# swacisko/ALGA

Measured on AMD Instinct MI355X. Metric: overlap_edges_per_sec, higher is better.
Workload: dtype u32; 1 GPU; cfg4_50M_150bp: 50000000 x 150 bp reads, genome 250000000, seed 11, err 0.00 -> 90621096 nodes (both strands, duplicates removed), min_overlap 82, rsoemo 116; generated on the device (alga_amd.workload.device_build) in 1.0 s; nodes=90621096, edges=92350115

## Files before the change

### alga_amd/csrc/engine.hip

```cpp
#include <hip/hip_runtime.h>

#include <algorithm>
#include <chrono>
#include <cstdio>
#include <cstdlib>
#include <cstring>
#include <new>
#include <string>
#include <thread>
#include <vector>

#include "engine_internal.h"

using namespace alga;

namespace {

using Prepared = AlgaPrepared;

int prepare(alga_engine *e, const alga_nodes *nodes, const alga_prefsuf_params *p, hipStream_t s, Prepared &out) {
    if (!nodes || !p) return alga_fail(e, ALGA_ERR_INVALID_ARGUMENT, "nodes/params must not be NULL");
    if (nodes->n < 0) return alga_fail(e, ALGA_ERR_INVALID_ARGUMENT, "negative node count");
    if (nodes->n > 0 && (!nodes->words || !nodes->len)) return alga_fail(e, ALGA_ERR_INVALID_ARGUMENT, "words/len must not be NULL");
    if (nodes->stride_words <= 0 && nodes->n > 0) return alga_fail(e, ALGA_ERR_INVALID_ARGUMENT, "stride_words must be positive");
// ... 89 lines not shown
    if ((rc = alga_ensure(e, e->cl_pile_tab, pile_table_bytes(n_buckets)))) return rc;
    if (e->cl_pile_tab.p != before || e->cl_pile_tab.cap != cap_before) {
        HIP_TRY(e, hipMemsetAsync(e->cl_pile_tab.p, 0, e->cl_pile_tab.cap, s));
        HIP_TRY(e, hipStreamSynchronize(s));
        e->pile_epoch = 0;
    }
    return ALGA_OK;
}

int discover_impl(alga_engine *e, const Prepared &pp, int32_t src_begin, int32_t src_end, hipStream_t s, uint64_t *n_rec, bool local = false,
                  bool *overflow = nullptr) {
    int rc;
    const NodesDev &nd = pp.nd;
    const PrefSufCfg &cfg = pp.cfg;
    unsigned long long *cnt = (unsigned long long *) e->counters.p;
    *n_rec = 0;
    HIP_TRY(e, hipEventRecord(e->ev[EV_START], s));
    if (pp.live >= (1ull << 31)) return alga_fail(e, ALGA_ERR_CAPACITY, "too many nodes for one seed table; shard the input");
    const bool clustered = local && pp.cluster_eq != 0;
    e->pairs_timed = false;
    e->store_timed = false;
    e->pile_timed = false;
    e->pile_deg_pending = false;
    const bool all_sources = src_begin == 0 && src_end == pp.nd.n;
    const bool pile_index_left = e->opt_pile_range != 0 && e->pile_n == pp.nd.n && e->pile_words == (const void *) pp.nd.words;
    bool pile = clustered && e->opt_pile != 0 && e->opt_cluster_pairs != 0 && e->opt_cluster_order != 0 && pp.local_sw == 1 &&
                      (pp.keys_shared == 0 || (pp.keys_shared == 2 && pile_index_left)) &&
                      (all_sources || (e->opt_pile_range != 0 && src_begin >= 0 && src_end <= pp.nd.n && src_begin < src_end)) && pile_plan(cfg, pp.cluster, pp.cluster_eq, pp.uniform_len, pp.nd.from != nullptr || pp.nd.to != nullptr);
    e->loc_second_used = false;
    bool keys_only = false;
    const bool need_vals = !e->opt_own_sort || e->opt_test_unsorted_index;
    uint32_t n_buckets = 0, filter_bits = 0;
    bool have_table = false;
    auto build_table = [&]() -> int {
        n_buckets = seed_buckets_for(pp.live, e->seed_fill_x10);
        const size_t table_bytes = (size_t) n_buckets * SEED_BUCKET * sizeof(unsigned long long);
        int r;
        if ((r = alga_ensure(e, e->table, table_bytes))) return r;
        HIP_TRY(e, hipMemsetAsync(e->table.p, 0xFF, table_bytes, s));
        filter_bits = seed_filter_bits_for(pp.live);
        if (filter_bits) {
            if ((r = alga_ensure(e, e->filter, filter_bits / 8))) return r;
            HIP_TRY(e, hipMemsetAsync(e->filter.p, 0, filter_bits / 8, s));
        }
        launch_seed_build(nd, cfg, (unsigned long long *) e->table.p, n_buckets, (uint32_t *) e->filter.p, filter_bits, s);
        if ((r = alga_check_launch(e, "k_seed_build"))) return r;
        e->stats.table_slots = (uint64_t) n_buckets * SEED_BUCKET;
        have_table = true;
        return ALGA_OK;
    };
    ClusterCfg cc{};
    if (clustered) {
        cc = pp.cluster;
        if ((rc = cluster_alloc(e, pp))) return rc;
        if (pp.keys_shared == 2) {
            const bool store_left = e->store_n == nd.n && e->store_words == (const void *) nd.words && e->store_eq == pp.cluster_eq && e->store_buckets == cc.n_buckets;
            const bool piles_serve = pile && e->pile_kept_pure && e->store_buckets == cc.n_buckets && e->store_eq == pp.cluster_eq;
            if (!(store_left || piles_serve) || src_begin < e->store_run_begin || src_end > e->store_run_end)
                return alga_fail(e, ALGA_ERR_INVALID_ARGUMENT, "keys_shared = 2: no entry array of this node set that covers the sources is left from the previous build");
            keys_only = pile && e->pile_keys_only;
        } else {
            int32_t run_begin = 0, run_end = nd.n;
            if (pp.keys_shared == 1) {
                if (e->keyed_n != nd.n || e->keyed_words != (const void *) nd.words || src_begin < e->keyed_begin || src_end > e->keyed_end)
                    return alga_fail(e, ALGA_ERR_INVALID_ARGUMENT, "keys_shared: alga_prefsuf_keys_device has not been called on this node set for a range that covers the sources");
                run_begin = e->keyed_begin; run_end = e->keyed_end;
            } else {
                keys_only = pile && e->opt_pile_runs != 0 && !e->expect_pairwise && !e->opt_pile_check;
                launch_cluster_keys(nd, cfg, cc, 0, nd.n, (uint32_t *) e->cl_keys[0].p, need_vals ? (uint32_t *) e->cl_vals[0].p : nullptr, (uint32_t *) e->cl_meta.p, e->cl_runs.p,
                                    (uint8_t *) e->cl_nruns.p, s, !keys_only);
                if ((rc = alga_check_launch(e, "k_node_runs"))) return rc;
            }
            HIP_TRY(e, hipEventRecord(e->ev[EV_KEYS], s));
            e->keyed_n = -1;
            e->store_n = -1;
            HIP_TRY(e, launch_cluster_store(nd, cc, (uint32_t *) e->cl_keys[0].p, (uint32_t *) e->cl_vals[0].p, (uint32_t *) e->cl_keys[1].p,
                                            (uint32_t *) e->cl_vals[1].p, e->sort_temp.p, cluster_sort_temp_bytes((uint64_t) nd.n), e->cl_dir.p, pp.keys_shared == 1 || !need_vals,
                                            e->ev[EV_SORT], cnt + CNT_TOTAL + 1, e->opt_test_unsorted_index != 0, s, e->opt_own_sort != 0));
            HIP_TRY(e, hipEventRecord(e->ev[EV_DIR], s));
            e->pile_n = -1;
            if (pile) {
                rc = e->opt_test_pile_oom ? alga_fail(e, ALGA_ERR_OUT_OF_MEMORY, "pile_alloc (option test_pile_oom)") : pile_alloc(e, (uint64_t) nd.n, cc.n_buckets, s);
                if (rc == ALGA_ERR_OUT_OF_MEMORY) {
                    (void) hipGetLastError();
                    alga_release(e->cl_pile_tab); alga_release(e->cl_pile_rec); alga_release(e->cl_pile_rec2); alga_release(e->cl_pile_succ); alga_release(e->cl_pile_own);
                    alga_release(e->cl_pile_list);
                    e->pile_epoch = 0; e->pile_n = -1;
                    e->err.clear();
                    pile = false;
                    rc = ALGA_OK;
                    if (keys_only) {
                        launch_cluster_keys(nd, cfg, cc, 0, nd.n, (uint32_t *) e->cl_keys[0].p, (uint32_t *) e->cl_vals[0].p, (uint32_t *) e->cl_meta.p, e->cl_runs.p,
                                            (uint8_t *) e->cl_nruns.p, s, true);
                        if ((rc = alga_check_launch(e, "k_node_runs"))) return rc;
                        keys_only = false;
                    }
                } else if (rc) return rc;
            }
            if (pile) {
                launch_pile_sample(nd, cc, pp.uniform_len, (const uint32_t *) e->cl_keys[1].p, (const uint32_t *) e->cl_vals[1].p, e->cl_dir.p,
                                   (unsigned long long *) e->cl_pile_cnt.p, e->opt_pile >= 2 ? e->opt_pile - 1 : 0, s);
                if ((rc = alga_check_launch(e, "k_pile_build<sample>"))) return rc;
            }
            HIP_TRY(e, launch_cluster_gather(nd, cc, pp.cluster_eq, (const uint32_t *) e->cl_keys[1].p, (const uint32_t *) e->cl_vals[1].p, (const uint32_t *) e->cl_meta.p,
                                             pp.uniform_len, e->cl_store.p, (pile && e->opt_pile_skip_gather) ? (const unsigned long long *) e->cl_pile_cnt.p : nullptr, s));
            HIP_TRY(e, hipEventRecord(e->ev[EV_GATHER], s));
            if (pile) {
                if (e->pile_epoch >= 511u) {
                    HIP_TRY(e, hipMemsetAsync(e->cl_pile_tab.p, 0, e->cl_pile_tab.cap, s));
                    e->pile_epoch = 0;
                }
                e->pile_epoch++;
                const bool from_consensus = e->opt_pile_runs != 0;
                launch_pile_build(nd, cfg, cc, pp.uniform_len, (const uint32_t *) e->cl_keys[1].p, (const uint32_t *) e->cl_vals[1].p, e->cl_dir.p, e->cl_pile_rec.p, e->cl_pile_rec2.p, e->cl_pile_tab.p,
                                  e->pile_epoch, e->cl_pile_succ.p, e->cl_runs.p, pp.uniform_len - cfg.Lmin + 1, (const unsigned long long *) e->cl_pile_cnt.p,
                                  from_consensus ? (uint32_t *) e->cl_pile_own.p : nullptr, (from_consensus && e->opt_pile_runs_list) ? e->cl_pile_list.p : nullptr, s);
                if ((rc = alga_check_launch(e, "k_pile_build"))) return rc;
                if (keys_only) {
                    launch_pile_own_ids((const uint32_t *) e->cl_pile_own.p, (const uint32_t *) e->cl_vals[1].p, (uint64_t) nd.n, (int32_t *) e->cl_defer.p, (uint32_t) nd.n,
                                        (unsigned long long *) e->cl_pile_cnt.p, s);
                    launch_cluster_runs_list(nd, cfg, cc, (const int32_t *) e->cl_defer.p, (const unsigned long long *) e->cl_pile_cnt.p + 3, (uint32_t) nd.n, (uint32_t) e->n_cu * 16u,
                                             e->cl_runs.p, (uint8_t *) e->cl_nruns.p, s);
                    launch_cluster_keys(nd, cfg, cc, 0, nd.n, (uint32_t *) e->cl_keys[0].p, (uint32_t *) e->cl_vals[0].p, (uint32_t *) e->cl_meta.p, e->cl_runs.p,
                                        (uint8_t *) e->cl_nruns.p, s, true, (const unsigned long long *) e->cl_pile_cnt.p);
                    if ((rc = alga_check_launch(e, "k_node_runs (own lists)"))) return rc;
                }
                if (e->opt_pile_check && from_consensus)
                    launch_pile_check(e->cl_pile_succ.p, (uint64_t) nd.n, cc.n_buckets, e->cl_pile_tab.p, e->cl_pile_rec2.p, e->pile_epoch, e->cl_runs.p, nd.n, pp.uniform_len - cfg.Lmin + 1,
                                      (unsigned long long *) e->cl_pile_cnt.p, s);
                e->pile_n = nd.n; e->pile_words = (const void *) nd.words;
                e->pile_keys_only = keys_only; e->pile_kept_pure = false;
                e->pile_timed = nd.n > 0;
            }
            e->store_timed = nd.n > 0;
            e->store_n = pile ? -1 : nd.n;
            e->store_words = (const void *) nd.words; e->store_eq = pp.cluster_eq; e->store_buckets = cc.n_buckets;
            e->store_run_begin = run_begin; e->store_run_end = run_end;
        }
        e->stats.table_slots = cc.n_buckets;
    } else if ((rc = build_table())) return rc;
    HIP_TRY(e, hipEventRecord(e->ev[EV_SEED], s));

    const uint64_t n_src = (uint64_t) std::max<int64_t>(0, (int64_t) src_end - src_begin);
    const uint64_t slack = std::max(probe_record_slack(e->n_cu, n_src, local), clustered ? cluster_record_slack(e->n_cu, n_src) : 0);
    uint64_t &hint = local ? e->rec_cap_hint_local : e->rec_cap_hint;
    uint64_t cap = std::max<uint64_t>(hint, (local ? 2 : 16) * n_src + 4096) + slack;
    if (local) {
        if ((rc = alga_ensure(e, e->outdeg, (size_t) (n_src + 1) * sizeof(uint32_t)))) return rc;
        if ((rc = alga_ensure(e, e->loc_first, (size_t) (n_src + 1) * sizeof(unsigned long long)))) return rc;
    }
    const uint32_t big_list_cap = 1u << 20;
    if (local && (rc = alga_ensure(e, e->loc_big_list, big_list_cap * sizeof(int32_t)))) return rc;
    for (int attempt = 0; attempt < 4; attempt++) {
        if (cap >= (1ull << 32) - 16) return alga_fail(e, ALGA_ERR_CAPACITY, "more than 2^32 overlap records; shard the input");
        if (local) HIP_TRY(e, hipMemsetAsync(e->outdeg.p, 0, (size_t) (n_src + 1) * sizeof(uint32_t), s));
        if ((rc = alga_ensure(e, e->rec_dst, cap * sizeof(uint32_t)))) return rc;
        if ((rc = alga_ensure(e, e->rec_val, cap * sizeof(unsigned long long)))) return rc;
        HIP_TRY(e, hipMemsetAsync(cnt, 0, CNT_TOTAL * sizeof(unsigned long long), s));
        ProbeBig big{(int32_t *) e->loc_big_list.p, big_list_cap, 0u, nullptr, 0u};
        e->defer_list_valid = clustered && e->opt_cluster_pairs && pp.local_sw == 1 && pp.cluster_eq <= 4;
        if (clustered) {
            if (e->opt_cluster_pairs && pp.local_sw == 1 && pp.cluster_eq <= 4) {
                if ((rc = alga_ensure(e, e->cl_defer, (size_t) (n_src + 64) * sizeof(int32_t)))) return rc;
                const uint32_t slot_stride = e->opt_stream_slots >= 4 ? (uint32_t) (n_src + 1) : 0u;
                if ((rc = alga_ensure(e, e->loc_second, (size_t) (slot_stride ? LOCAL_SLOTS_MAX - 1 : 1) * (n_src + 1) * sizeof(unsigned long long)))) return rc;
                e->loc_second_used = true;
                e->loc_slot_stride = slot_stride;
                const bool by_key = e->opt_cluster_order != 0 && src_begin == 0 && src_end == nd.n;
                const bool piled = pile && e->pile_n == nd.n && e->pile_words == (const void *) nd.words;
                if (piled) {
// ... 44 lines not shown
        if ((rc = alga_check_launch(e, "k_probe_sources"))) return rc;
        HIP_TRY(e, hipEventRecord(e->ev[EV_PROBE], s));
        HIP_TRY(e, hipMemcpyAsync(e->h_counters, cnt, (CNT_TOTAL + 2) * sizeof(unsigned long long), hipMemcpyDeviceToHost, s));
        HIP_TRY(e, hipStreamSynchronize(s));
        if (clustered && e->h_counters[CNT_TOTAL + 1] != 0) {
            e->store_n = -1; e->keyed_n = -1;
            return alga_fail(e, ALGA_ERR_HIP, "clustered index: the sorted key array is not in order (entry directory invalid)");
        }
        if (local && e->h_counters[CNT_LOCAL_OVERFLOW] != 0) {
            const uint64_t n_big = e->h_counters[CNT_LOCAL_OVERFLOW], max_items = e->h_counters[CNT_LOCAL_MAXITEMS];
            const uint64_t limit = e->big_limit >= 0 ? (uint64_t) e->big_limit : (uint64_t) local_big_limit();
            if (n_big > big_list_cap || max_items > limit) { if (overflow) *overflow = true; *n_rec = 0; return ALGA_OK; }
            big.count = (uint32_t) n_big;
            big.item_cap = (uint32_t) ((max_items + 63) & ~63ull);
            if ((rc = alga_ensure(e, e->loc_big_items, probe_big_bytes(e->n_cu, big.count, pp.local_sw, big.item_cap)))) return rc;
            big.items = e->loc_big_items.p;
            if (!have_table && (rc = build_table())) return rc;
            if (e->pile_deg_pending) {
                launch_pile_deg((int32_t) n_src, (unsigned long long *) e->loc_first.p, (uint32_t *) e->outdeg.p, (const unsigned long long *) e->cl_pile_cnt.p, s);
                e->pile_deg_pending = false;
            }
            HIP_TRY(e, hipMemsetAsync(cnt + CNT_LOCAL_OVERFLOW, 0, sizeof(unsigned long long), s));
            launch_probe(nd, cfg, (const unsigned long long *) e->table.p, n_buckets, (const uint32_t *) e->filter.p, filter_bits, src_begin, src_end,
                         (uint32_t *) e->rec_dst.p, (unsigned long long *) e->rec_val.p, cap, cnt, e->n_cu, pp.local_sw, (uint32_t *) e->outdeg.p,
                         (unsigned long long *) e->loc_first.p, &big, s);
            if ((rc = alga_check_launch(e, "k_probe_sources (second pass)"))) return rc;
            HIP_TRY(e, hipEventRecord(e->ev[EV_PROBE], s));
            HIP_TRY(e, hipMemcpyAsync(e->h_counters, cnt, CNT_TOTAL * sizeof(unsigned long long), hipMemcpyDeviceToHost, s));
            HIP_TRY(e, hipStreamSynchronize(s));
            if (e->h_counters[CNT_LOCAL_OVERFLOW] != 0) { if (overflow) *overflow = true; *n_rec = 0; return ALGA_OK; }
            e->stats.big_sources = n_big;
        }
        const uint64_t need = e->h_counters[CNT_RECORDS];
        if (need <= cap) {
            *n_rec = need;
            hint = std::max<uint64_t>(hint, need + need / 16 + 4096);
            if (overflow) *overflow = false;
            if (local) { e->stats.transitive_compares = e->h_counters[CNT_TR_COMPARES]; e->stats.generic_sources = e->h_counters[CNT_LOCAL_GENERIC]; }
            e->stats.records = e->h_counters[CNT_VALID_RECORDS];
            e->stats.raw_overlaps = e->h_counters[CNT_RAW];
            e->stats.windows_probed = e->h_counters[CNT_WINDOWS];
            e->stats.slots_scanned = e->h_counters[CNT_SLOTS];
            e->stats.probe_rounds = e->h_counters[CNT_ROUNDS];
            e->stats.pile_buckets = e->h_counters[CNT_PILE_BUCKETS]; e->stats.pile_irregular = e->h_counters[CNT_PILE_IRREGULAR];
            e->stats.pile_own_lists = e->h_counters[CNT_PILE_OWN];
            if (pile && pp.keys_shared != 2 && e->pile_n == nd.n) {
                const bool kept = e->opt_pile == 2 || e->stats.pile_irregular * (uint64_t) ALGA_PILE_DECLINE_ONE_IN <= e->stats.pile_buckets;
                e->stats.pile_mixed = kept && e->stats.pile_irregular * (uint64_t) ALGA_PILE_IRREGULAR_ONE_IN > e->stats.pile_buckets;
                e->stats.pile_deferred = e->stats.pile_mixed ? e->h_counters[CNT_DEFERRED_PILE] : (kept ? e->h_counters[CNT_DEFERRED] : 0);
                if (!kept || e->stats.pile_mixed || !e->opt_pile_skip_gather) e->store_n = nd.n;
                e->expect_pairwise = !kept;
                e->pile_kept_pure = kept && !e->stats.pile_mixed && e->opt_pile_skip_gather != 0;
                e->stats.pile_list_checked = 0; e->stats.pile_list_mismatch = 0;
                if (e->opt_pile_check) {
                    unsigned long long chk[2] = {0ull, 0ull};
                    HIP_TRY(e, hipMemcpyAsync(chk, (const unsigned long long *) e->cl_pile_cnt.p + 4, sizeof(chk), hipMemcpyDeviceToHost, s));
                    HIP_TRY(e, hipStreamSynchronize(s));
                    e->stats.pile_list_checked = chk[0]; e->stats.pile_list_mismatch = chk[1];
                }
            }
            if (!pile) e->expect_pairwise = false;
            e->stats.probe_used = clustered ? ALGA_PROBE_CLUSTER : ALGA_PROBE_TABLE;
            if (clustered) e->stats.deferred_sources = e->defer_list_valid ? e->h_counters[CNT_DEFERRED] : n_src;
            return ALGA_OK;
        }
        cap = need + need / 16 + 4096 + slack;
    }
    return alga_fail(e, ALGA_ERR_HIP, "record buffer kept overflowing");
}

int key_bits_for(int64_t n_owned) {
    int b = 1;
    while (b < 31 && (1ll << b) < n_owned) b++;
    return std::min(32, b + 1);
}

int reduce_impl(alga_engine *e, const Prepared &pp, const uint32_t *rec_dst, const unsigned long long *rec_val, uint64_t n_rec,
                uint64_t n_valid_hint, int32_t dst_begin, int32_t dst_end, hipStream_t s, uint64_t *n_edges) {
    int rc;
    const NodesDev &nd = pp.nd;
    const PrefSufCfg &cfg = pp.cfg;
    unsigned long long *cnt = (unsigned long long *) e->counters.p;
    const int32_t n_owned = dst_end - dst_begin;
    *n_edges = 0;
    if (n_rec >= (1ull << 32) - 16) return alga_fail(e, ALGA_ERR_CAPACITY, "more than 2^32 overlap records; shard the input");
    const int bits = key_bits_for(n_owned);
    const size_t temp_bytes = sort_records_temp_bytes(n_rec, bits);
    if ((rc = alga_ensure(e, e->keys, (size_t) (n_rec + 1) * sizeof(uint32_t)))) return rc;
    if ((rc = alga_ensure(e, e->seg_key, (size_t) (n_rec + 1) * sizeof(uint32_t)))) return rc;
    if ((rc = alga_ensure(e, e->seg_val, (size_t) (n_rec + 1) * sizeof(unsigned long long)))) return rc;
    if ((rc = alga_ensure(e, e->sort_temp, temp_bytes))) return rc;
    if ((rc = alga_ensure(e, e->heads, (size_t) (n_rec + 1) * 16))) return rc;
    if ((rc = alga_ensure(e, e->rowptr, (size_t) (n_owned + 2) * sizeof(uint32_t)))) return rc;
    HIP_TRY(e, hipMemsetAsync(cnt + CNT_SORT_VALID, 0, sizeof(unsigned long long), s));
    launch_make_keys(rec_dst, n_rec, dst_begin, dst_end, (uint32_t *) e->keys.p, cnt + CNT_SORT_VALID, s);
    if ((rc = alga_check_launch(e, "k_make_keys"))) return rc;
    HIP_TRY(e, sort_records(e->sort_temp.p, temp_bytes, (const uint32_t *) e->keys.p, (uint32_t *) e->seg_key.p, rec_val,
                            (unsigned long long *) e->seg_val.p, n_rec, bits, s));
    launch_rowptr_from_sorted((const uint32_t *) e->seg_key.p, cnt + CNT_SORT_VALID, n_rec, n_owned, (uint32_t *) e->rowptr.p, s);
    if ((rc = alga_check_launch(e, "k_rowptr_from_sorted"))) return rc;
    launch_gather_heads(nd, (const unsigned long long *) e->seg_val.p, cnt + CNT_SORT_VALID, n_rec, e->heads.p, s);
    if ((rc = alga_check_launch(e, "k_gather_heads"))) return rc;
    HIP_TRY(e, hipEventRecord(e->ev[EV_GROUP], s));

    if ((rc = alga_ensure(e, e->out_cnt, (size_t) (n_owned + 1) * sizeof(uint32_t)))) return rc;
    if ((rc = alga_ensure(e, e->outdeg, (size_t) (nd.n + 1) * sizeof(uint32_t)))) return rc;
// ... 151 lines not shown
    *out = e;
    return ALGA_OK;
}

void alga_engine_destroy(alga_engine *e) {
    if (!e) return;
    DeviceGuard guard;
    (void) hipSetDevice(e->device);
    if (e->own_stream) (void) hipStreamSynchronize(e->own_stream);
    if (e->side_stream) (void) hipStreamSynchronize(e->side_stream);
    for (DevBuf *b : e->owned) alga_release(*b);
    alga_release(e->up_raw);
    for (DevBuf *b : {&e->in_bytes[0], &e->in_bytes[1], &e->in_nl[0], &e->in_nl[1], &e->in_tiles, &e->in_tile_off}) alga_release(*b);
    for (DevBuf *b : {&e->sp_rowptr, &e->sp_sorted, &e->sp_list, &e->sp_cnt, &e->sp_orow, &e->sp_out, &e->sp_in}) alga_release(*b);
    alga_staging_release(e);
    for (void *&p : e->gfa_pin) { if (p) (void) hipHostFree(p); p = nullptr; }
    for (auto &kv : e->host_lists) free(kv.first);
    e->host_lists.clear();
    engine_free_handles(e);
    delete e;
}

const char *alga_last_error(const alga_engine *e) { return e ? e->err.c_str() : "no engine"; }

int alga_engine_device_name(const alga_engine *e, char *buf, size_t buflen) {
    if (!e || !buf || buflen == 0) return ALGA_ERR_INVALID_ARGUMENT;
    snprintf(buf, buflen, "%s", e->dev_name);
    return ALGA_OK;
}

int alga_engine_set_option(alga_engine *e, const char *name, int64_t value) {
    if (!e || !name) return ALGA_ERR_INVALID_ARGUMENT;
    e->err.clear();
    if (!strcmp(name, "probe")) {
        if (value < ALGA_PROBE_AUTO || value > ALGA_PROBE_CLUSTER) return alga_fail(e, ALGA_ERR_INVALID_ARGUMENT, "option probe: 0 auto, 1 table, 2 cluster");
        e->opt_probe = (int) value;
    } else if (!strcmp(name, "cluster_bucket_bias")) {
        if (value < -8 || value > 8) return alga_fail(e, ALGA_ERR_INVALID_ARGUMENT, "option cluster_bucket_bias: -8 .. 8");
        e->opt_cluster_bucket_bias = (int) value;
    } else if (!strcmp(name, "cluster_pairs")) {
        e->opt_cluster_pairs = value != 0;
    } else if (!strcmp(name, "pile")) {
        e->opt_pile = (value == 2 || value == 3) ? (int) value : (value != 0);
    } else if (!strcmp(name, "pile_runs")) {
        e->opt_pile_runs = value != 0;
    } else if (!strcmp(name, "pile_runs_list")) {
        e->opt_pile_runs_list = value != 0;
    } else if (!strcmp(name, "pile_deg_fold")) {
        e->opt_pile_deg_fold = value != 0;
    } else if (!strcmp(name, "pile_probe_lean")) {
        e->opt_pile_probe_lean = value != 0;
    } else if (!strcmp(name, "pile_check")) {
        e->opt_pile_check = value != 0;
    } else if (!strcmp(name, "pile_skip_gather")) {
        e->opt_pile_skip_gather = value != 0;
    } else if (!strcmp(name, "cluster_order")) {
        e->opt_cluster_order = value != 0;
    } else if (!strcmp(name, "local_big_max")) {
        e->big_limit = value < 0 ? -1 : (int) std::min<int64_t>(value, 1 << 20);
    } else if (!strcmp(name, "shard_bucket_max")) {
        e->opt_shard_dmax = (int) std::max<int64_t>(1, std::min<int64_t>(value, 4096));
    } else if (!strcmp(name, "rsort_variant")) {
        rsort_set_variant((int) value);
    } else if (!strcmp(name, "stream_slots")) {
        e->opt_stream_slots = value >= 4 ? 4 : 2;
    } else if (!strcmp(name, "pile_range")) {
        e->opt_pile_range = value != 0;
    } else if (!strcmp(name, "pkb_legacy")) {
        e->opt_pkb_legacy = (int) value;
    } else if (!strcmp(name, "own_sort")) {
        e->opt_own_sort = value != 0;
    } else if (!strcmp(name, "test_presort_oom")) {
        e->opt_test_presort_oom = value != 0;
    } else if (!strcmp(name, "test_pile_oom")) {
        e->opt_test_pile_oom = value != 0;
    } else if (!strcmp(name, "test_unsorted_index")) {
        e->opt_test_unsorted_index = value != 0;
    } else if (!strcmp(name, "gfa_chunk_mb")) {
        if (value < 1 || value > 4096) return alga_fail(e, ALGA_ERR_INVALID_ARGUMENT, "option gfa_chunk_mb: 1 .. 4096");
        e->opt_gfa_chunk_mb = (int) value;
    } else if (!strcmp(name, "auto_reduction_per_target")) {
        e->opt_force_per_target = value != 0;
    } else return alga_fail(e, ALGA_ERR_INVALID_ARGUMENT, "unknown option");
    return ALGA_OK;
}

int alga_engine_reserve(alga_engine *e, int32_t n_nodes, int32_t max_len, int32_t min_overlap, uint64_t n_edges_hint) {
    if (!e) return ALGA_ERR_INVALID_ARGUMENT;
    e->err.clear();
    if (n_nodes < 0 || max_len < 1 || min_overlap < 1) return alga_fail(e, ALGA_ERR_INVALID_ARGUMENT, "alga_engine_reserve: n_nodes >= 0, max_len >= 1, min_overlap >= 1");
    DeviceGuard guard;
    HIP_TRY(e, hipSetDevice(e->device));
    int rc;
    const uint64_t n = (uint64_t) n_nodes;
    const uint64_t E = n_edges_hint ? n_edges_hint : n + n / 16 + 4096;
    if ((rc = alga_ensure(e, e->counters, (CNT_TOTAL + 2) * sizeof(unsigned long long)))) return rc;
    Prepared pp;
    pp.nd.n = n_nodes; pp.max_len = max_len; pp.live = n;
    pp.cfg.Lmin = min_overlap; pp.cfg.Lcap = std::min(max_len, 500) + 1; pp.cfg.rsoemo = min_overlap; pp.cfg.soes = 3;
    int eq = 0;
    const bool local = max_len <= 500 && max_len - min_overlap <= LOCAL_MAX_SPAN;
    const bool clustered = local && e->opt_probe != ALGA_PROBE_TABLE &&
                           cluster_plan(pp.cfg, max_len, n, e->opt_cluster_bucket_bias, &pp.cluster, &eq);
    if (clustered) {
        pp.cluster_eq = eq;
        if ((rc = cluster_alloc(e, pp))) return rc;
// ... 644 lines not shown
```

### alga_amd/csrc/engine_internal.h

```cpp
#pragma once
#include <hip/hip_runtime.h>

#include <cstdio>
#include <algorithm>
#include <string>
#include <vector>
#include <unordered_map>

#include "../../include/alga_amd.h"
#include "prefsuf_common.h"
#include "prefsuf_kernels.h"
#include "pkb_kernels.h"

struct DevBuf {
    void  *p = nullptr;
    size_t cap = 0;
};

enum { EV_START = 0, EV_SEED, EV_PROBE, EV_GROUP, EV_REDUCE, EV_EMIT, EV_PAIRS, EV_KEYS, EV_SORT, EV_GATHER, EV_DIR, EV_COUNT };
constexpr int ALGA_STAGE_THREADS = 8;

struct alga_engine {
    std::vector<DevBuf *> owned;
    int         device = -1;
    hipStream_t own_stream = nullptr;
    hipStream_t side_stream = nullptr;
    hipEvent_t  ev_side = nullptr;
    std::string err;
    char        dev_name[256] = {0};
    int         n_cu = 256;
    int         seed_fill_x10 = 20;
    int         opt_probe = 0;
    int         opt_cluster_bucket_bias = 0;
    int         opt_force_per_target = 0;
    int         opt_shard_dmax = 4096;
    int         opt_test_unsorted_index = 0;
    hipEvent_t  ev[EV_COUNT] = {};
    DevBuf table, filter, counters, rowptr, rec_dst, rec_val, keys, seg_key, seg_val, heads, sort_temp, out_cnt, outdeg, out_rowptr, edges, scan_scratch;
    DevBuf cl_defer;
    uint32_t h_first_hkey = 255;
    int32_t keyed_n = -1, keyed_begin = 0, keyed_end = 0;
    bool defer_list_valid = false;
    const void *keyed_words = nullptr;
    int32_t store_n = -1, store_run_begin = 0, store_run_end = 0, store_eq = 0;
    uint32_t store_buckets = 0;
    const void *store_words = nullptr;
    int stat_max_len = 0, stat_min_len = 0; uint64_t stat_live = 0; unsigned long long stat_mask_asym = 0;
    const void *stat_len = nullptr, *stat_from = nullptr, *stat_to = nullptr;
    bool   warmed = false;
    bool   pairs_timed = false;
    bool   store_timed = false;
    bool   pile_keys_only = false, pile_kept_pure = false;
    int    opt_pile_range = 1;
    int    opt_pile_skip_gather = 1;
    int    opt_pile = 1;
    int    opt_pile_runs = 1;
    int    opt_pile_runs_list = 1;
    DevBuf cl_pile_list;
    int    opt_pile_deg_fold = 1;
    int    opt_pile_probe_lean = 1;
    bool   pile_deg_pending = false;
    int    opt_pile_check = 0;
    bool   expect_pairwise = false;
    DevBuf cl_pile_side_r, cl_pile_cursor;
    DevBuf cl_pile_own;
    int    opt_pkb_legacy = 0;
    int    opt_own_sort = 1;
    int    opt_test_presort_oom = 0;
    int    opt_test_pile_oom = 0;
    bool   pile_timed = false;
    DevBuf cl_pile_succ;
    DevBuf cl_pile_rec2;
    DevBuf cl_pile_rec, cl_pile_cnt, cl_pile_tab;
    uint32_t pile_epoch = 0;
    int32_t pile_n = -1; const void *pile_words = nullptr;
    int    opt_cluster_order = 1;
    int    opt_cluster_pairs = 1;
    DevBuf cl_keys[2], cl_vals[2], cl_meta, cl_runs, cl_nruns, cl_store, cl_dir;
    DevBuf loc_second;
    bool   loc_second_used = false;
    uint32_t loc_slot_stride = 0;
    int    opt_stream_slots = 4;
    DevBuf loc_first, loc_big_list, loc_big_items;
    int    big_limit = -1;
    DevBuf edge_keys, edge_keys2, edge_vals, edge_vals2, edges_sorted, xs_dst, xs_val;
    DevBuf up_words, up_len, up_from, up_to;
    DevBuf up_len_narrow;
    DevBuf cp_deg, cp_dst, cp_off;
    DevBuf cl_defer2;
    DevBuf pk_keys, pk_keys2, pk_vals, pk_vals2, pk_marks, pk_big, pk_add, pk_ekeys, pk_ekeys2, pk_flag, pk_pos, pk_edges[2], pk_rowptr, pk_deg,
           pk_mask, pk_cnt, pk_io, pk_io2, pk_tips, pk_heads, pk_g[2], pk_addk, pk_addk2, pk_merged, pk_hsz, pk_hsz2, pk_heads2, pk_nadd, pk_koff,
           pk_gsz, pk_fixlist, pk_bounds, pk_tiprec, pk_tipidx, pk_keys_all, pk_vals_all;
    DevBuf pk_keys2b, pk_vals2b, pk_headsb, pk_hszb, sort_temp2, pk_fixlist2, pk_cnt2;
    DevBuf pp_rows, pp_len, pp_perm[2], pp_keys[2], pp_mark, pp_keep, pp_pos, pp_out_rows, pp_out_len, pp_out_pair, pp_tally;
    bool        stage_ready = false;
    void       *stage_pin[ALGA_STAGE_THREADS][2] = {};
    hipEvent_t  stage_ev[ALGA_STAGE_THREADS][2] = {};
    hipStream_t stage_stream[ALGA_STAGE_THREADS] = {};
    DevBuf      up_raw;
    std::unordered_map<void *, size_t> host_lists;
    void       *host_spare = nullptr;
    size_t      host_spare_cap = 0;
    DevBuf      in_bytes[2], in_nl[2], in_tiles, in_tile_off;
    DevBuf      sp_rowptr, sp_sorted, sp_list, sp_cnt, sp_orow, sp_out, sp_in;
    DevBuf      gfa_sizes, gfa_off, gfa_rowptr, gfa_tiles, gfa_bounds, gfa_buf;
    void       *gfa_pin[2] = {nullptr, nullptr};
    size_t      gfa_pin_cap = 0;
    int         opt_gfa_chunk_mb = 256;
    DevBuf      sh_keys[2], sh_vals[2], sh_store, sh_dir, sh_desc_out, sh_dkey[2], sh_dval[2], sh_small_top, sh_pending, sh_bitmap, sh_small_out,
                sh_ssrc[2], sh_skey[2], sh_edges_out, sh_deg, sh_rowptr, sh_cursor, sh_edges, sh_flagged, sh_cnt, sh_gflag, sh_gpos, sh_gstart;
    struct {
        int      phase = 0;
        int      rank = 0, n_ranks = 1, eq = 0, uniform_len = 0;
        int32_t  n = 0;
        const void *words = nullptr;
        alga::PrefSufCfg cfg{};
        alga::ClusterCfg cc{};
        uint32_t bucket_base = 0, bpr = 0;
        uint64_t n_targets = 0, n_desc = 0, n_rec = 0;
        uint32_t *d_keys_sorted = nullptr;
        unsigned long long *d_vals_sorted = nullptr;
    } sh;
    alga_shard_stats shard_stats{};
    struct {
        int      phase = 0;
        int      rounds = 0, round = 0, rank = 0, n_ranks = 1, cur = 0, key_bits = 0;
        int32_t  prio[4] = {0, 1, 2, 3};
        uint64_t E = 0, nk = 0;
        uint32_t n_tips = 0;
        int      pre_set = 0, cur_set = 0;
        bool     no_look_ahead = false;
// ... 84 lines not shown
```

### alga_amd/csrc/prefsuf_cluster.hip

```cpp
#include <hip/hip_runtime.h>
#include <algorithm>
#include "prefsuf_common.h"
#include "prefsuf_kernels.h"
#include "prefsuf_device.h"
#include "prefsuf_cluster_device.h"

namespace alga {


template <int TKW, bool WIDE, bool RUNS>
__global__ void __launch_bounds__(TK_ROWS) k_node_runs(NodesDev nd, PrefSufCfg cfg, ClusterCfg cc, int node_begin, int node_end,
                                                        uint32_t *__restrict__ keys, uint32_t *__restrict__ vals, uint32_t *__restrict__ meta,
                                                        uint2 *__restrict__ runs, uint8_t *__restrict__ nruns, const int32_t *__restrict__ id_list, const unsigned long long *__restrict__ id_count,
                                                        const unsigned long long *__restrict__ only_if_declined ) {
    if (only_if_declined && !pile_cnt_declines(only_if_declined)) return;
    __shared__ uint32_t s[TK_ROWS][TKW];
    __shared__ uint32_t stk[RUNS ? 2 * (NR_STACK + 1) : 1][TK_ROWS];
    __shared__ uint16_t rbuf[RUNS ? CL_RMAX + 1 : 1][TK_ROWS];
    const int list_n = id_list ? (int) min((unsigned long long) (node_end - node_begin), *id_count) : 0;
    __shared__ int sid[TK_ROWS];
    for (int blk = (int) blockIdx.x; id_list ? blk * TK_ROWS < list_n : node_begin + blk * TK_ROWS < node_end; blk += (int) gridDim.x) {
    const int base = node_begin + blk * TK_ROWS;
    const int nrows = id_list ? min(TK_ROWS, list_n - blk * TK_ROWS) : min(TK_ROWS, node_end - base);
    if (blk != (int) blockIdx.x) __syncthreads();
// ... 64 lines not shown
            b0 &= b0 - 1ull;
            const int bit = 2 * e, q = bit >> 5, r = bit & 31;
            const uint32_t x0 = row[q], x1 = row[q + 1], x2 = row[q + 2];
            const uint32_t pk = order_key0(kmer_hash(funnel(x0, x1, r) & cc.lo_mask, funnel(x1, x2, r) & cc.hi_mask), e);
            cur0 = pk < cur0 ? pk : cur0;
        }
    }
    uint32_t key = 0xFFFFFFFFu, m = act ? (((uint32_t) len << 8) | (is_src ? CL_META_FROM : 0u)) : 0u;
    if (is_tgt) {
        uint32_t pmin = cur0;
        if (pmin == 0xFFFFFFFFu) {
            for (int k = 0; k < w; k++) { uint32_t h, pk; kmer_key(row, k, true, cc, h, pk); pmin = pk < pmin ? pk : pmin; }
        }
        uint32_t h, pk;
        kmer_key(row, (int) (pmin & 255u), true, cc, h, pk);
        key = tgt_sort_key(cluster_key(h, fs), pmin & 255u, fs);
        m = (pmin & 255u) | ((uint32_t) len << 8) | (is_src ? CL_META_FROM : 0u);
    }
    if (in) { keys[i] = key; if (vals) vals[i] = (uint32_t) i; meta[i] = m; }
    }
}

template <int EQ, bool UNIFORM>
__global__ void __launch_bounds__(256) k_tgt_gather(NodesDev nd, uint64_t count ,
                                                     const uint32_t *__restrict__ keys, const uint32_t *__restrict__ vals,
                                                     const uint32_t *__restrict__ meta, uint32_t uniform_meta, int fs, uint4 *__restrict__ store,
                                                     const unsigned long long *__restrict__ pile_cnt ) {
    if (pile_cnt && pile_cnt[1] * PILE_IRREGULAR_ONE_IN <= pile_cnt[0]) return;
    for (uint64_t t = (uint64_t) blockIdx.x * blockDim.x + threadIdx.x; t < count * EQ; t += (uint64_t) gridDim.x * blockDim.x) {
    const uint64_t j = t / EQ;
    const int c = (int) (t % EQ);
    const uint32_t key = keys[j];
    const uint32_t id = vals[j];
    const uint32_t *row = nd.words + (size_t) id * nd.stride;
    uint4 v;
    if ((nd.stride & 3) == 0 && 4 * c + 3 < nd.stride && ((uintptr_t) nd.words & 15u) == 0) v = reinterpret_cast<const uint4 *>(row)[c];
    else {
        v.x = 4 * c + 0 < nd.stride ? row[4 * c + 0] : 0u; v.y = 4 * c + 1 < nd.stride ? row[4 * c + 1] : 0u;
        v.z = 4 * c + 2 < nd.stride ? row[4 * c + 2] : 0u; v.w = 4 * c + 3 < nd.stride ? row[4 * c + 3] : 0u;
    }
    if (c == EQ - 1) {
        v.y = id; v.z = key;
        if (!UNIFORM) v.w = meta[id];
        else if (key != 0xFFFFFFFFu) v.w = uniform_meta | ((key >> fs) & ((1u << CL_MBITS) - 1u));
        else v.w = (uint32_t) nd.len[id] == (uniform_meta >> 8 & 0xFFFu) ? uniform_meta : 0u;
    }
    store[j * EQ + c] = v;
    }
}

constexpr int TD_TILE = 256, TD_HALO = 96;
__global__ void __launch_bounds__(TD_TILE) k_tgt_dir(const uint32_t *__restrict__ keys, uint64_t n, int shift, uint32_t n_buckets ,
                                                     uint32_t bucket_base , uint4 *__restrict__ dir,
                                                     unsigned long long *__restrict__ bad ) {
    __shared__ uint32_t sb[TD_TILE + TD_HALO + 1];
    const uint64_t base = (uint64_t) blockIdx.x * TD_TILE;
    const uint32_t nb3 = n_buckets << 3;
    auto tagged = [&](uint64_t k) -> uint32_t { if (k >= n) return nb3; const uint32_t x = keys[k]; return x == 0xFFFFFFFFu ? nb3 : (x >> (shift - 3)) - (bucket_base << 3); };
    for (int k = (int) threadIdx.x; k <= TD_TILE + TD_HALO; k += TD_TILE)
        sb[k] = (base == 0 && k == 0) ? 0xFFFFFFFFu : tagged(base + (uint64_t) k - 1u);
    __syncthreads();
    const int t = (int) threadIdx.x, lane = lane_id();
    const uint64_t j = base + (uint64_t) t;
    auto put = [&](int64_t b, const uint4 &rec) { dir[b] = rec; };
    auto tally = [](unsigned long long acc, uint32_t cls) { return acc + (0x0101010101010100ull << (8u * cls)); };
    if (j >= 1 && j < n && sb[t + 1] < sb[t]) atomicOr(bad, 1ull);
    const uint32_t b = sb[t + 1] >> 3;
    const bool start = j <= n && b != (sb[t] >> 3);
    if (start && b == n_buckets) put(b, make_uint4((uint32_t) j, 0u, 0u, 0u));
    const bool real = start && b != n_buckets;
    constexpr int TD_SHORT = 4;
    const bool is_short = real && (sb[t + 1 + TD_SHORT] >> 3) != b;
    if (is_short) {
        unsigned long long acc = 0ull;
        int u = 0;
#pragma unroll
        for (; u < TD_SHORT; u++) {
            const uint32_t x = sb[t + 1 + u];
            if ((x >> 3) != b) break;
            acc = tally(acc, x & 7u);
        }
        put(b, make_uint4((uint32_t) j, (uint32_t) u, (uint32_t) acc, (uint32_t) (acc >> 32)));
    }
    unsigned long long longs = __ballot(real && !is_short);
    const int g = lane >> 4, gl = lane & 15;
    while (longs != 0ull) {
        int lsel = 64;
#pragma unroll
        for (int q = 0; q < 4; q++) {
            const int l = longs ? __builtin_ctzll(longs) : 64;
            longs = longs ? (longs & (longs - 1ull)) : 0ull;
            lsel = g == q ? l : lsel;
        }
        const bool has = lsel < 64;
        const int t0 = (t & ~63) + (has ? lsel : 0);
        const uint32_t bb = bperm(b, has ? lsel : 0);
        unsigned long long acc = 0ull;
        bool open = has, past = false;
        for (int u = 0;; u += 16) {
            const int idx = t0 + 1 + u + gl;
            const bool staged = idx <= TD_TILE + TD_HALO;
            const uint32_t x = staged ? sb[idx] : 0xFFFFFFFFu;
            const bool inb = open && staged && (x >> 3) == bb;
            const unsigned long long c = inb ? ((0x0101010101010100ull << (8u * (x & 7u))) | 1ull) : 0ull;
            uint32_t lo = (uint32_t) c, hi = (uint32_t) (c >> 32);
            lo += (uint32_t) __builtin_amdgcn_update_dpp(0, (int) lo, 0x111, 0xF, 0xF, true); hi += (uint32_t) __builtin_amdgcn_update_dpp(0, (int) hi, 0x111, 0xF, 0xF, true);
            lo += (uint32_t) __builtin_amdgcn_update_dpp(0, (int) lo, 0x112, 0xF, 0xF, true); hi += (uint32_t) __builtin_amdgcn_update_dpp(0, (int) hi, 0x112, 0xF, 0xF, true);
            lo += (uint32_t) __builtin_amdgcn_update_dpp(0, (int) lo, 0x114, 0xF, 0xF, true); hi += (uint32_t) __builtin_amdgcn_update_dpp(0, (int) hi, 0x114, 0xF, 0xF, true);
            lo += (uint32_t) __builtin_amdgcn_update_dpp(0, (int) lo, 0x118, 0xF, 0xF, true); hi += (uint32_t) __builtin_amdgcn_update_dpp(0, (int) hi, 0x118, 0xF, 0xF, true);
            lo = bperm(lo, lane | 15); hi = bperm(hi, lane | 15);
            acc += ((unsigned long long) hi << 32) | lo;
            const uint32_t took = lo & 255u, cnt = (uint32_t) acc & 255u;
            if (open && took < 16u) { open = false; past = t0 + 1 + u + (int) took > TD_TILE + TD_HALO; }
            else if (open && cnt >= 240u) { open = false; past = true; }
            if (__ballot(open) == 0ull) break;
        }
        if (has && gl == 0) {
// ... 48 lines not shown
    __shared__ uint32_t sRecC[PROBE_WAVES][WBUF_LOCAL];
    __shared__ unsigned long long sRecV[PROBE_WAVES][WBUF_LOCAL];
    __shared__ uint32_t sCnt[PROBE_WAVES][3];
    __shared__ uint32_t sItemC[PROBE_WAVES][ITEMMAX];
    __shared__ uint32_t sItemM[PROBE_WAVES][ITEMMAX];
    __shared__ uint4 sItemO[PROBE_WAVES][ITEMMAX * SW];
    __shared__ uint8_t sItemT[PROBE_WAVES][64 * SW];
    __shared__ uint4 sMask[KF > 0 ? 129 : 1];
    const int wave = __builtin_amdgcn_readfirstlane((int) (threadIdx.x >> 6));
    const int lane = lane_id();
    WaveLds w{sB[wave][0], nullptr, nullptr, &sCnt[wave][0], sRecC[wave], sRecV[wave], &sCnt[wave][1]};
    ItemLds it{sItemC[wave], sItemM[wave], sItemO[wave], sItemT[wave], &sCnt[wave][2]};
    if (lane == 0) { *w.recN = 0; *it.N = 0; }
    if constexpr (KF > 0) {
        for (int t = (int) threadIdx.x; t <= 128; t += PROBE_WAVES * 64)
            sMask[t] = make_uint4(low_bits32(t), low_bits32(t - 32), low_bits32(t - 64), low_bits32(t - 96));
        __syncthreads();
    }
    uint64_t chunk_base = 0;
    int chunk_fill = REC_CHUNK_LOCAL;
    uint64_t st_raw = 0, st_slots = 0, st_win = 0, st_rec = 0, st_cmp = 0, st_generic = 0;
    const int total_waves = (int) gridDim.x * PROBE_WAVES;
    const int kfull = KF ? KF : (2 * cfg.Lmin) >> 5;

    const int pre_words = nd.stride < STAGE_WORDS ? nd.stride : STAGE_WORDS;
    int Bl = src_begin + (int) blockIdx.x * PROBE_WAVES + wave;
    int n_id = 0, n_len = 0, n_nr = 0; uint32_t n_word = 0; uint2 n_run = make_uint2(0u, 0u);
    auto fetch = [&]() {
        if (Bl < src_end) {
            const int b = src_list ? __builtin_amdgcn_readfirstlane(src_list[Bl]) : Bl;
            n_id = b;
            n_len = nd.len[b];
            n_nr = nruns[b];
            n_word = lane < pre_words ? nd.words[(size_t) b * nd.stride + lane] : 0u;
            if (lane < CL_RMAX) n_run = runs[(size_t) b * CL_RMAX + lane];
        }
    };
    fetch();
    auto advance = [&](int &B, int &lenB, int &nr, uint32_t &word0, uint2 &run) -> bool {
        while (Bl < src_end) {
            B = n_id; lenB = __builtin_amdgcn_readfirstlane(n_len); nr = __builtin_amdgcn_readfirstlane(n_nr); word0 = n_word; run = n_run;
            Bl = total_waves <= src_end - Bl ? Bl + total_waves : src_end;
            fetch();
            if (nr != 0) return true;
        }
        return false;
    };
    auto stage = [&](int buf, int lenB, int nr, uint32_t word0, const uint2 &run) -> uint32_t {
        const int nwB = blocks_of(lenB);
        wave_lds_fence();
        if (lane < STAGE_WORDS) sB[wave][buf][lane] = lane < nwB ? word0 : 0u;
        return lane < nr ? run.x >> cc.idx_shift : 0u;
    };
    auto index_loads = [&](uint32_t bucket, uint4 &rec) { rec = dir[bucket]; };
    auto finish_runs = [&](int buf, int nr, const uint2 &run, const uint4 &rec) -> uint32_t {
        uint32_t e0, cnt;
        run_slice(rec, run.y, e0, cnt);
        cnt = lane < nr ? cnt : 0u;
        if (lane < CL_RMAX) sRun[wave][buf][lane] = make_uint4(run.y, run.x, e0, cnt);
        uint32_t m = cnt, t;
        t = (uint32_t) __builtin_amdgcn_update_dpp(0, (int) m, 0x111, 0xF, 0xF, true); m = m > t ? m : t;
        t = (uint32_t) __builtin_amdgcn_update_dpp(0, (int) m, 0x112, 0xF, 0xF, true); m = m > t ? m : t;
        t = (uint32_t) __builtin_amdgcn_update_dpp(0, (int) m, 0x114, 0xF, 0xF, true); m = m > t ? m : t;
        wave_lds_fence();
        return (uint32_t) __builtin_amdgcn_readlane((int) m, CL_RMAX - 1);
    };
    auto load_runs = [&](int buf, int gs, uint4 &rp) { rp = sRun[wave][buf][(lane >> gs) & (CL_RMAX - 1)]; };
    auto load_entries = [&](const uint4 &rp, uint32_t k0, int gs, bool &ev, size_t &ei, uint32_t (&ew)[4 * EQ]) {
        const uint32_t j = k0 + ((uint32_t) lane & ((1u << gs) - 1u));
        ev = j < rp.w;
        ei = ev ? (size_t) min(rp.z + j, (uint32_t) nd.n - 1u) : (size_t) 0;
        if (BYID) {
            const uint32_t key = by.skeys[ei], id = min(by.sids[ei], (uint32_t) nd.n - 1u);
            const uint32_t *row = nd.words + (size_t) id * nd.stride;
#pragma unroll
            for (int k = 0; k < WC; k++) ew[k] = k < nd.stride ? row[k] : 0u;
            ew[4 * EQ - 3] = id; ew[4 * EQ - 2] = key;
            ew[4 * EQ - 1] = key != 0xFFFFFFFFu ? (by.uniform_meta | ((key >> (cc.idx_shift - CL_MBITS)) & ((1u << CL_MBITS) - 1u))) : 0u;
            return;
        }
#pragma unroll
        for (int c = 0; c < EQ; c++) { const uint4 v = store[ei * EQ + c]; ew[4 * c] = v.x; ew[4 * c + 1] = v.y; ew[4 * c + 2] = v.z; ew[4 * c + 3] = v.w; }
    };

    int B = 0, lenB = 0, nr = 0;
    uint32_t word0 = 0, mc = 0;
    uint2 run = make_uint2(0u, 0u);
    bool have = advance(B, lenB, nr, word0, run);
    int buf = 0;
    if (have) {
        uint4 rec0;
        const uint32_t bk = stage(0, lenB, nr == CL_RUNS_FLAGGED ? 0 : nr, word0, run);
        index_loads(bk, rec0);
        mc = finish_runs(0, nr == CL_RUNS_FLAGGED ? 0 : nr, run, rec0);
    }
    while (have) {
        const uint32_t *sb = sB[wave][buf];
        const int nwin = lenB - cfg.Lmin + 1;
        int nB = 0, nlenB = 0, nnr = 0;
        uint32_t nword0 = 0, nbk = 0;
        uint4 nrec;
        uint2 nrun = make_uint2(0u, 0u);
        const bool have_next = advance(nB, nlenB, nnr, nword0, nrun);
        const int nnr_eff = nnr == CL_RUNS_FLAGGED ? 0 : nnr;
        const bool flagged = nr == CL_RUNS_FLAGGED;
        int gs = (nr > 4 || flagged) ? 3 : 4;
        uint32_t k0 = 0;
// ... 101 lines not shown
                        if (__popcll(surv) == 1) {
                            if (v_pass && !removed) {
                                o.first[B - o.src_base] = ((unsigned long long) v_id << 32) | (uint32_t) d;
                                o.deg[B - o.src_base] = 1u;
                                st_rec++;
                            }
                            if (STATS && has_pred) st_cmp++;
                            reduced = true;
                        }
                    }
                }
                if (!reduced) {
                    if (v_pass) {
                        const int slot = (int) __builtin_amdgcn_mbcnt_hi((uint32_t) (v_pm >> 32), __builtin_amdgcn_mbcnt_lo((uint32_t) v_pm, 0u));
                        it.C[slot] = v_id; it.M[slot] = v_m; it.O[slot] = v_o;
                    }
                }
            }
        } else {
            for (;;) {
                k0 += 1u << gs;
                if (k0 >= mc) break;
                load_entries(rp, k0, gs, ev, ei, ew);
                verify(true);
            }
        }
        if (flagged) {
            gs = 3;
            for (int wb = 0; wb < nwin; wb += 64) {
                const int wl = wb + lane;
                const bool wv = wl < nwin;
                uint32_t wm = 0xFFFFFFFFu;
                for (int k = 0; k < cc.w; k++) {
                    uint32_t h, pk;
                    kmer_key(sb, (wv ? wl : 0) + k, true, cc, h, pk);
                    wm = pk < wm ? pk : wm;
                }
                const uint32_t prev = bperm(wm, (lane + 63) & 63);
                const bool start = wv && (lane == 0 || wm != prev);
                const uint64_t runmask = __ballot(start);
                const int nrun_all = __popcll(runmask);
                const uint64_t higher = lane >= 63 ? 0ull : runmask & ~((2ull << lane) - 1ull);
                const int wend = nwin - wb < 64 ? nwin - wb : 64;
                const int p1 = wb + (higher ? __builtin_ctzll(higher) : wend);
                const int rank = (int) __builtin_amdgcn_mbcnt_hi((uint32_t) (runmask >> 32), __builtin_amdgcn_mbcnt_lo((uint32_t) runmask, 0u));
                uint32_t key = 0u;
                { uint32_t h, pk; kmer_key(sb, (int) (wm & 255u) < 192 ? (int) (wm & 255u) : 0, true, cc, h, pk); key = cluster_key(h, cc.idx_shift - CL_MBITS); }
                for (int rb = 0; rb < nrun_all; rb += CL_RMAX) {
                    wave_lds_fence();
                    if (lane < CL_RMAX) sRun[wave][buf][lane] = make_uint4(0u, 0u, 0u, 0u);
                    wave_lds_fence();
                    uint32_t cnt = 0u;
                    if (start && rank >= rb && rank < rb + CL_RMAX) {
                        const uint4 rec = dir[key >> cc.idx_shift];
                        const uint32_t ry = (wm & 255u) | ((uint32_t) wl << 8) | ((uint32_t) p1 << 16);
                        uint32_t e0;
                        run_slice(rec, ry, e0, cnt);
                        sRun[wave][buf][rank - rb] = make_uint4(ry, key, e0, cnt);
                    }
                    wave_lds_fence();
                    const uint32_t mcs = (uint32_t) wave_max_u64_dpp((uint64_t) cnt);
                    load_runs(buf, gs, rp);
                    for (k0 = 0; k0 < mcs; k0 += 1u << gs) { load_entries(rp, k0, gs, ev, ei, ew); verify(true); }
                }
            }
        }
        wave_lds_fence();
        if (STATS && lane == 0) st_win += (uint64_t) nwin;
        if (n_items > ITEMMAX) {
            if (lane == 0) {
                const unsigned long long k = atomicAdd(&o.counters[CNT_LOCAL_OVERFLOW], 1ull);
                if (k < (unsigned long long) o.big_list_cap) o.big_list[k] = B;
                atomicMax(&o.counters[CNT_LOCAL_MAXITEMS], (unsigned long long) n_items);
                if (STATS) { st_raw -= (uint64_t) n_items; st_win -= (uint64_t) nwin; }
            }
        } else if (n_items > 0 && !reduced) {
            local_reduce<STATS, WBUF_LOCAL, SW>(nd, cfg, it, w, o, B, lenB, n_items, st_rec, st_cmp, st_generic);
        }
        const int nb2 = (int) __builtin_amdgcn_readfirstlane((int) *w.recN);
        if (nb2 >= WFLUSH_LOCAL) flush_records<REC_CHUNK_LOCAL, WBUF_LOCAL>(o, w, chunk_base, chunk_fill);
        mc = finish_runs(buf ^ 1, nnr_eff, nrun, nrec);
        have = have_next; B = nB; lenB = nlenB; nr = nnr; buf ^= 1;
    }
    flush_records<REC_CHUNK_LOCAL, WBUF_LOCAL>(o, w, chunk_base, chunk_fill);
    close_chunk<REC_CHUNK_LOCAL>(o, chunk_base, chunk_fill);
    st_rec = wave_sum_u64(st_rec);
    if (lane == 0 && st_rec) atomicAdd(&o.counters[CNT_VALID_RECORDS], (unsigned long long) st_rec);
    if (STATS) {
        st_raw = wave_sum_u64(st_raw); st_slots = wave_sum_u64(st_slots); st_win = wave_sum_u64(st_win);
        st_cmp = wave_sum_u64(st_cmp); st_generic = wave_sum_u64(st_generic);
        if (lane == 0) {
            atomicAdd(&o.counters[CNT_RAW], (unsigned long long) st_raw);
            atomicAdd(&o.counters[CNT_SLOTS], (unsigned long long) st_slots);
            atomicAdd(&o.counters[CNT_WINDOWS], (unsigned long long) st_win);
            atomicAdd(&o.counters[CNT_TR_COMPARES], (unsigned long long) st_cmp);
            atomicAdd(&o.counters[CNT_LOCAL_GENERIC], (unsigned long long) st_generic);
        }
    }
}

#ifndef CLQ_OCC_IDORDER
#define CLQ_OCC_IDORDER 5
#endif
constexpr int clq_occ(int eq, int kf, bool bykey) { return (eq == 4 || (eq == 3 && kf == 3)) ? 5 : (bykey ? 6 : CLQ_OCC_IDORDER); }
template <bool STATS, int EQ, int KF, bool BYKEY, bool LIST = false>
__global__ void __launch_bounds__(PROBE_WAVES * 64, clq_occ(EQ, KF, BYKEY))
k_probe_stream(NodesDev nd, PrefSufCfg cfg, ClusterCfg cc, const uint4 *__restrict__ store, const uint4 *__restrict__ dir,
// ... 71 lines not shown
    uint2 b_run = make_uint2(0u, 0u);
    auto next_pos = [&](int p) { return step <= src_end - p ? p + step : src_end; };
    auto list_at = [&](int pos) -> int {
        const int j = pos + g, js = j < last_src ? j : last_src;
        return (int) min((uint32_t) src_list[js], (uint32_t) nd.n - 1u);
    };
    int a_lid = 0, n_lid = 0;
    if constexpr (LIST) { a_lid = list_at(posA); n_lid = list_at(next_pos(posA)); }
    auto fetchA = [&]() {
        const int j = posA + g;
        a_valid = j < src_end;
        const int js = j < last_src ? j : last_src;
        if constexpr (LIST) {
            a_id = a_lid;
            a_len = nd.len[a_lid];
            a_word = nd.words[(size_t) a_lid * nd.stride + col];
        } else
        if constexpr (BYKEY) {
            const uint32_t *ent = reinterpret_cast<const uint32_t *>(store) + (size_t) js * (4 * EQ);
            a_word = ent[col];
            a_id = (int) min(ent[4 * EQ - 3], (uint32_t) nd.n - 1u);
            a_len = (int) ((ent[4 * EQ - 1] >> 8) & 0xFFFu);
        } else {
            a_id = js;
            a_len = nd.len[js];
            a_word = nd.words[(size_t) js * nd.stride + col];
        }
    };
    auto fetchB = [&]() {
        b_run = runs[(size_t) b_id * CL_RMAX + (gl & (CL_RMAX - 1))];
        b_nrw = run_w[(size_t) b_id * (2 * CL_RMAX) + 1];
    };
    auto take = [&](int &id, int &len, int &nrn, uint32_t &word, uint2 &run) {
        id = b_id;
        len = b_valid ? b_len : 0; nrn = b_valid ? (int) (b_nrw >> 24) : 0;
        word = (b_valid && gl < pre_words) ? b_word : 0u;
        run = (b_valid && gl < CL_RMAX) ? b_run : make_uint2(0u, 0u);
    };
    auto advance = [&](bool adv) {
        b_valid = adv ? a_valid : b_valid; b_id = adv ? a_id : b_id; b_len = adv ? a_len : b_len; b_word = adv ? a_word : b_word;
        posB = adv ? posA : posB;
        posA = adv ? (step <= src_end - posA ? posA + step : src_end) : posA;
        if constexpr (LIST) { a_lid = adv ? n_lid : a_lid; n_lid = list_at(next_pos(posA)); }
        fetchB();
        fetchA();
    };
    fetchA();
    auto stage = [&](int qb, int id, int lenB, int nr_eff, uint32_t word0, const uint2 &run) -> uint32_t {
        wave_lds_fence();
        sB[wave][4 * qb + g][gl] = gl < blocks_of(lenB) ? word0 : 0u;
        if (gl == 0) sSrc[wave][4 * qb + g] = make_uint2((uint32_t) id, (uint32_t) lenB);
        return gl < nr_eff ? run.x >> cc.idx_shift : 0u;
    };
    auto index_loads = [&](uint32_t bucket, uint4 &rec) { rec = dir[bucket]; };
    auto finish_runs = [&](int qb, int nr_eff, const uint2 &run, const uint4 &rec) -> uint32_t {
        uint32_t e0, cnt;
        run_slice(rec, run.y, e0, cnt);
        cnt = gl < nr_eff ? cnt : 0u;
        uint32_t inc = cnt, t;
        t = (uint32_t) __builtin_amdgcn_update_dpp(0, (int) inc, 0x111, 0xF, 0xF, true); inc += t;
        t = (uint32_t) __builtin_amdgcn_update_dpp(0, (int) inc, 0x112, 0xF, 0xF, true); inc += t;
        t = (uint32_t) __builtin_amdgcn_update_dpp(0, (int) inc, 0x114, 0xF, 0xF, true); inc += t;
        if (gl < CL_RMAX) {
            sRun[wave][4 * qb + g][gl] = make_uint4(run.y, run.x, e0 - (inc - cnt), cnt);
            reinterpret_cast<uint8_t *>(&sIncl[wave][4 * qb + g])[gl] = (uint8_t) (inc > 255u ? 255u : inc);
        }
        if (gl == 0) { sOcc[wave][4 * qb + g] = 0ull; sStat[wave][4 * qb + g] = 0u; }
        wave_lds_fence();
        return inc;
    };
    auto quad_plan = [&](uint32_t inc, int nrv, uint32_t &t4w, uint32_t &fl ) {
        t4w = 0u; fl = 0u;
#pragma unroll
        for (int q = 0; q < 4; q++) {
            const int T = __builtin_amdgcn_readlane((int) inc, q * 16 + CL_RMAX - 1), nrq = __builtin_amdgcn_readlane(nrv, q * 16);
            const bool p = nrq != 0 && nrq != CL_RUNS_FLAGGED && T <= 64;
            t4w |= (p ? (uint32_t) T : 0u) << (8 * q);
            fl |= (p ? 1u << q : 0u) | (nrq != 0 ? 16u << q : 0u);
        }
    };

    uint64_t tw = 0ull;
    uint32_t fl0 = 0u, fl1 = 0u;
    int b0 = 0, b1 = 1, b2 = 2, cur = 0;
    uint32_t red = 0u;
    int pos0 = posA;
    bool have0 = posA < src_end;
    if (have0) {
        int id, len, nrv; uint32_t word0; uint2 run; uint4 rec;
        advance(true);
        take(id, len, nrv, word0, run);
        pos0 = posB;
        advance(true);
        {
            const int ne = nrv == CL_RUNS_FLAGGED ? 0 : nrv;
            const uint32_t bk = stage(0, id, len, ne, word0, run);
            index_loads(bk, rec);
            const uint32_t inc = finish_runs(0, ne, run, rec);
            uint32_t t4w;
            quad_plan(inc, nrv, t4w, fl0);
            tw = (uint64_t) t4w;
        }
        const bool have1 = posB < src_end;
        take(id, len, nrv, word0, run);
        advance(have1);
        {
            const int ne = nrv == CL_RUNS_FLAGGED ? 0 : nrv;
// ... 260 lines not shown
    const int nwin = max_len - cfg.Lmin + 1;
    if (e > CL_MAX_EQ || nwin < 1 || nwin > 128) return false;
    int kk = std::min(32, std::max(cfg.Lmin - 63, std::min(cfg.Lmin, CL_KMIN)));
    const int nw_half = std::min(nwin, 64);
    if (nw_half > std::min(cfg.Lmin - kk + 1, 64)) kk = cfg.Lmin - nw_half + 1;
    if (kk < CL_KMIN_HARD || kk > 32 || kk > cfg.Lmin) return false;
    c->kk = kk;
    c->w = std::min(cfg.Lmin - kk + 1, 64);
    c->lo_mask = kk >= 16 ? 0xFFFFFFFFu : ((1u << (2 * kk)) - 1u);
    c->hi_mask = kk <= 16 ? 0u : (kk >= 32 ? 0xFFFFFFFFu : ((1u << (2 * kk - 32)) - 1u));
    int bits = 4;
    while (bits < 28 && (1ull << bits) < live) bits++;
    bits = std::max(4, std::min(32 - CL_MBITS, bits + bucket_log2_bias));
    c->n_buckets = 1u << bits;
    c->idx_shift = 32 - bits;
    *eq = e;
    return true;
}

size_t cluster_sort_temp_bytes(uint64_t n) { return sort_u32_pairs_temp_bytes(n); }

void launch_cluster_keys(const NodesDev &nd, const PrefSufCfg &cfg, const ClusterCfg &cc, int32_t node_begin, int32_t node_end, uint32_t *keys, uint32_t *vals,
                         uint32_t *meta, void *runs, uint8_t *nruns, hipStream_t s, bool with_runs, const unsigned long long *only_if_declined) {
    if (node_end <= node_begin) return;
    const uint64_t m = (uint64_t) (node_end - node_begin);
    const unsigned long long *gate = only_if_declined;
    const dim3 grid((unsigned) (gate ? std::min<uint64_t>((m + TK_ROWS - 1) / TK_ROWS, 8192) : (m + TK_ROWS - 1) / TK_ROWS)), block(TK_ROWS);
    const int32_t *nol = nullptr; const unsigned long long *noc = nullptr;
#define NR_LAUNCH(TKW, WIDE) do { if (with_runs) hipLaunchKernelGGL((k_node_runs<TKW, WIDE, true>), grid, block, 0, s, nd, cfg, cc, (int) node_begin, (int) node_end, keys, vals, meta, (uint2 *) runs, nruns, nol, noc, gate); \
                                  else hipLaunchKernelGGL((k_node_runs<TKW, WIDE, false>), grid, block, 0, s, nd, cfg, cc, (int) node_begin, (int) node_end, keys, vals, meta, (uint2 *) runs, nruns, nol, noc, gate); } while (0)
    if (blocks_of(cfg.Lcap - 1) > 13 || (cfg.Lcap - 1) - cfg.Lmin + 1 > 64) NR_LAUNCH(21, true);
    else if (blocks_of(cfg.Lcap - 1) <= 9) NR_LAUNCH(11, false);
    else NR_LAUNCH(17, false);
#undef NR_LAUNCH
}

void launch_cluster_runs_list(const NodesDev &nd, const PrefSufCfg &cfg, const ClusterCfg &cc, const int32_t *ids, const unsigned long long *count, uint32_t cap, uint32_t grid_blocks,
                              void *runs, uint8_t *nruns, hipStream_t s) {
    if (cap == 0 || nd.n <= 0) return;
    const dim3 grid(std::max<uint32_t>(1u, std::min<uint32_t>(grid_blocks, (cap + TK_ROWS - 1) / TK_ROWS))), block(TK_ROWS);
    uint32_t *nok = nullptr;
#define NR_LAUNCH(TKW, WIDE) hipLaunchKernelGGL((k_node_runs<TKW, WIDE, true>), grid, block, 0, s, nd, cfg, cc, 0, (int) cap, nok, nok, nok, (uint2 *) runs, nruns, ids, count, (const unsigned long long *) nullptr)
    if (blocks_of(cfg.Lcap - 1) > 13 || (cfg.Lcap - 1) - cfg.Lmin + 1 > 64) NR_LAUNCH(21, true);
    else if (blocks_of(cfg.Lcap - 1) <= 9) NR_LAUNCH(11, false);
    else NR_LAUNCH(17, false);
#undef NR_LAUNCH
}

__global__ void __launch_bounds__(256) k_iota(uint32_t *__restrict__ v, uint32_t n) {
    for (uint32_t i = blockIdx.x * 256u + threadIdx.x; i < n; i += gridDim.x * 256u) v[i] = i;
}

hipError_t launch_cluster_store(const NodesDev &nd, const ClusterCfg &cc, uint32_t *keys, uint32_t *vals, uint32_t *keys2, uint32_t *vals2,
                                void *sort_temp, size_t sort_temp_bytes, void *dir, bool fill_vals,
                                hipEvent_t ev_sorted, unsigned long long *bad_flag, bool test_skip_sort, hipStream_t s, bool own_sort) {
    if (nd.n <= 0) return hipSuccess;
    const uint64_t n = (uint64_t) nd.n;
    if (fill_vals && (!own_sort || test_skip_sort)) hipLaunchKernelGGL(k_iota, dim3((unsigned) std::min<uint64_t>((n + 255) / 256, 8192)), dim3(256), 0, s, vals, (uint32_t) n);
    hipError_t err = hipSuccess;
    if (test_skip_sort) {
        err = hipMemcpyAsync(keys2, keys, n * sizeof(uint32_t), hipMemcpyDeviceToDevice, s);
        if (err == hipSuccess) err = hipMemcpyAsync(vals2, vals, n * sizeof(uint32_t), hipMemcpyDeviceToDevice, s);
    } else err = sort_u32_pairs(sort_temp, sort_temp_bytes, keys, keys2, own_sort ? (const uint32_t *) nullptr : vals, vals2, n, cc.idx_shift - 3, s, own_sort);
    if (err != hipSuccess) return err;
    if (ev_sorted) (void) hipEventRecord(ev_sorted, s);
    err = hipMemsetAsync(dir, 0, ((size_t) cc.n_buckets + 2) * 16, s);
    if (err != hipSuccess) return err;
    hipLaunchKernelGGL(k_tgt_dir, dim3((unsigned) ((n + 1 + TD_TILE - 1) / TD_TILE)), dim3(TD_TILE), 0, s, (const uint32_t *) keys2, n, cc.idx_shift, cc.n_buckets, 0u, (uint4 *) dir, bad_flag);
    return hipGetLastError();
}

hipError_t launch_cluster_gather(const NodesDev &nd, const ClusterCfg &cc, int eq, const uint32_t *keys2, const uint32_t *vals2, const uint32_t *meta, int uniform_len,
                                 void *store, const unsigned long long *pile_cnt, hipStream_t s) {
    if (nd.n <= 0) return hipSuccess;
    const uint64_t n = (uint64_t) nd.n;
    const uint64_t pieces = n * (uint64_t) eq;
    const unsigned g = (unsigned) std::min<uint64_t>((pieces + 255) / 256, 1u << 16);
    const int fs = cc.idx_shift - CL_MBITS;
    const uint32_t um = uniform_len > 0 ? (((uint32_t) uniform_len << 8) | CL_META_FROM) : 0u;
#define TG_LAUNCH(E, U) hipLaunchKernelGGL((k_tgt_gather<E, U>), dim3(g), dim3(256), 0, s, nd, n, keys2, vals2, meta, um, fs, (uint4 *) store, pile_cnt)
#define TG_EQ(E) do { if (uniform_len > 0) TG_LAUNCH(E, true); else TG_LAUNCH(E, false); } while (0)
    if (eq == 2)      TG_EQ(2);
    else if (eq == 3) TG_EQ(3);
    else if (eq == 4) TG_EQ(4);
    else              TG_EQ(5);
#undef TG_EQ
#undef TG_LAUNCH
    return hipGetLastError();
}

hipError_t launch_cluster_store_slice(const NodesDev &nd, const ClusterCfg &cc, int eq, uint64_t m, uint32_t bucket_base, uint32_t n_buckets_local, uint32_t *keys,
                                      uint32_t *vals, uint32_t *keys2, uint32_t *vals2, const uint32_t *meta, int uniform_len, void *sort_temp, size_t sort_temp_bytes,
                                      void *store, void *dir, unsigned long long *bad_flag, hipStream_t s, bool own_sort) {
    hipError_t err = hipMemsetAsync(dir, 0, ((size_t) n_buckets_local + 2) * 16, s);
    if (err != hipSuccess || m == 0) return err;
    err = sort_u32_pairs(sort_temp, sort_temp_bytes, keys, keys2, vals, vals2, m, cc.idx_shift - 3, s, own_sort);
    if (err != hipSuccess) return err;
    const uint64_t n = m, pieces = m * (uint64_t) eq;
    const unsigned g = (unsigned) ((pieces + 255) / 256);
    const int fs = cc.idx_shift - CL_MBITS;
    const uint32_t um = uniform_len > 0 ? (((uint32_t) uniform_len << 8) | CL_META_FROM) : 0u;
#define TG_LAUNCH(E, U) hipLaunchKernelGGL((k_tgt_gather<E, U>), dim3(g), dim3(256), 0, s, nd, n, (const uint32_t *) keys2, (const uint32_t *) vals2, meta, um, fs, (uint4 *) store, (const unsigned long long *) nullptr)
#define TG_EQ(E) do { if (uniform_len > 0) TG_LAUNCH(E, true); else TG_LAUNCH(E, false); } while (0)
    if (eq == 2)      TG_EQ(2);
    else if (eq == 3) TG_EQ(3);
    else if (eq == 4) TG_EQ(4);
    else              TG_EQ(5);
#undef TG_EQ
#undef TG_LAUNCH
    hipLaunchKernelGGL(k_tgt_dir, dim3((unsigned) ((n + 1 + TD_TILE - 1) / TD_TILE)), dim3(TD_TILE), 0, s, (const uint32_t *) keys2, n, cc.idx_shift, n_buckets_local, bucket_base,
                       (uint4 *) dir, bad_flag);
    return hipGetLastError();
}

uint64_t cluster_probe_blocks(int n_cu, uint64_t n_src) {
    return std::max<uint64_t>(1, std::min<uint64_t>((n_src + PROBE_WAVES - 1) / PROBE_WAVES, (uint64_t) std::max(1, n_cu) * CL_OCC));
}

uint64_t cluster_record_slack(int n_cu, uint64_t n_src) { return cluster_probe_blocks(n_cu, n_src) * PROBE_WAVES * (uint64_t) REC_CHUNK_LOCAL; }

void launch_probe_stream(const NodesDev &nd, const PrefSufCfg &cfg, const ClusterCfg &cc, int eq, const void *store, const void *dir,
                         const void *runs, const uint8_t *nruns, int32_t src_begin, int32_t src_end, bool by_key, unsigned long long *counters, int n_cu,
                         uint32_t *deg, unsigned long long *first, unsigned long long *second, int32_t *defer_list, uint32_t defer_cap,
                         const unsigned long long *pile_cnt, hipStream_t s, uint32_t slot_stride) {
    const int64_t ns = (int64_t) src_end - src_begin;
    if (ns <= 0) return;
    const uint64_t quads = ((uint64_t) ns + 3) / 4;
    const int kf = (2 * cfg.Lmin) >> 5;
    const int kfs = (eq == 3 && (kf == 5 || kf == 3)) || (eq == 2 && kf == 3) ? kf : 0;
    dim3 grid((unsigned) std::max<uint64_t>(1, std::min<uint64_t>((quads + PROBE_WAVES - 1) / PROBE_WAVES, (uint64_t) std::max(1, n_cu) * clq_occ(eq <= 3 ? eq : 4, kfs, by_key)))),
         block(PROBE_WAVES * 64);
    ProbeOut o{nullptr, nullptr, 0, counters, deg, first, by_key ? 0 : src_begin, second};
    o.slot_stride = slot_stride;
    const uint4 *st = (const uint4 *) store;
#define CLQ_LAUNCH(ST, E, K, BK) hipLaunchKernelGGL((k_probe_stream<ST, E, K, BK>), grid, block, 0, s, nd, cfg, cc, st, (const uint4 *) dir, (const uint2 *) runs, nruns, src_begin, src_end, o, defer_list, defer_cap, pile_cnt, \
                                                    (const int32_t *) nullptr, (const unsigned long long *) nullptr)
#define CLQ_ORDER(ST, E, K) do { if (by_key) CLQ_LAUNCH(ST, E, K, true); else CLQ_LAUNCH(ST, E, K, false); } while (0)
#define CLQ_STATS(E, K) do { if (cfg.stats) CLQ_ORDER(true, E, K); else CLQ_ORDER(false, E, K); } while (0)
    if (eq == 3 && kf == 5)      CLQ_STATS(3, 5);
    else if (eq == 3 && kf == 3) CLQ_STATS(3, 3);
    else if (eq == 2 && kf == 3) CLQ_STATS(2, 3);
    else if (eq == 2)            CLQ_STATS(2, 0);
    else if (eq == 3)            CLQ_STATS(3, 0);
    else                         CLQ_STATS(4, 0);
#undef CLQ_STATS
#undef CLQ_ORDER
#undef CLQ_LAUNCH
}

__global__ void __launch_bounds__(256) k_defer_swap(const unsigned long long *__restrict__ pile_cnt, unsigned long long *__restrict__ counters, const int32_t *__restrict__ list2,
                                                     int32_t *__restrict__ list, uint32_t cap) {
    if (!pile_cnt_mixed(pile_cnt)) return;
    const uint64_t n2 = min(counters[CNT_DEFERRED2], (unsigned long long) cap);
    for (uint64_t i = (uint64_t) blockIdx.x * blockDim.x + threadIdx.x; i < n2; i += (uint64_t) gridDim.x * blockDim.x) list[i] = list2[i];
    if (blockIdx.x == 0 && threadIdx.x == 0) { counters[CNT_DEFERRED_PILE] = counters[CNT_DEFERRED]; counters[CNT_DEFERRED] = n2; }
}

void launch_probe_stream_list(const NodesDev &nd, const PrefSufCfg &cfg, const ClusterCfg &cc, int eq, const void *store, const void *dir, const void *runs, const uint8_t *nruns,
                              int32_t *src_list, uint32_t list_cap, unsigned long long *counters, int n_cu, uint32_t *deg, unsigned long long *first,
                              unsigned long long *second, int32_t *defer2, const unsigned long long *pile_cnt, hipStream_t s, uint32_t slot_stride, int32_t src_base) {
    if (eq != 3 || list_cap == 0) return;
    const int kf = (2 * cfg.Lmin) >> 5;
    const int kfs = (kf == 5 || kf == 3) ? kf : 0;
    const dim3 grid((unsigned) std::max(1, n_cu) * clq_occ(3, kfs, false)), block(PROBE_WAVES * 64);
// ... 51 lines not shown
```

### alga_amd/csrc/prefsuf_cluster_device.h

```cpp
#pragma once
#include <hip/hip_runtime.h>
#include "prefsuf_common.h"
#include "../../include/alga_amd.h"
#include "prefsuf_device.h"

namespace alga {

__device__ __forceinline__ uint32_t kmer_hash(uint32_t lo, uint32_t hi) {
    return (lo ^ __funnelshift_l(hi, hi, 13) ^ (hi >> 7)) * 0x9E3779B1u;
}

__device__ __forceinline__ bool kmer_class0(uint32_t lo) { return (lo & 3u) == 0u && ((((lo >> 2) ^ (lo >> 3)) & 1u) != 0u); }
__device__ __forceinline__ uint32_t order_key0(uint32_t h, int pos) { return ((h >> 1) & 0x7FFFFF00u) | (uint32_t) pos; }
__device__ __forceinline__ uint32_t order_key(uint32_t h, uint32_t lo, int pos) { return order_key0(h, pos) | (kmer_class0(lo) ? 0u : 0x80000000u); }
__device__ __forceinline__ uint32_t class0_mask16(uint32_t cur, uint32_t nxt) {
    const uint32_t nx = __funnelshift_r(cur, nxt, 2);
    return ~(cur | (cur >> 1)) & (nx ^ (nx >> 1)) & 0x55555555u;
}
__device__ __forceinline__ uint32_t compress_even(uint32_t x) {
    x = (x | (x >> 1)) & 0x33333333u;
    x = (x | (x >> 2)) & 0x0F0F0F0Fu;
    x = (x | (x >> 4)) & 0x00FF00FFu;
    return (x | (x >> 8)) & 0x0000FFFFu;
}

__device__ __forceinline__ uint32_t cluster_key(uint32_t h, int fs) {
    uint32_t k = h * 0x9E3779B1u;
    k ^= k >> 15;
    k *= 0x85EBCA77u;
    k ^= k >> 13;
    k *= 0xC2B2AE3Du;
    return (k >> (fs + CL_MBITS)) == (0xFFFFFFFFu >> (fs + CL_MBITS)) ? k ^ 0x80000000u : k;
}

__device__ __forceinline__ uint32_t tgt_sort_key(uint32_t ckey, uint32_t m_c, int fs) {
    const uint32_t fm = ((1u << CL_MBITS) - 1u) << fs;
    return (ckey & ~fm) | ((m_c << fs) & fm);
}
__device__ __forceinline__ bool same_cluster(uint32_t entry_key, uint32_t ckey, int fs) {
    return ((entry_key ^ ckey) & ~(((1u << CL_MBITS) - 1u) << fs)) == 0u;
}

constexpr unsigned long long PILE_IRREGULAR_ONE_IN = ALGA_PILE_IRREGULAR_ONE_IN;
constexpr unsigned long long PILE_DECLINE_ONE_IN = ALGA_PILE_DECLINE_ONE_IN;
__device__ __forceinline__ bool pile_cnt_declines(const unsigned long long *c) { return c[1] * PILE_DECLINE_ONE_IN > c[0]; }
__device__ __forceinline__ bool pile_cnt_mixed(const unsigned long long *c) { return !pile_cnt_declines(c) && c[1] * PILE_IRREGULAR_ONE_IN > c[0]; }
__device__ __forceinline__ void run_slice(const uint4 &rec, uint32_t run_y, uint32_t &e0, uint32_t &cnt) {
    const int q = (int) (run_y & 255u), p0 = (int) ((run_y >> 8) & 255u), p1 = (int) ((run_y >> 16) & 255u);
    int mlo = q - p1 + 1, mhi = q - p0;
    mlo = mlo < 0 ? 0 : mlo; mhi = mhi > 63 ? 63 : mhi;
    e0 = rec.x; cnt = rec.y;
    if (mhi < mlo) { cnt = 0u; return; }
    if (rec.y > 255u) return;
    const int s0 = mlo >> 3, s1 = (mhi >> 3) + 1;
    const uint32_t b0 = ((s0 < 4 ? rec.z : rec.w) >> (8 * (s0 & 3))) & 255u;
    const uint32_t b1 = s1 >= 8 ? rec.y : (((s1 < 4 ? rec.z : rec.w) >> (8 * (s1 & 3))) & 255u);
    e0 = rec.x + b0; cnt = b1 - b0;
}

template <int RS = 1, int RW = 0>
__device__ __forceinline__ uint32_t row_word(const uint32_t *row, int k) {
    if (RW > 0) { const uint32_t v = row[(k < RW ? k : RW - 1) * RS]; return k < RW ? v : 0u; }
    return row[k * RS];
}

template <int RS = 1, int RW = 0>
__device__ __forceinline__ void kmer_key(const uint32_t *row, int i, bool valid, const ClusterCfg &cc, uint32_t &h, uint32_t &pk) {
    const int bit = 2 * i, q = bit >> 5, r = bit & 31;
    const uint32_t x0 = row_word<RS, RW>(row, q), x1 = row_word<RS, RW>(row, q + 1), x2 = row_word<RS, RW>(row, q + 2);
    const uint32_t lo = funnel(x0, x1, r) & cc.lo_mask;
    h = kmer_hash(lo, funnel(x1, x2, r) & cc.hi_mask);
    pk = valid ? order_key(h, lo, i) : 0xFFFFFFFFu;
}

constexpr int TK_ROWS = 128;
constexpr int NR_STACK = 8;

template <bool WIDE, int RCAP = CL_RMAX, int RS = 1, int RW = 0>
__device__ __forceinline__ void node_runs_core(const uint32_t *row, int nwin, bool act, const ClusterCfg &cc, uint32_t (*stk)[TK_ROWS], uint16_t (*rbuf)[TK_ROWS], int t,
                                               int &nr, bool &uncovered, bool &stack_ovf, uint32_t &cur0, int step = 64) {
    constexpr int S0 = NR_STACK + 1;
    const int w = cc.w;
    nr = 0; uncovered = false; stack_ovf = false; cur0 = 0xFFFFFFFFu;
    for (int hb = (WIDE && nwin > step) ? ((nwin - 1) / step) * step : 0; hb >= 0; hb -= step) {
        const int h0 = hb >> 4;
        auto rowh = [&](int k) -> uint32_t { return row_word<RS, RW>(row, h0 + k); };
        const int nwh = !WIDE ? nwin : (nwin - hb < step ? nwin - hb : step);
        const int nk = act ? nwh - 1 + w : 0;
        uint64_t m_lo, m_hi;
        {
            uint32_t dm[4];
#pragma unroll
            for (int d = 0; d < 4; d++) {
                const uint32_t x0 = rowh(2 * d), x1 = rowh(2 * d + 1), x2 = rowh(2 * d + 2);
                dm[d] = compress_even(class0_mask16(x0, x1)) | (compress_even(class0_mask16(x1, x2)) << 16);
            }
            m_lo = (uint64_t) dm[0] | ((uint64_t) dm[1] << 32);
            m_hi = (uint64_t) dm[2] | ((uint64_t) dm[3] << 32);
            m_lo &= nk >= 64 ? ~0ull : (nk <= 0 ? 0ull : ((1ull << nk) - 1ull));
// ... 77 lines not shown
```

### alga_amd/csrc/prefsuf_common.h

```cpp
#pragma once
#include <stdint.h>

#if defined(__HIPCC__)
#define ALGA_HD __host__ __device__
#else
#define ALGA_HD
#endif

namespace alga {

constexpr uint32_t OL_OFF_MASK = 0x3FFFFFu;
constexpr int      OL_LEN_SHIFT = 22;
constexpr uint32_t OL_LEN_MASK = 0x1FFu;
constexpr int      OL_MAX_NODE_LEN = (1 << 22) - 1;
constexpr uint32_t OL_SMALL = 0x80000000u;

ALGA_HD inline uint32_t ol_pack(int off, int L, bool small) {
    return (uint32_t) off | ((uint32_t) L << OL_LEN_SHIFT) | (small ? OL_SMALL : 0u);
}
ALGA_HD inline int  ol_off(uint32_t ol) { return (int) (ol & OL_OFF_MASK); }
ALGA_HD inline int  ol_len(uint32_t ol) { return (int) ((ol >> OL_LEN_SHIFT) & OL_LEN_MASK); }
ALGA_HD inline bool ol_small(uint32_t ol) { return (ol & OL_SMALL) != 0; }

constexpr int SEED_MAX_NT = 64;
// ... 19 lines not shown

enum Counter {
    CNT_RECORDS = 0,
    CNT_RAW,
    CNT_WINDOWS,
    CNT_SLOTS,
    CNT_TR_LISTED,
    CNT_TR_COMPARES,
    CNT_TR_REMOVED,
    CNT_EDGES,
    CNT_MAX_IN,
    CNT_LIVE_NODES,
    CNT_VALID_RECORDS,
    CNT_SORT_VALID,
    CNT_MASK_ASYM,
    CNT_LOCAL_OVERFLOW,
    CNT_LOCAL_GENERIC,
    CNT_LOCAL_MAXITEMS,
    CNT_DEFERRED,
    CNT_ROUNDS,
    CNT_PILE_BUCKETS,
    CNT_PILE_IRREGULAR,
    CNT_PILE_OWN,
    CNT_DEFERRED2,
    CNT_DEFERRED_PILE,
    CNT_TOTAL = 24
};
constexpr int LOCAL_SLOTS_MAX = 4;


struct NodesDev {
    const uint32_t *words;
    const int32_t  *len;
    const uint8_t  *from;
    const uint8_t  *to;
    int32_t n;
    int32_t stride;
};

constexpr int      CL_KMIN = 16;
constexpr int      CL_KMIN_HARD = 8;
constexpr int      CL_MBITS = 6;
constexpr int      CL_RMAX = 8;
constexpr int      CL_RUNS_FLAGGED = 0xFF;
constexpr int      CL_MAX_EQ = 5;
constexpr uint32_t CL_META_FROM = 1u << 20;
struct ClusterCfg {
    int32_t  kk;
    int32_t  w;
    uint32_t lo_mask;
    uint32_t hi_mask;
    int32_t  idx_shift;
    uint32_t n_buckets;
};

struct PrefSufCfg {
    int32_t Lmin;
    int32_t rsoemo;
    int32_t Lcap;
    int32_t soes;
    int32_t seed_words;
    uint32_t seed_last_mask;
    int32_t reversed;
    int32_t stats;
};

}
```

### alga_amd/csrc/prefsuf_kernels.h

```cpp
#pragma once
#include <hip/hip_runtime.h>
#include <stddef.h>
#include <stdint.h>
#include "prefsuf_common.h"

namespace alga {

struct alga_edge_dev { int32_t src, dst, offset; };

void launch_restride(const uint32_t *in, int stride_in, uint32_t *out, int stride_out, uint64_t n, hipStream_t s);
void launch_widen_len(const void *in, int elem_bytes , int32_t *out, uint64_t n, hipStream_t s);
void launch_compact_edges(const alga_edge_dev *edges, int32_t n, uint64_t n_edges, uint8_t *deg, uint32_t *dst, uint8_t *off, unsigned long long *bad, hipStream_t s);
void launch_expand_twins(const uint32_t *in, int stride_in, const int32_t *len , uint32_t *out, int stride_out, uint64_t n_pairs, hipStream_t s);
void launch_node_stats(const NodesDev &nd, unsigned long long *counters, int *max_len , hipStream_t s);

uint32_t seed_buckets_for(uint64_t live_nodes, int fill_x10);
uint32_t seed_filter_bits_for(uint64_t live_nodes);
void launch_seed_build(const NodesDev &nd, const PrefSufCfg &cfg, unsigned long long *table, uint32_t n_buckets, uint32_t *filter,
                       uint32_t filter_bits, hipStream_t s);

struct ProbeBig { int32_t *list; uint32_t list_cap; uint32_t count; void *items; uint32_t item_cap; };
int    local_item_capacity();
int    local_big_limit();
size_t probe_big_bytes(int n_cu, uint32_t count, int local, uint32_t item_cap);

void launch_probe(const NodesDev &nd, const PrefSufCfg &cfg, const unsigned long long *table, uint32_t n_buckets,
                  const uint32_t *filter, uint32_t filter_bits, int32_t src_begin, int32_t src_end, uint32_t *rec_dst, unsigned long long *rec_val, uint64_t rec_cap,
                  unsigned long long *counters, int n_cu, int local , uint32_t *deg , unsigned long long *first ,
                  const ProbeBig *big , hipStream_t s);
uint64_t probe_record_slack(int n_cu, uint64_t n_src, bool local);
void launch_local_emit(int32_t src_base, int32_t n_src, const uint32_t *deg, const unsigned long long *first, const unsigned long long *second,
                       const uint32_t *rec_dst, const unsigned long long *rec_val, uint64_t n_rec, const uint32_t *rowptr, uint32_t *cursor,
                       alga_edge_dev *edges, const int32_t *record_sources, const unsigned long long *record_sources_count, uint32_t record_sources_cap, hipStream_t s, uint32_t slot_stride = 0);

bool       cluster_plan(const PrefSufCfg &cfg, int max_len, uint64_t live, int bucket_log2_bias, ClusterCfg *c, int *eq);
size_t     cluster_sort_temp_bytes(uint64_t n);
void       launch_cluster_keys(const NodesDev &nd, const PrefSufCfg &cfg, const ClusterCfg &cc, int32_t node_begin, int32_t node_end, uint32_t *keys,
                               uint32_t *vals, uint32_t *meta, void *runs, uint8_t *nruns, hipStream_t s, bool with_runs = true ,
                               const unsigned long long *only_if_declined = nullptr );
void       launch_cluster_runs_list(const NodesDev &nd, const PrefSufCfg &cfg, const ClusterCfg &cc, const int32_t *ids, const unsigned long long *count, uint32_t cap,
                                    uint32_t grid_blocks, void *runs, uint8_t *nruns, hipStream_t s);
hipError_t launch_cluster_store(const NodesDev &nd, const ClusterCfg &cc, uint32_t *keys, uint32_t *vals, uint32_t *keys2 , uint32_t *vals2, void *sort_temp,
                                size_t sort_temp_bytes, void *dir, bool fill_vals, hipEvent_t ev_sorted ,
                                unsigned long long *bad_flag ,
                                bool test_skip_sort , hipStream_t s, bool own_sort = true);
hipError_t launch_cluster_gather(const NodesDev &nd, const ClusterCfg &cc, int eq, const uint32_t *keys2, const uint32_t *vals2, const uint32_t *meta,
                                 int uniform_len , void *store,
                                 const unsigned long long *pile_cnt , hipStream_t s);
uint64_t   cluster_record_slack(int n_cu, uint64_t n_src);
void       launch_probe_clustered(const NodesDev &nd, const PrefSufCfg &cfg, const ClusterCfg &cc, int eq, const void *store, const void *dir,
                                  const void *runs, const uint8_t *nruns, int32_t src_begin, int32_t src_end, const int32_t *src_list, int32_t src_base, uint32_t *rec_dst, unsigned long long *rec_val, uint64_t rec_cap,
                                  unsigned long long *counters, int n_cu, uint32_t *deg, unsigned long long *first, const ProbeBig *big,
                                  const unsigned long long *list_count ,
                                  int sw , hipStream_t s,
                                  const uint32_t *skeys = nullptr, const uint32_t *sids = nullptr, int uniform_len = 0,
                                  const unsigned long long *pile_cnt = nullptr );
void       launch_probe_stream(const NodesDev &nd, const PrefSufCfg &cfg, const ClusterCfg &cc, int eq, const void *store, const void *dir,
                               const void *runs, const uint8_t *nruns, int32_t src_begin, int32_t src_end, bool by_key ,
                               unsigned long long *counters, int n_cu, uint32_t *deg, unsigned long long *first, unsigned long long *second, int32_t *defer_list,
                               uint32_t defer_cap, const unsigned long long *pile_cnt ,
                               hipStream_t s, uint32_t slot_stride = 0 );
void       launch_pile_deg(int32_t n, unsigned long long *first, uint32_t *deg, const unsigned long long *pile_cnt, hipStream_t s);
bool       pile_plan(const PrefSufCfg &cfg, const ClusterCfg &cc, int eq, int uniform_len, bool masks);
size_t     pile_record_bytes(uint64_t n);
size_t     pile_table_bytes(uint32_t n_buckets);
void       launch_pile_sample(const NodesDev &nd, const ClusterCfg &cc, int uniform_len, const uint32_t *skeys , const uint32_t *sids , const void *dir,
                              unsigned long long *pile_cnt , int no_sample, hipStream_t s);
constexpr int PILE_CNT_WORDS = 6;
size_t     pile_own_mask_bytes(uint64_t n);
size_t     pile_list_bytes(uint64_t n);
void       launch_pile_build(const NodesDev &nd, const PrefSufCfg &cfg, const ClusterCfg &cc, int uniform_len, const uint32_t *skeys, const uint32_t *sids, const void *dir, void *rec,
                             void *rec2 , void *tab, uint32_t epoch, void *side, const void *runs, int nwin, const unsigned long long *pile_cnt,
                             uint32_t *own_mask ,
                             void *plist , hipStream_t s);
void       launch_pile_own_ids(const uint32_t *own_mask, const uint32_t *sids, uint64_t n_entries, int32_t *list, uint32_t cap, unsigned long long *pile_cnt, hipStream_t s);
void       launch_pile_check(const void *side, uint64_t n_entries, uint32_t n_buckets, const void *tab, const void *rec2, uint32_t epoch, const void *runs, int n_nodes, int nwin,
                             unsigned long long *pile_cnt, hipStream_t s);
void       launch_probe_stream_list(const NodesDev &nd, const PrefSufCfg &cfg, const ClusterCfg &cc, int eq, const void *store, const void *dir, const void *runs, const uint8_t *nruns,
                                    int32_t *src_list, uint32_t list_cap, unsigned long long *counters, int n_cu, uint32_t *deg, unsigned long long *first,
                                    unsigned long long *second, int32_t *defer2, const unsigned long long *pile_cnt, hipStream_t s, uint32_t slot_stride = 0,
                                    int32_t src_base = 0 );
void       launch_pile_probe(const NodesDev &nd, const PrefSufCfg &cfg, const ClusterCfg &cc, int uniform_len, const void *tab, uint32_t epoch, const void *rec, const void *rec2, const void *side,
                             const void *runs, unsigned long long *counters, uint32_t *deg, unsigned long long *first, unsigned long long *second, int32_t *defer_list,
                             uint32_t defer_cap, const unsigned long long *pile_cnt, int n_cu, hipStream_t s, int32_t src_begin, int32_t src_end,
                             void *side_range , unsigned long long *cursor ,
                             bool lean = true );

size_t     rsort_u32_pairs_temp_bytes(uint64_t n);
void       rsort_set_variant(int v);
hipError_t rsort_u32_pairs(void *temp, size_t temp_bytes, const uint32_t *keys_in, uint32_t *keys_out, const uint32_t *vals_in, uint32_t *vals_out, uint64_t n,
                           int begin_bit, hipStream_t s);
size_t     sort_u32_pairs_temp_bytes(uint64_t n);
hipError_t sort_u32_pairs(void *temp, size_t temp_bytes, const uint32_t *keys_in, uint32_t *keys_out, const uint32_t *vals_in, uint32_t *vals_out,
                          uint64_t n, int begin_bit , hipStream_t s, bool own_sort = true );
size_t     rsort_u64_pairs_temp_bytes(uint64_t n);
hipError_t rsort_u64_pairs(void *temp, size_t temp_bytes, const unsigned long long *keys_in, unsigned long long *keys_out, const unsigned long long *vals_in,
                           unsigned long long *vals_out, uint64_t n, int bits, hipStream_t s);
hipError_t rsort_u32_u64(void *temp, size_t temp_bytes, const uint32_t *keys_in, uint32_t *keys_out, const unsigned long long *vals_in, unsigned long long *vals_out,
                         uint64_t n, int begin_bit, int end_bit, hipStream_t s);
size_t     sort_u64_pairs_temp_bytes(uint64_t n, int bits);
hipError_t sort_u64_pairs(void *temp, size_t temp_bytes, const unsigned long long *keys_in, unsigned long long *keys_out,
                          const unsigned long long *vals_in, unsigned long long *vals_out, uint64_t n, int bits, hipStream_t s);

void launch_make_keys(const uint32_t *rec_dst, uint64_t n_rec, int32_t dst_begin, int32_t dst_end, uint32_t *keys,
                      unsigned long long *n_valid, hipStream_t s);
size_t     sort_records_temp_bytes(uint64_t n, int bits);
hipError_t sort_records(void *temp, size_t temp_bytes, const uint32_t *keys_in, uint32_t *keys_out, const unsigned long long *vals_in,
                        unsigned long long *vals_out, uint64_t n, int bits, hipStream_t s);
void launch_rowptr_from_sorted(const uint32_t *keys, const unsigned long long *n_valid_ptr, uint64_t n_rec_max, int32_t n_owned,
                               uint32_t *rowptr, hipStream_t s);

size_t   scan_scratch_bytes(uint64_t n);
uint64_t scan_total_index(uint64_t n);
void launch_exclusive_scan(const uint32_t *in, uint64_t n, uint32_t *out, uint64_t *scratch, hipStream_t s);
void launch_exclusive_scan_pile_deg(uint32_t *deg, uint64_t n, uint32_t *out, uint64_t *scratch, unsigned long long *first, const unsigned long long *pile_cnt, hipStream_t s);
constexpr int MAIL_SEGS = 6;
struct MailSeg { const uint32_t *src; uint32_t words, dst; };
struct MailArgs {
    MailSeg seg[MAIL_SEGS];
    int n = 0;
    void add(const void *src, uint32_t words, uint32_t dst_word) { seg[n].src = (const uint32_t *) src; seg[n].words = words; seg[n].dst = dst_word; n++; }
};
void launch_mail(const MailArgs &a, uint32_t *host_block_dev, hipStream_t s);

int  reduce_targets_per_block(uint64_t n_records, uint64_t n_targets);
void launch_gather_heads(const NodesDev &nd, const unsigned long long *seg_val, const unsigned long long *n_valid_ptr, uint64_t n_rec_max,
                         void *heads , hipStream_t s);
void launch_reduce_targets(const NodesDev &nd, const PrefSufCfg &cfg, int32_t dst_begin, int32_t n_owned, int32_t targets_per_block,
// ... 15 lines not shown
```

### alga_amd/csrc/prefsuf_pile.hip

```cpp
#include <hip/hip_runtime.h>
#include <algorithm>
#include "prefsuf_common.h"
#include "prefsuf_kernels.h"
#include "prefsuf_device.h"
#include "prefsuf_cluster_device.h"

namespace alga {

constexpr int PB_TILE = 192, PB_HALO = 64, PB_THREADS = PB_TILE + PB_HALO;
constexpr int PILE_SW = 13;
constexpr int PILE_MAXSUB = 4;
constexpr int PILE_EQ = 3;

__device__ __forceinline__ bool pile_declines(const unsigned long long *pile_cnt) { return pile_cnt_declines(pile_cnt); }

__device__ __forceinline__ uint32_t pile_who(uint32_t group, uint32_t w, uint32_t n_buckets, uint64_t n_entries) {
    return group == 0u ? min(w, n_buckets) : (uint32_t) min((uint64_t) w, n_entries) | 0x80000000u;
}

__device__ __forceinline__ void load_row9(const NodesDev &nd, uint32_t id, uint32_t (&row)[9]) {
    const uint32_t *rp = nd.words + (size_t) id * nd.stride;
    if ((nd.stride & 3) == 0 && nd.stride >= 12 && ((uintptr_t) nd.words & 15u) == 0) {
        const uint4 v0 = reinterpret_cast<const uint4 *>(rp)[0], v1 = reinterpret_cast<const uint4 *>(rp)[1];
        row[0] = v0.x; row[1] = v0.y; row[2] = v0.z; row[3] = v0.w; row[4] = v1.x; row[5] = v1.y; row[6] = v1.z; row[7] = v1.w;
        row[8] = rp[8];
    } else {
#pragma unroll
        for (int k = 0; k < 9; k++) row[k] = k < nd.stride ? rp[k] : 0u;
    }
}

template <bool SAMPLE>
__global__ void __launch_bounds__(PB_THREADS, 6) k_pile_build(NodesDev nd, const uint32_t *__restrict__ skeys, const uint32_t *__restrict__ sids, uint64_t n_entries, const uint4 *__restrict__ dir, ClusterCfg cc, int U,
                                                           uint4 *__restrict__ rec, uint4 *__restrict__ tab, uint32_t epoch,
                                                           uint4 *__restrict__ side, unsigned long long *__restrict__ pile_cnt, uint32_t *__restrict__ own_mask,
                                                           uint32_t *__restrict__ plist, uint32_t *__restrict__ pcount) {
    if (!SAMPLE && pile_declines(pile_cnt)) return;
    const int idx_shift = cc.idx_shift, kk = cc.kk;
    __shared__ uint32_t sRow[PB_THREADS][PILE_SW];
    __shared__ unsigned long long sKm[PB_THREADS];
    __shared__ unsigned long long sLead[PB_THREADS];
    __shared__ unsigned long long sRm[PB_THREADS];
    __shared__ uint32_t sMin[PB_THREADS], sMax[PB_THREADS];
    __shared__ uint32_t sBad[PB_THREADS];
    __shared__ uint8_t sTag[PB_THREADS];
    __shared__ uint32_t sCount[3];
    __shared__ uint32_t sPiles;
    const int t = (int) threadIdx.x;
    const uint64_t base = (uint64_t) blockIdx.x * PB_TILE;
    const uint64_t j = base + (uint64_t) t;
    const bool have = j < n_entries;
    const uint64_t jc = have ? j : (n_entries ? n_entries - 1 : 0);
    const uint32_t key = skeys[jc], node_id = min(sids[jc], (uint32_t) nd.n - 1u);
    const uint32_t meta = key >> (cc.idx_shift - CL_MBITS);
    const bool tgt = have && key != 0xFFFFFFFFu;
    uint4 drec = make_uint4(0u, 0u, 0u, 0u);
    if (tgt) drec = dir[key >> idx_shift];
    const uint64_t e0 = drec.x;
    const uint32_t cnt = drec.y;
    const bool owned = tgt && e0 >= base && e0 < base + PB_TILE && e0 <= j && j - e0 < (uint64_t) cnt;
    const int s = owned ? (int) (e0 - base) : 0;
    const int i = owned ? (int) (j - e0) : 0;
    const bool part = owned && cnt <= 64u;
    uint32_t row[9] = {0u, 0u, 0u, 0u, 0u, 0u, 0u, 0u, 0u};
    if (part) load_row9(nd, node_id, row);
    sLead[t] = 0ull; sRm[t] = 0ull; sMin[t] = 0xFFFFFFFFu; sMax[t] = 0u; sBad[t] = 0u;
    if (t < 3) sCount[t] = 0u;
    if (t == 0) sPiles = 0u;
    __syncthreads();
    const int m = (int) (meta & 63u);
    uint32_t A[PILE_SW];
    {
        const int w0 = (2 * m) >> 5, sh = (2 * m) & 31;
        const int lo = 2 * (64 - m), hi = lo + 2 * U;
        uint32_t Rp[18];
#pragma unroll
        for (int k = 0; k < 18; k++) Rp[k] = 0u;
#pragma unroll
        for (int k = 0; k < 9; k++) Rp[4 + k] = row[k];
        uint32_t m1 = 0u - (uint32_t) (w0 & 1), m2 = 0u - (uint32_t) ((w0 >> 1) & 1);
        asm volatile("" : "+v"(m1), "+v"(m2));
        uint32_t y1[PILE_SW + 3], y[PILE_SW + 1];
#pragma unroll
        for (int k = 0; k < PILE_SW + 3; k++) y1[k] = (Rp[k + 1] & m1) | (Rp[k] & ~m1);
#pragma unroll
        for (int k = 0; k <= PILE_SW; k++) y[k] = (y1[k + 2] & m2) | (y1[k] & ~m2);
#pragma unroll
        for (int k = 0; k < PILE_SW; k++) A[k] = funnel(y[k], y[k + 1], sh) & low_bits32(hi - 32 * k) & ~low_bits32(lo - 32 * k);
    }
    const unsigned long long kmask = kk >= 32 ? ~0ull : ((1ull << (2 * kk)) - 1ull);
    const unsigned long long kmer = (((unsigned long long) A[5] << 32) | A[4]) & kmask;
    sKm[t] = kmer;
#pragma unroll
    for (int k = 0; k < PILE_SW; k++) sRow[t][k] = A[k];
    __syncthreads();
    int L = t;
    if (part) {
        for (int u = 0; u < i; u++) if (sKm[s + u] == kmer) { L = s + u; break; }
        if (L == t) {
            atomicOr(&sLead[s], 1ull << i);
            sTag[t] = (uint8_t) (cluster_key(kmer_hash((uint32_t) kmer & cc.lo_mask, (uint32_t) (kmer >> 32) & cc.hi_mask), idx_shift - CL_MBITS) & 31u);
        }
        atomicMin(&sMin[L], ((uint32_t) m << 16) | (uint32_t) t);
        atomicMax(&sMax[L], ((uint32_t) m << 16) | (uint32_t) t);
        const unsigned long long bit = 1ull << (63 - m);
        if (atomicOr(&sRm[L], bit) & bit) atomicOr(&sBad[s], 1u);
    }
    __syncthreads();
    uint32_t *sSlot = reinterpret_cast<uint32_t *>(sKm);
    int my_slot = -1, my_rank = 0;
    if (part) {
        const unsigned long long lm = sLead[s];
        const int kgrp = __popcll(lm & ((1ull << (L - s)) - 1ull));
        if (kgrp < PILE_MAXSUB) {
            int before = 0;
            unsigned long long rest = lm;
#pragma unroll
            for (int g = 0; g < PILE_MAXSUB - 1; g++) {
                if (g < kgrp) { before += __popcll(sRm[s + __builtin_ctzll(rest)]); rest &= rest - 1ull; }
            }
            my_rank = m == 0 ? 0 : __popcll(sRm[L] >> (64 - m));
            my_slot = s + before + my_rank;
            if (my_slot < s + (int) cnt) sSlot[my_slot] = node_id; else my_slot = -1;
        }
    }
    uint32_t S[PILE_SW];
#pragma unroll
    for (int k = 0; k < PILE_SW; k++) S[k] = 0u;
    if (part) {
        const int t0 = (int) (sMax[L] & 0xFFFFu), t1 = (int) (sMin[L] & 0xFFFFu);
        const int lo = 2 * (64 - m), hi = lo + 2 * U;
        uint32_t diff = 0u;
#pragma unroll
        for (int k = 0; k < PILE_SW; k++) {
            S[k] = sRow[t0][k] | sRow[t1][k];
            diff |= (A[k] ^ S[k]) & low_bits32(hi - 32 * k) & ~low_bits32(lo - 32 * k);
        }
        if (diff != 0u) atomicOr(&sBad[s], 1u);
    }
    __syncthreads();
    if (owned) {
        uint4 *line = tab + (size_t) (key >> idx_shift) * 8;
        if (!part) {
            if (i == 0) {
                if (!SAMPLE) { line[3] = make_uint4(0u, 0u, 0u, (1u << 22) | (epoch << 23)); line[4] = make_uint4(127u, drec.x, drec.z, drec.w); }
                atomicAdd(&sCount[0], 1u); atomicAdd(&sCount[1], 1u);
            }
        } else {
            const unsigned long long lm = sLead[s];
            const int nsub = __popcll(lm);
            const int iL = L - s;
            const int k = __popcll(lm & ((1ull << iL) - 1ull));
            if (!SAMPLE) {
                const unsigned long long right = m == 0 ? 0ull : (sRm[L] >> (64 - m));
                uint32_t succ_id = 0xFFFFFFFFu, delta = 0u;
                if (right != 0ull && my_slot > s && my_rank >= 1) { succ_id = sSlot[my_slot - 1]; delta = 1u + (uint32_t) __builtin_ctzll(right); }
                const bool first_group = (k == 0 || own_mask != nullptr) && k < PILE_MAXSUB && sBad[s] == 0u && nsub <= PILE_MAXSUB;
                const bool leftmost = first_group && t == (int) (sMax[L] & 0xFFFFu);
                side[j] = make_uint4(node_id, succ_id, delta | ((uint32_t) m << 8) | ((uint32_t) k << 16) | (leftmost ? 0x40000000u : 0u) | (first_group ? 0x80000000u : 0u),
                                     k == 0 ? key >> idx_shift : (uint32_t) (e0 + (uint64_t) k));
                if (leftmost && plist) plist[(size_t) blockIdx.x * PB_THREADS + atomicAdd(&sPiles, 1u)] = pile_who((uint32_t) k, k == 0 ? key >> idx_shift : (uint32_t) (e0 + (uint64_t) k), cc.n_buckets, n_entries);
                if (!first_group && own_mask) atomicOr(&own_mask[j >> 5], 1u << (j & 31u));
            }
            if (!SAMPLE && L == t && k >= 1 && k < PILE_MAXSUB) {
                const unsigned long long rm = sRm[t];
                const uint64_t slot = e0 + (uint64_t) k;
                rec[slot * 4 + 0] = make_uint4(S[0], S[1], S[2], S[3]);
                rec[slot * 4 + 1] = make_uint4(S[4], S[5], S[6], S[7]);
                rec[slot * 4 + 2] = make_uint4(S[8], S[9], S[10], S[11]);
                rec[slot * 4 + 3] = make_uint4(S[12], 0u, (uint32_t) rm, (uint32_t) (rm >> 32));
            }
            if (i == 0) {
                uint32_t tg[PILE_MAXSUB] = {0u, 0u, 0u, 0u};
                unsigned long long rest = lm;
#pragma unroll
                for (int g = 0; g < PILE_MAXSUB; g++) {
                    if (rest) { tg[g] = sTag[s + __builtin_ctzll(rest)]; rest &= rest - 1ull; }
                }
                const bool irregular = sBad[s] != 0u || nsub > PILE_MAXSUB;
                const uint32_t ns1 = (uint32_t) (nsub < PILE_MAXSUB ? nsub : PILE_MAXSUB) - 1u;
                if (!SAMPLE) {
                    const unsigned long long rm = sRm[t];
                    line[0] = make_uint4(S[0], S[1], S[2], S[3]);
                    line[1] = make_uint4(S[4], S[5], S[6], S[7]);
                    line[2] = make_uint4(S[8], S[9], S[10], S[11]);
                    line[3] = make_uint4(S[12], (uint32_t) rm, (uint32_t) (rm >> 32), tg[0] | (tg[1] << 5) | (tg[2] << 10) | (tg[3] << 15) | (ns1 << 20) | (irregular ? 1u << 22 : 0u) | (epoch << 23));
                }
                atomicAdd(&sCount[0], 1u);
                if (irregular) atomicAdd(&sCount[1], 1u);
            }
            if (!SAMPLE && L == s && t == (int) (sMax[s] & 0xFFFFu)) {
                line[4] = make_uint4(cnt, drec.x, drec.z, drec.w);
                line[5] = make_uint4(sSlot[s], sMin[s] >> 16, 0u, 0u);
            }
        }
    }
    if (!SAMPLE && have && t < PB_TILE && !(tgt && cnt <= 64u)) {
        side[j] = make_uint4(node_id, 0xFFFFFFFFu, 0u, 0u);
        if (own_mask) atomicOr(&own_mask[j >> 5], 1u << (j & 31u));
    }
    if (SAMPLE && owned) atomicAdd(&sCount[2], 1u);
    __syncthreads();
    if (!SAMPLE && plist && t == 0) pcount[blockIdx.x] = sPiles;
    if (SAMPLE && t < 3 && sCount[t]) atomicAdd(&pile_cnt[t], (unsigned long long) sCount[t]);
}

constexpr int PILE_RUNS = 8;
__device__ __forceinline__ void pile_list_store(uint4 *line, uint32_t entries, bool ok, int n, const uint32_t (&key)[PILE_RUNS], const uint32_t (&kc)[PILE_RUNS], uint32_t c1_last) {
    uint32_t *lw = reinterpret_cast<uint32_t *>(line);
    if (ok) {
        line[5] = make_uint4(key[0], key[1], key[2], key[3]);
        line[6] = make_uint4(key[4], key[5], key[6], key[7]);
        line[7] = make_uint4(kc[0] | (kc[1] << 16), kc[2] | (kc[3] << 16), kc[4] | (kc[5] << 16), kc[6] | (kc[7] << 16));
        bool dup = false;
#pragma unroll
        for (int a = 0; a < PILE_RUNS; a++)
#pragma unroll
            for (int b = a + 1; b < PILE_RUNS; b++) dup = dup || (b < n && key[a] == key[b]);
        lw[16] = (entries & 255u) | ((uint32_t) n << 8) | ((c1_last & 255u) << 16) | (dup ? 0x80000000u : 0u);
    } else lw[16] = entries & 255u;
}

__global__ void __launch_bounds__(256) k_pile_runs(const uint4 *__restrict__ side, uint64_t n_entries, uint32_t n_buckets, uint4 *__restrict__ tab, const uint2 *__restrict__ runs,
                                                   int n_nodes, int nwin, const unsigned long long *__restrict__ pile_cnt) {
    if (pile_declines(pile_cnt)) return;
    const uint64_t j = (uint64_t) blockIdx.x * 256 + threadIdx.x;
    if (j >= n_entries) return;
    const uint4 sd = side[j];
    if (((sd.z >> 30) & 1u) == 0u) return;
    uint4 *line = tab + (size_t) min(sd.w, n_buckets) * 8;
    const uint4 l4 = line[4], l5 = line[5];
    const uint4 *r0 = reinterpret_cast<const uint4 *>(runs + (size_t) min(sd.x, (uint32_t) n_nodes - 1u) * CL_RMAX);
    const uint4 *r1 = reinterpret_cast<const uint4 *>(runs + (size_t) min(l5.x, (uint32_t) n_nodes - 1u) * CL_RMAX);
    const uint4 a0 = r0[0], a1 = r0[1], a2 = r0[2], a3 = r0[3], b0 = r1[0], b1 = r1[1], b2 = r1[2];
    const int s0 = -(int) ((sd.z >> 8) & 63u), s1 = -(int) (l5.y & 63u), seam = s0 + nwin;
    const uint32_t k0[CL_RMAX] = {a0.x, a0.z, a1.x, a1.z, a2.x, a2.z, a3.x, a3.z}, y0[CL_RMAX] = {a0.y, a0.w, a1.y, a1.w, a2.y, a2.w, a3.y, a3.w};
    const uint32_t k1[6] = {b0.x, b0.z, b1.x, b1.z, b2.x, b2.z}, y1[6] = {b0.y, b0.w, b1.y, b1.w, b2.y, b2.w};
    const int nr0 = (int) (y0[0] >> 24), nr1 = (int) (y1[0] >> 24);
    bool ok = nr0 >= 1 && nr0 <= CL_RMAX && nr1 >= 1 && nr1 <= 6 && s1 <= seam;
    uint32_t ok_[PILE_RUNS], kc_[PILE_RUNS];
#pragma unroll
    for (int k = 0; k < PILE_RUNS; k++) { ok_[k] = 0u; kc_[k] = 0u; }
    int n = 0;
    uint32_t last_key = 0u, last_pos = 0xFFFFFFFFu, c1_last = 0u;
#pragma unroll
    for (int r = CL_RMAX - 1; r >= 0; r--) {
        if (ok && r < nr0) {
            const uint32_t kpos = (uint32_t) (s0 + (int) (y0[r] & 255u) + 64), c0 = (uint32_t) (s0 + (int) ((y0[r] >> 8) & 255u) + 64), c1 = (uint32_t) (s0 + (int) ((y0[r] >> 16) & 255u) + 64);
#pragma unroll
// ... 603 lines not shown
            const int ds0 = U - cfg.rsoemo + 1;
            const unsigned long long lowm = ds0 <= 0 ? 0ull : (ds0 >= 64 ? ~0ull : ((1ull << ds0) - 1ull));
            two = d2 < ds0 || __popcll(occ & ((1ull << d2) - 1ull) & ~lowm) < 3;
        }
        if (id1 == 0xFFFFFFFFu || (nkept == 2 && id2 == 0xFFFFFFFFu)) dfr = true;
        else {
            slot_val = ((unsigned long long) id1 << 32) | (uint32_t) d1 | (two ? 0x100u : 0u);
            if (two) o.second[Bs - o.src_base] = ((unsigned long long) id2 << 32) | (uint32_t) d2;
            st_rec += two ? 2 : 1;
        }
    }
    if (have) o.first[Bs - o.src_base] = slot_val;
    dfr = dfr && nr_code != 0;
    const uint64_t dm = __ballot(dfr);
    if (dm != 0ull) {
        if (dfr) sDefer[wave][n_defer + (int) __builtin_amdgcn_mbcnt_hi((uint32_t) (dm >> 32), __builtin_amdgcn_mbcnt_lo((uint32_t) dm, 0u))] = Bs;
        n_defer += __popcll(dm);
        wave_lds_fence();
        if (n_defer >= 64) flush_defer();
    }
    }
    flush_defer();
    st_rec = wave_sum_u64(st_rec);
    if (lane == 0 && st_rec) atomicAdd(&o.counters[CNT_VALID_RECORDS], (unsigned long long) st_rec);
}

__global__ void __launch_bounds__(256) k_pile_deg(int32_t n, unsigned long long *__restrict__ first, uint32_t *__restrict__ deg, const unsigned long long *__restrict__ pile_cnt) {
    if (pile_declines(pile_cnt)) return;
    const int64_t i = (int64_t) blockIdx.x * 256 + threadIdx.x;
    if (i >= n) return;
    const unsigned long long f = first[i];
    if (f == LOCAL_FIRST_NONE || deg[i] != 0u) return;
    deg[i] = 1u + (uint32_t) ((f >> 8) & 1ull);
    if (f & 0x100ull) first[i] = f & ~0x100ull;
}

bool pile_plan(const PrefSufCfg &cfg, const ClusterCfg &cc, int eq, int uniform_len, bool masks) {
    if (eq != PILE_EQ || uniform_len <= 0 || masks || cfg.stats) return false;
    if (uniform_len > 144 || blocks_of(uniform_len) > 9) return false;
    if (uniform_len - cfg.Lmin + 1 > 64 || cc.w > 64 || cc.w < 16 || cc.kk > 32 || cc.kk < 1) return false;
    return true;
}
size_t pile_record_bytes(uint64_t n) { return (size_t) (n + 2) * 64; }

size_t pile_table_bytes(uint32_t n_buckets) { return ((size_t) n_buckets + 2) * 128; }

__global__ void k_pile_sample_close(unsigned long long *__restrict__ pile_cnt) {
    const unsigned long long by_entries = pile_cnt[2] / 8ull;
    if (by_entries > pile_cnt[0]) pile_cnt[0] = by_entries;
}

__global__ void k_pile_sample_force(unsigned long long *__restrict__ pile_cnt, unsigned long long buckets, unsigned long long irregular) { pile_cnt[0] = buckets; pile_cnt[1] = irregular; }

void launch_pile_sample(const NodesDev &nd, const ClusterCfg &cc, int uniform_len, const uint32_t *skeys, const uint32_t *sids, const void *dir, unsigned long long *pile_cnt,
                        int no_sample, hipStream_t s) {
    (void) hipMemsetAsync(pile_cnt, 0, PILE_CNT_WORDS * sizeof(unsigned long long), s);
    const uint64_t n_entries = nd.n > 0 ? (uint64_t) nd.n : 0;
    if (no_sample == 2) hipLaunchKernelGGL(k_pile_sample_force, dim3(1), dim3(1), 0, s, pile_cnt, 100ull, 1ull);
    if (n_entries == 0 || no_sample) return;
    const uint64_t tiles = (n_entries + PB_TILE - 1) / PB_TILE;
    const dim3 sample((unsigned) std::max<uint64_t>(1, std::min<uint64_t>(tiles, std::max<uint64_t>(64, tiles / 32)))), block(PB_THREADS);
    hipLaunchKernelGGL((k_pile_build<true>), sample, block, 0, s, nd, skeys, sids, n_entries, (const uint4 *) dir, cc, uniform_len, (uint4 *) nullptr, (uint4 *) nullptr, 0u, (uint4 *) nullptr, pile_cnt,
                       (uint32_t *) nullptr, (uint32_t *) nullptr, (uint32_t *) nullptr);
    hipLaunchKernelGGL(k_pile_sample_close, dim3(1), dim3(1), 0, s, pile_cnt);
}

void launch_pile_build(const NodesDev &nd, const PrefSufCfg &cfg, const ClusterCfg &cc, int uniform_len, const uint32_t *skeys, const uint32_t *sids, const void *dir, void *rec, void *rec2,
                       void *tab, uint32_t epoch, void *side, const void *runs, int nwin, const unsigned long long *pile_cnt, uint32_t *own_mask, void *plist, hipStream_t s) {
    const uint64_t n_entries = nd.n > 0 ? (uint64_t) nd.n : 0;
    if (n_entries == 0) return;
    const uint64_t tiles = (n_entries + PB_TILE - 1) / PB_TILE;
    if (!own_mask) plist = nullptr;
    uint32_t *pl = (uint32_t *) plist, *pc = pl ? pl + tiles * PB_THREADS : nullptr;
    if (own_mask) (void) hipMemsetAsync(own_mask, 0, pile_own_mask_bytes(n_entries), s);
    hipLaunchKernelGGL((k_pile_build<false>), dim3((unsigned) tiles), dim3(PB_THREADS), 0, s, nd, skeys, sids, n_entries, (const uint4 *) dir, cc, uniform_len, (uint4 *) rec, (uint4 *) tab, epoch,
                       (uint4 *) side, const_cast<unsigned long long *>(pile_cnt), own_mask, pl, pc);
    if (pl)
        hipLaunchKernelGGL(k_pile_runs_consensus_list, dim3((unsigned) ((tiles + PR_SEGS - 1) / PR_SEGS)), dim3(TK_ROWS), 0, s, (const uint32_t *) pl, (const uint32_t *) pc, (uint32_t) tiles,
                           (const uint4 *) side, n_entries, (uint4 *) tab, (const uint4 *) rec, (uint4 *) rec2, cc, uniform_len, cfg.Lmin, pile_cnt, own_mask);
    else if (own_mask)
        hipLaunchKernelGGL(k_pile_runs_consensus, dim3((unsigned) ((n_entries + PR_TILE - 1) / PR_TILE)), dim3(TK_ROWS), 0, s, (const uint4 *) side, n_entries, cc.n_buckets, (uint4 *) tab,
                           (const uint4 *) rec, (uint4 *) rec2, cc, uniform_len, cfg.Lmin, pile_cnt, own_mask);
    else
        hipLaunchKernelGGL(k_pile_runs, dim3((unsigned) ((n_entries + 255) / 256)), dim3(256), 0, s, (const uint4 *) side, n_entries, cc.n_buckets, (uint4 *) tab, (const uint2 *) runs, nd.n, nwin, pile_cnt);
}

size_t pile_own_mask_bytes(uint64_t n) { return (size_t) ((n + 31) / 32 + 1024) * 4; }

size_t pile_list_bytes(uint64_t n) { const uint64_t tiles = (n + PB_TILE - 1) / PB_TILE; return (size_t) (tiles * (PB_THREADS + 1) + 64) * 4; }

void launch_pile_own_ids(const uint32_t *own_mask, const uint32_t *sids, uint64_t n_entries, int32_t *list, uint32_t cap, unsigned long long *pile_cnt, hipStream_t s) {
    if (n_entries == 0) return;
    const uint64_t words = (n_entries + 31) / 32;
    hipLaunchKernelGGL(k_pile_own_ids, dim3((unsigned) ((words + 1023) / 1024)), dim3(256), 0, s, own_mask, sids, n_entries, list, cap, pile_cnt + 3, (const unsigned long long *) pile_cnt);
}

void launch_pile_check(const void *side, uint64_t n_entries, uint32_t n_buckets, const void *tab, const void *rec2, uint32_t epoch, const void *runs, int n_nodes, int nwin,
                       unsigned long long *pile_cnt, hipStream_t s) {
    if (n_entries == 0) return;
    hipLaunchKernelGGL(k_pile_list_check, dim3((unsigned) ((n_entries + 255) / 256)), dim3(256), 0, s, (const uint4 *) side, n_entries, n_buckets, (const uint4 *) tab, (const uint4 *) rec2, epoch,
                       (const uint2 *) runs,
                       n_nodes, nwin, pile_cnt + 4, (const unsigned long long *) pile_cnt);
}

constexpr int PSR_IPT = 4;
__global__ void __launch_bounds__(256) k_pile_side_range(const uint4 *__restrict__ side, uint64_t n_entries, uint32_t src_begin, uint32_t src_end, uint4 *__restrict__ out,
                                                         uint64_t out_cap, unsigned long long *__restrict__ cursor, const unsigned long long *__restrict__ pile_cnt) {
    if (pile_declines(pile_cnt)) return;
    __shared__ uint32_t cnt[PSR_IPT * 4];
    __shared__ unsigned long long base;
    const int wave = (int) (threadIdx.x >> 6);
    const uint64_t b0 = (uint64_t) blockIdx.x * (256 * PSR_IPT);
    uint4 v[PSR_IPT];
    uint32_t before[PSR_IPT];
    bool in[PSR_IPT];
#pragma unroll
    for (int k = 0; k < PSR_IPT; k++) {
        const uint64_t j = b0 + (uint64_t) k * 256 + threadIdx.x;
        v[k] = j < n_entries ? side[j] : make_uint4(0xFFFFFFFFu, 0u, 0u, 0u);
        in[k] = j < n_entries && v[k].x >= src_begin && v[k].x < src_end;
        const uint64_t m = __ballot(in[k]);
        before[k] = (uint32_t) __builtin_amdgcn_mbcnt_hi((uint32_t) (m >> 32), __builtin_amdgcn_mbcnt_lo((uint32_t) m, 0u));
        if ((threadIdx.x & 63u) == 0u) cnt[k * 4 + wave] = (uint32_t) __popcll(m);
    }
    __syncthreads();
    if (threadIdx.x == 0) {
        uint32_t tot = 0;
        for (int i = 0; i < PSR_IPT * 4; i++) tot += cnt[i];
        base = tot ? atomicAdd(cursor, (unsigned long long) tot) : 0ull;
    }
    __syncthreads();
    uint32_t run = 0;
#pragma unroll
    for (int k = 0; k < PSR_IPT; k++) {
        uint32_t mine = run;
        for (int w = 0; w < 4; w++) { if (w < wave) mine += cnt[k * 4 + w]; run += cnt[k * 4 + w]; }
        const unsigned long long at = base + mine + before[k];
        if (in[k] && at < out_cap) out[at] = v[k];
    }
}

void launch_pile_probe(const NodesDev &nd, const PrefSufCfg &cfg, const ClusterCfg &cc, int uniform_len, const void *tab, uint32_t epoch, const void *rec, const void *rec2,
                       const void *side, const void *runs, unsigned long long *counters, uint32_t *deg, unsigned long long *first, unsigned long long *second,
                       int32_t *defer_list, uint32_t defer_cap, const unsigned long long *pile_cnt, int n_cu, hipStream_t s, int32_t src_begin, int32_t src_end,
                       void *side_range, unsigned long long *cursor, bool lean) {
    const uint64_t n_entries = nd.n > 0 ? (uint64_t) nd.n : 0;
    if (n_entries == 0 || src_end <= src_begin) return;
// ... 24 lines not shown
```

### alga_amd/csrc/prefsuf_shard.hip

```cpp
#include <hip/hip_runtime.h>
#include <algorithm>
#include "prefsuf_common.h"
#include "prefsuf_kernels.h"
#include "prefsuf_device.h"
#include "prefsuf_cluster_device.h"
#include "prefsuf_shard.h"

namespace alga {

constexpr int SJ_QW = 17;
constexpr int SJ_DMAX = 4096;
constexpr int SJ_WAVES = 4;

__device__ __forceinline__ uint32_t shard_owner(uint32_t key, int shift, uint32_t bpr, uint32_t n_ranks) {
    const uint32_t o = (key >> shift) / bpr;
    return o < n_ranks ? o : n_ranks - 1u;
}

__device__ __forceinline__ uint32_t wave_min_u32_dpp(uint32_t v) {
    uint32_t t;
    t = (uint32_t) __builtin_amdgcn_update_dpp(-1, (int) v, 0x111, 0xF, 0xF, false); v = t < v ? t : v;
    t = (uint32_t) __builtin_amdgcn_update_dpp(-1, (int) v, 0x112, 0xF, 0xF, false); v = t < v ? t : v;
    t = (uint32_t) __builtin_amdgcn_update_dpp(-1, (int) v, 0x114, 0xF, 0xF, false); v = t < v ? t : v;
    t = (uint32_t) __builtin_amdgcn_update_dpp(-1, (int) v, 0x118, 0xF, 0xF, false); v = t < v ? t : v;
// ... 211 lines not shown
#pragma unroll
            for (int k = 4 * EQ; k < SJ_QW; k++) sb[k] = 0u;
        } else {
#pragma unroll
            for (int k = 0; k < SJ_QW; k++) sb[k] = (k < nw && k < nd.stride) ? row[k] : 0u;
        }
        sSrc[wave][lane] = src; sLen[wave][lane] = (uint32_t) lenA;
        wave_lds_fence();
    };
    auto verify = [&](bool has, const uint32_t (&ew)[4 * EQ], int &p) -> bool {
        const uint32_t id = ew[4 * EQ - 3], ekey = ew[4 * EQ - 2], meta = ew[4 * EQ - 1];
        const int lenC = (int) ((meta >> 8) & 0xFFFu);
        p = q - (int) (meta & 255u);
        const bool ok = has & same_cluster(ekey, key, fs) & (p >= p0) & (p < p1) & (id != src) & (lenC >= lenA - p);
        p = ok ? p : 0;
        const int nb = 2 * (lenA - p), qw = (2 * p) >> 5, sh = (2 * p) & 31;
        uint32_t diff = 0;
#pragma unroll
        for (int k = 0; k < WC; k++) {
            const uint32_t x = funnel(sb[qw + k], sb[qw + k + 1], sh) ^ ew[k];
            if (k < kfull) diff |= x;
            else diff |= x & low_bits32(nb - 32 * k);
        }
        return ok && diff == 0;
    };
    auto via = [&](uint32_t srcB, int lenB, int pB, uint32_t b0, uint32_t b1, uint32_t b2, uint32_t b3, int p, int rho_c) -> bool {
        const int delta = p - pB;
        const bool same = srcB == src;
        const int rho_b = lenB - (lenA - delta);
        const bool vok = (!same) & (pB > 0) & (delta >= 0) & (lenB - pB >= Lbig) & (rho_b >= 0) & (rho_b <= rho_c) & ((rho_b > 0) | (srcB > src));
        const int dd = delta < 0 ? 0 : delta;
        const int nb = 2 * pB, qw = (2 * dd) >> 5, sh = (2 * dd) & 31;
        const uint32_t diff = ((funnel(sb[qw], sb[qw + 1], sh) ^ b0) & low_bits32(nb)) | ((funnel(sb[qw + 1], sb[qw + 2], sh) ^ b1) & low_bits32(nb - 32)) |
                              ((funnel(sb[qw + 2], sb[qw + 3], sh) ^ b2) & low_bits32(nb - 64)) | ((funnel(sb[qw + 3], sb[qw + 4], sh) ^ b3) & low_bits32(nb - 96));
        return (vok && diff == 0) || (same && pB < p);
    };
    auto push = [&](uint32_t C, int p) {
        const int L = lenA - p;
        const unsigned long long val = ((unsigned long long) ol_pack(p, L, L < cfg.rsoemo) << 32) | src;
        const uint32_t i = atomicAdd(w.recN, 1u);
        if (i < (uint32_t) SJ_WB) { w.recC[i] = C; w.recV[i] = val; }
        else store_record(o, atomicAdd(&o.counters[CNT_RECORDS], 1ull), C, val);
        st_rec++;
    };
    auto maybe_flush = [&]() {
        wave_lds_fence();
        const int nb2 = (int) __builtin_amdgcn_readfirstlane((int) *w.recN);
        if (nb2 >= SJ_WB / 2) flush_records<REC_CHUNK, SJ_WB>(o, w, chunk_base, chunk_fill);
    };

    auto big_group = [&](uint64_t gs, int D) {
        if (D > dmax) { if (lane == 0) atomicOr(declined, 1ull); return; }
        const uint32_t b = (uint32_t) __builtin_amdgcn_readfirstlane((int) (dkey[gs] >> shift));
        const uint4 rec = dir[b];
        const uint32_t e0 = rec.x, ecnt = rec.y;
        const int nch = (D + 63) >> 6;
        for (int cc2 = 0; cc2 < nch; cc2++) {
            const int cnt = D - 64 * cc2 < 64 ? D - 64 * cc2 : 64;
            if (lane < cnt) { const uint64_t i = gs + 64u * (uint64_t) cc2 + lane; small_top[3 * i] = 0ull; small_top[3 * i + 1] = 0ull; small_top[3 * i + 2] = 0ull; }
        }
        for (uint32_t c = 0; c < ecnt; c++) {
            uint32_t ew[4 * EQ];
            {
                const uint4 *ent = store + (size_t) (e0 + c) * EQ;
#pragma unroll
                for (int k4 = 0; k4 < EQ; k4++) { const uint4 v = ent[k4]; ew[4 * k4] = v.x; ew[4 * k4 + 1] = v.y; ew[4 * k4 + 2] = v.z; ew[4 * k4 + 3] = v.w; }
            }
            const uint32_t meta = ew[4 * EQ - 1], idC = ew[4 * EQ - 3];
            const int lenC = (int) ((meta >> 8) & 0xFFFu);
            uint64_t any = 0ull;
            for (int cc2 = 0; cc2 < nch; cc2++) {
                const int cnt = D - 64 * cc2 < 64 ? D - 64 * cc2 : 64;
                load_descs(gs + 64u * (uint64_t) cc2, cnt);
                int p;
                const bool V = verify(act, ew, p);
                const uint64_t m = __ballot(V);
                if (lane == 0) sVM[wave][cc2] = m;
                any |= m;
                const int L = lenA - p;
                if (V && L < cfg.rsoemo) {
                    const uint64_t i = gs + 64u * (uint64_t) cc2 + lane;
                    uint64_t a = small_top[3 * i], b2 = small_top[3 * i + 1], c2 = small_top[3 * i + 2];
                    top3_insert(a, b2, c2, ((uint64_t) (uint32_t) L << 32) | idC);
                    small_top[3 * i] = a; small_top[3 * i + 1] = b2; small_top[3 * i + 2] = c2;
                }
            }
            wave_lds_fence();
            if (any == 0ull) continue;
            for (int cc2 = 0; cc2 < nch; cc2++) {
                const uint64_t cm = sVM[wave][cc2];
                if (cm == 0ull) continue;
                const int cnt = D - 64 * cc2 < 64 ? D - 64 * cc2 : 64;
                if (nch > 1) load_descs(gs + 64u * (uint64_t) cc2, cnt);
                const bool V = ((cm >> lane) & 1ull) != 0ull;
                const int p = q - (int) (meta & 255u);
                const int rho_c = lenC - (lenA - p);
                bool removed = false;
                for (int bb = 0; bb < nch; bb++) {
                    for (uint64_t bm = sVM[wave][bb]; bm != 0ull; bm &= bm - 1ull) {
                        const int bl = __builtin_ctzll(bm);
                        const bool test = V && !removed && !(bb == cc2 && bl == lane);
                        if (__ballot(test) == 0ull) continue;
                        const uint64_t bi = gs + 64u * (uint64_t) bb + (uint64_t) bl;
                        const unsigned long long vB = dval[bi];
                        const uint32_t srcB = (uint32_t) __builtin_amdgcn_readfirstlane((int) (uint32_t) vB);
                        const int pB = (int) ((uint32_t) __builtin_amdgcn_readfirstlane((int) (uint32_t) (vB >> 32)) & 255u) - (int) (meta & 255u);
                        const int lenB = ulen > 0 ? ulen : __builtin_amdgcn_readfirstlane(nd.len[srcB]);
                        const int nwB = blocks_of(lenB);
                        const uint32_t *rb = nd.words + (size_t) srcB * nd.stride;
                        uint32_t rB[4];
#pragma unroll
                        for (int k = 0; k < 4; k++) rB[k] = (k < nwB && k < nd.stride) ? rb[k] : 0u;
                        removed = removed || (test && p >= pB && via(srcB, lenB, pB, rB[0], rB[1], rB[2], rB[3], p, rho_c));
                    }
                }
                if (V && !removed) push(idC, p);
                maybe_flush();
            }
        }
    };

    const uint32_t total_waves = gridDim.x * SJ_WAVES;
    for (uint32_t g0 = ((uint32_t) blockIdx.x * SJ_WAVES + (uint32_t) wave) * SJ_GCH; g0 < n_groups; g0 += total_waves * SJ_GCH) {
        const uint32_t gend = g0 + SJ_GCH < n_groups ? g0 + SJ_GCH : n_groups;
        uint32_t ga = g0;
        while (ga < gend) {
            const uint32_t s0 = gstart[ga];
            const uint32_t gi = ga + 1u + (uint32_t) lane;
            const uint32_t ge = gstart[gi <= gend ? gi : gend];
            const uint64_t fits = __ballot(gi <= gend && ge - s0 <= 64u);
            const int ng = fits == ~0ull ? 64 : __builtin_ctzll(~fits);
            if (ng == 0) {
                big_group((uint64_t) s0, (int) min(gstart[ga + 1u] - s0, (uint32_t) SJ_DMAX + 1u));
                ga++;
                continue;
            }
            const int cnt = (int) ((uint32_t) __builtin_amdgcn_readlane((int) ge, ng - 1) - s0);
            ga += (uint32_t) ng;
            load_descs((uint64_t) s0, cnt);
            const uint32_t b = act ? key >> shift : 0xFFFFFFFFu;
            const uint32_t bprev = bperm(b, (lane + 63) & 63);
            const uint64_t starts = __ballot(act && (lane == 0 || b != bprev));
            const int gfirst = 63 - __builtin_clzll((long long) ((starts & (lane >= 63 ? ~0ull : ((2ull << lane) - 1ull))) | 1ull));
            const uint4 rec = dir[act ? b - bucket_base : 0u];
            uint32_t e0 = rec.x, ecnt = act ? rec.y : 0u;
            const uint64_t wide = __ballot(act && ecnt > 64u);
            if (wide != 0ull) ecnt = ecnt > 64u ? 0u : ecnt;
            const uint32_t max_e = wave_max_u32_dpp_or0(ecnt);
            int ebase;
            {
                uint32_t inc = (act && lane == gfirst) ? ecnt : 0u, t;
                t = (uint32_t) __builtin_amdgcn_update_dpp(0, (int) inc, 0x111, 0xF, 0xF, false); inc += t;
                t = (uint32_t) __builtin_amdgcn_update_dpp(0, (int) inc, 0x112, 0xF, 0xF, false); inc += t;
                t = (uint32_t) __builtin_amdgcn_update_dpp(0, (int) inc, 0x114, 0xF, 0xF, false); inc += t;
                t = (uint32_t) __builtin_amdgcn_update_dpp(0, (int) inc, 0x118, 0xF, 0xF, false); inc += t;
                t = (uint32_t) __builtin_amdgcn_update_dpp(0, (int) inc, 0x142, 0xA, 0xF, false); inc += t;
                t = (uint32_t) __builtin_amdgcn_update_dpp(0, (int) inc, 0x143, 0xC, 0xF, false); inc += t;
                ebase = (int) (bperm(inc, gfirst) - ecnt);
            }
            uint64_t vmask = 0, k0 = 0, k1 = 0, k2 = 0;
            uint32_t en[4 * EQ];
            auto load_entry = [&](uint32_t c, uint32_t (&ew)[4 * EQ]) {
                const uint4 *ent = store + (size_t) (c < ecnt ? e0 + c : e0) * EQ;
#pragma unroll
                for (int k4 = 0; k4 < EQ; k4++) { const uint4 v = ent[k4]; ew[4 * k4] = v.x; ew[4 * k4 + 1] = v.y; ew[4 * k4 + 2] = v.z; ew[4 * k4 + 3] = v.w; }
            };
            load_entry(0u, en);
            for (uint32_t c = 0; c < max_e; c++) {
                uint32_t ew[4 * EQ];
#pragma unroll
                for (int k = 0; k < 4 * EQ; k++) ew[k] = en[k];
                load_entry(c + 1u, en);
                const bool has = c < ecnt;
                int p;
                const bool V = verify(has, ew, p);
                vmask |= V ? 1ull << c : 0ull;
                const int L = lenA - p;
                if (V && L < cfg.rsoemo) top3_insert(k0, k1, k2, ((uint64_t) (uint32_t) L << 32) | ew[4 * EQ - 3]);
                if (has && lane == gfirst && ebase + (int) c < SJ_ES) { sEI[wave][ebase + (int) c] = ew[4 * EQ - 3]; sEM[wave][ebase + (int) c] = ew[4 * EQ - 1]; }
            }
            if (act && ((wide >> gfirst) & 1ull) == 0ull) { small_top[3 * ((uint64_t) s0 + lane)] = k0; small_top[3 * ((uint64_t) s0 + lane) + 1] = k1; small_top[3 * ((uint64_t) s0 + lane) + 2] = k2; }
            wave_lds_fence();
            bool serial = __ballot(act && vmask != 0ull && ebase + 64 - (int) __builtin_clzll(vmask | 1ull) > SJ_ES) != 0ull;
            if (!serial) {
                const int total_e = (int) bperm((uint32_t) (ebase + (int) ecnt), 63 - (int) __builtin_clzll((long long) (starts | 1ull)));
                wave_lds_fence();
                for (int k = lane; k < total_e && k < SJ_ES; k += 64) sTab[wave][k] = 0xFFFFFFFFu;
                wave_lds_fence();
                for (uint64_t m = vmask; m != 0ull; m &= m - 1ull) {
                    const int es = ebase + (int) __builtin_ctzll(m);
                    atomicMin(&sTab[wave][es], ((uint32_t) (q - (int) (sEM[wave][es] & 255u)) << 6) | (uint32_t) lane);
                }
                wave_lds_fence();
                bool undecided = false;
                uint64_t mine = 0ull;
                for (uint64_t m = vmask; m != 0ull; m &= m - 1ull) {
                    const int c = (int) __builtin_ctzll(m), es = ebase + c;
// ... 331 lines not shown
```

### alga_amd/engine.py

```python
import ctypes as C
import os

import numpy as np

_HERE = os.path.dirname(os.path.abspath(__file__))
_LIB = None

EDGE_DTYPE = np.dtype([("src", np.int32), ("dst", np.int32), ("offset", np.int32)])


class AlgaError(RuntimeError):
    def __init__(self, code, msg):
        super().__init__("alga_amd error %d: %s" % (code, msg))
        self.code = code


class _Nodes(C.Structure):
    _fields_ = [("words", C.c_void_p), ("stride_words", C.c_int32), ("len", C.c_void_p), ("n", C.c_int32),
                ("align_from", C.c_void_p), ("align_to", C.c_void_p)]


class PrefSufParams(C.Structure):
    _fields_ = [("min_overlap", C.c_int32), ("rsoe_min_overlap", C.c_int32), ("soes", C.c_int32),
                ("max_len_cap", C.c_int32), ("collect_stats", C.c_int32), ("reduction", C.c_int32),
                ("keys_shared", C.c_int32), ("twin_rows", C.c_int32)]


class CompactEdges(C.Structure):
    _fields_ = [("n_nodes", C.c_int32), ("n_edges", C.c_uint64), ("degree", C.c_void_p), ("dst", C.c_void_p), ("offset", C.c_void_p)]


class PrefSufStats(C.Structure):
    _fields_ = [("raw_overlaps", C.c_uint64), ("transitive_listed", C.c_uint64), ("transitive_compares", C.c_uint64),
                ("transitive_removed", C.c_uint64), ("windows_probed", C.c_uint64), ("slots_scanned", C.c_uint64),
                ("records", C.c_uint64), ("edges", C.c_uint64), ("table_slots", C.c_uint64),
                ("max_in_records", C.c_uint64), ("ms_total", C.c_double), ("ms_seed", C.c_double),
                ("ms_probe", C.c_double), ("ms_group", C.c_double), ("ms_reduce", C.c_double), ("ms_emit", C.c_double),
                ("nodes_live", C.c_uint64), ("reduction_used", C.c_uint64), ("generic_sources", C.c_uint64),
                ("big_sources", C.c_uint64), ("probe_used", C.c_uint64), ("deferred_sources", C.c_uint64), ("ms_probe_pairs", C.c_double),
                ("ms_keys", C.c_double), ("ms_sort", C.c_double), ("ms_gather", C.c_double), ("ms_dir", C.c_double), ("probe_rounds", C.c_uint64), ("ms_pile", C.c_double),
                ("pile_buckets", C.c_uint64), ("pile_irregular", C.c_uint64), ("pile_list_checked", C.c_uint64), ("pile_list_mismatch", C.c_uint64),
                ("pile_own_lists", C.c_uint64), ("host_ms_check", C.c_double), ("host_ms_upload", C.c_double), ("host_ms_build", C.c_double),
                ("host_ms_download", C.c_double), ("pile_mixed", C.c_uint64), ("pile_deferred", C.c_uint64)]

    def as_dict(self):
        return {k: getattr(self, k) for k, _ in self._fields_ if k != "reserved"}


class IngestParams(C.Structure):
    _fields_ = [("trim_left", C.c_int32), ("trim_right", C.c_int32), ("remove_reads_with_n", C.c_int32), ("rna", C.c_int32),
                ("scale", C.c_float), ("min_overlap", C.c_int32), ("rsoemo", C.c_int32), ("remove_pref_reads", C.c_int32),
                ("threads", C.c_int32)]


class NodeSet(C.Structure):
    _fields_ = [("n", C.c_int32), ("stride_words", C.c_int32), ("words", C.POINTER(C.c_uint32)), ("len", C.POINTER(C.c_int32)),
                ("pair_off", C.POINTER(C.c_uint8)), ("LEN", C.c_int32), ("min_overlap", C.c_int32), ("rsoemo", C.c_int32),
                ("li_kmer_length", C.c_int32), ("records", C.c_int64), ("removed_n", C.c_int32), ("removed_str", C.c_int32),
                ("removed_prefix", C.c_int32), ("removed_short", C.c_int32), ("avg_len", C.c_double)]


class ParsedReads(C.Structure):
    _fields_ = [("n_nodes", C.c_int64), ("stride_words", C.c_int32), ("rows", C.POINTER(C.c_uint32)), ("len", C.POINTER(C.c_int32)),
                ("paired", C.c_int32), ("records", C.c_int64), ("removed_n", C.c_int32), ("removed_str", C.c_int32), ("LEN", C.c_int32),
                ("min_overlap", C.c_int32), ("rsoemo", C.c_int32), ("li_kmer_length", C.c_int32), ("avg_len", C.c_double),
                ("owner", C.c_void_p)]


class PreprocessInput(C.Structure):
    _fields_ = [("rows", C.c_void_p), ("stride_words", C.c_int32), ("len", C.c_void_p), ("n_nodes", C.c_int64),
                ("remove_pref_reads", C.c_int32), ("min_keep_len", C.c_int32)]


class DeviceNodeSet(C.Structure):
    _fields_ = [("d_words", C.c_void_p), ("d_len", C.c_void_p), ("d_pair_off", C.c_void_p), ("n", C.c_int32), ("stride_words", C.c_int32),
                ("removed_prefix", C.c_int32), ("removed_short", C.c_int32), ("max_len", C.c_int32), ("ms_device", C.c_double)]


class IngestInfo(C.Structure):
    _fields_ = [("records", C.c_int64), ("removed_n", C.c_int32), ("removed_str", C.c_int32), ("LEN", C.c_int32), ("min_overlap", C.c_int32),
                ("rsoemo", C.c_int32), ("li_kmer_length", C.c_int32), ("paired", C.c_int32), ("avg_len", C.c_double), ("ms_parse", C.c_double),
                ("ms_preprocess", C.c_double), ("ms_upload", C.c_double)]


class PkbParams(C.Structure):
    _fields_ = [("min_overlap_area", C.c_int32), ("max_offset_pct", C.c_int32), ("min_identity_pct", C.c_int32),
                ("same_ends", C.c_int32), ("li_k", C.c_int32), ("li_intervals", C.c_int32), ("rounds", C.c_int32),
                ("kmer_length_bucket", C.c_int32)]


class PkbStats(C.Structure):
    _fields_ = [("kmers", C.c_uint64 * 4), ("groups", C.c_uint64 * 4), ("can_align_calls", C.c_uint64 * 4),
                ("edges_after", C.c_uint64 * 4), ("max_group", C.c_uint64), ("ms_total", C.c_double), ("group_hist", (C.c_uint64 * 8) * 4)]


PROBE = {"auto": 0, "table": 1, "cluster": 2}
# ... 819 lines not shown
```

### include/alga_amd.h

```cpp
#ifndef ALGA_AMD_H
#define ALGA_AMD_H

#include <stddef.h>
#include <stdint.h>

#ifdef __cplusplus
extern "C" {
#endif

#define ALGA_AMD_ABI_VERSION 7

typedef enum {
    ALGA_OK = 0,
    ALGA_ERR_INVALID_ARGUMENT = -1,
    ALGA_ERR_NO_DEVICE = -2,
    ALGA_ERR_HIP = -3,
    ALGA_ERR_OUT_OF_MEMORY = -4,
    ALGA_ERR_CAPACITY = -5,
    ALGA_ERR_IO = -6,
    ALGA_ERR_UNSUPPORTED = -7
} alga_status;

typedef enum { ALGA_REDUCTION_AUTO = 0, ALGA_REDUCTION_PER_TARGET = 1, ALGA_REDUCTION_SOURCE_SIDE = 2 } alga_reduction;

// ... 2 lines not shown
typedef struct alga_engine alga_engine;

typedef struct { int32_t src, dst, offset; } alga_edge;

typedef struct {
    const uint32_t *words;
    int32_t         stride_words;
    const int32_t  *len;
    int32_t         n;
    const uint8_t  *align_from;
    const uint8_t  *align_to;
} alga_nodes;

typedef struct {
    int32_t min_overlap;
    int32_t rsoe_min_overlap;
    int32_t soes;
    int32_t max_len_cap;
    int32_t collect_stats;
    int32_t reduction;
    int32_t keys_shared;
    int32_t twin_rows;
} alga_prefsuf_params;

typedef struct {
    uint64_t raw_overlaps;
    uint64_t transitive_listed;
    uint64_t transitive_compares;
    uint64_t transitive_removed;
    uint64_t windows_probed;
    uint64_t slots_scanned;
    uint64_t records;
    uint64_t edges;
    uint64_t table_slots;
    uint64_t max_in_records;
    double   ms_total;
    double   ms_seed, ms_probe, ms_group, ms_reduce, ms_emit;
    uint64_t nodes_live;
    uint64_t reduction_used;
    uint64_t generic_sources;
    uint64_t big_sources;
    uint64_t probe_used;
    uint64_t deferred_sources;
    double   ms_probe_pairs;
    double   ms_keys, ms_sort, ms_gather, ms_dir;
    uint64_t probe_rounds;
    double   ms_pile;
    uint64_t pile_buckets, pile_irregular;
    uint64_t pile_list_checked, pile_list_mismatch;
    uint64_t pile_own_lists;
    double   host_ms_check, host_ms_upload, host_ms_build, host_ms_download;
    uint64_t pile_mixed;
    uint64_t pile_deferred;
} alga_prefsuf_stats;
#define ALGA_PILE_IRREGULAR_ONE_IN 250
#define ALGA_PILE_DECLINE_ONE_IN 20

int         alga_abi_version(void);
int         alga_engine_create(int hip_device, alga_engine **out);
void        alga_engine_destroy(alga_engine *e);
const char *alga_last_error(const alga_engine *e);
int         alga_engine_device_name(const alga_engine *e, char *buf, size_t buflen);

int         alga_engine_set_option(alga_engine *e, const char *name, int64_t value);

void        alga_prefsuf_default_params(alga_prefsuf_params *p);

int  alga_prefsuf_build_host(alga_engine *e, const alga_nodes *nodes, const alga_prefsuf_params *p,
                             alga_edge **edges, uint64_t *n_edges);
void alga_free_edges(alga_engine *e, alga_edge *edges);

typedef struct {
    int32_t         n_nodes;
    uint64_t        n_edges;
    const uint8_t  *degree;
    const uint32_t *dst;
    const uint8_t  *offset;
} alga_compact_edges;
int         alga_prefsuf_build_host_compact(alga_engine *e, const alga_nodes *nodes, const alga_prefsuf_params *p, alga_compact_edges *out);
int         alga_download_edges_compact(alga_engine *e, int32_t n_nodes, const alga_edge *d_edges, uint64_t n_edges, alga_compact_edges *out);
void        alga_free_compact_edges(alga_engine *e, alga_compact_edges *c);

void       *alga_host_alloc(alga_engine *e, size_t bytes);
void        alga_host_free(alga_engine *e, void *p);

int  alga_engine_reserve(alga_engine *e, int32_t n_nodes, int32_t max_len, int32_t min_overlap, uint64_t n_edges_hint);

int  alga_upload_nodes(alga_engine *e, const alga_nodes *nodes, alga_nodes *dev);
int  alga_upload_twin_nodes(alga_engine *e, const alga_nodes *nodes , alga_nodes *dev);
int  alga_download_edges(alga_engine *e, const alga_edge *d_edges, uint64_t n_edges, alga_edge **edges);

int  alga_prefsuf_build_device(alga_engine *e, const alga_nodes *nodes, const alga_prefsuf_params *p,
                               void *hip_stream, const alga_edge **d_edges, uint64_t *n_edges);

int  alga_copy_to_host(alga_engine *e, void *dst, const void *d_src, size_t bytes);

int  alga_device_alloc(alga_engine *e, size_t bytes, void **d_out);
void alga_device_free(alga_engine *e, void *d_ptr);
int  alga_copy_to_device(alga_engine *e, void *d_dst, const void *src, size_t bytes);

int  alga_prefsuf_last_stats(const alga_engine *e, alga_prefsuf_stats *out);

int  alga_prefsuf_discover_device(alga_engine *e, const alga_nodes *nodes, const alga_prefsuf_params *p,
                                  int32_t src_begin, int32_t src_end, void *hip_stream,
                                  const uint32_t **d_dst, const uint64_t **d_val, uint64_t *n_records);
int  alga_prefsuf_reduce_device(alga_engine *e, const alga_nodes *nodes, const alga_prefsuf_params *p,
// ... 213 lines not shown
```

Baseline: 5.062 billion edges/s.

## Build bucket directory inside pile build and epoch-tag it to skip memset

```diff
diff --git a/alga_amd/csrc/engine.hip b/alga_amd/csrc/engine.hip
--- a/alga_amd/csrc/engine.hip
+++ b/alga_amd/csrc/engine.hip
@@ -165,6 +165,7 @@
     ClusterCfg cc{};
     if (clustered) {
         cc = pp.cluster;
+        cc.dir_epoch = e->dir_epoch;
         if ((rc = cluster_alloc(e, pp))) return rc;
         if (pp.keys_shared == 2) {
             const bool store_left = e->store_n == nd.n && e->store_words == (const void *) nd.words && e->store_eq == pp.cluster_eq && e->store_buckets == cc.n_buckets;
@@ -188,8 +189,19 @@
             e->keyed_n = -1;
             e->store_n = -1;
             HIP_TRY(e, launch_cluster_store(nd, cc, (uint32_t *) e->cl_keys[0].p, (uint32_t *) e->cl_vals[0].p, (uint32_t *) e->cl_keys[1].p,
-                                            (uint32_t *) e->cl_vals[1].p, e->sort_temp.p, cluster_sort_temp_bytes((uint64_t) nd.n), e->cl_dir.p, pp.keys_shared == 1 || !need_vals,
-                                            e->ev[EV_SORT], cnt + CNT_TOTAL + 1, e->opt_test_unsorted_index != 0, s, e->opt_own_sort != 0));
+                                            (uint32_t *) e->cl_vals[1].p, e->sort_temp.p, cluster_sort_temp_bytes((uint64_t) nd.n), pp.keys_shared == 1 || !need_vals,
+                                            e->ev[EV_SORT], e->opt_test_unsorted_index != 0, s, e->opt_own_sort != 0));
+            if (e->cl_dir.p != e->dir_p || e->cl_dir.cap != e->dir_cap || e->dir_epoch >= DIR_EPOCH_LAST) {
+                HIP_TRY(e, hipMemsetAsync(e->cl_dir.p, 0, e->cl_dir.cap, s));
+                e->dir_p = e->cl_dir.p; e->dir_cap = e->cl_dir.cap;
+                e->dir_epoch = 0;
+            }
+            cc.dir_epoch = ++e->dir_epoch;
+            const bool dir_first = !pile || e->expect_pairwise || !e->opt_pile_dir;
+            if (dir_first) {
+                HIP_TRY(e, launch_cluster_dir(cc, (const uint32_t *) e->cl_keys[1].p, (uint64_t) nd.n, e->cl_dir.p, !e->opt_pile_dir, cnt + CNT_TOTAL + 1, nullptr, s));
+                if ((rc = alga_check_launch(e, "k_tgt_dir"))) return rc;
+            }
             HIP_TRY(e, hipEventRecord(e->ev[EV_DIR], s));
             e->pile_n = -1;
             if (pile) {
@@ -202,6 +214,10 @@
                     e->err.clear();
                     pile = false;
                     rc = ALGA_OK;
+                    if (!dir_first) {
+                        HIP_TRY(e, launch_cluster_dir(cc, (const uint32_t *) e->cl_keys[1].p, (uint64_t) nd.n, e->cl_dir.p, false, cnt + CNT_TOTAL + 1, nullptr, s));
+                        if ((rc = alga_check_launch(e, "k_tgt_dir"))) return rc;
+                    }
                     if (keys_only) {
                         launch_cluster_keys(nd, cfg, cc, 0, nd.n, (uint32_t *) e->cl_keys[0].p, (uint32_t *) e->cl_vals[0].p, (uint32_t *) e->cl_meta.p, e->cl_runs.p,
                                             (uint8_t *) e->cl_nruns.p, s, true);
@@ -211,9 +227,14 @@
                 } else if (rc) return rc;
             }
             if (pile) {
-                launch_pile_sample(nd, cc, pp.uniform_len, (const uint32_t *) e->cl_keys[1].p, (const uint32_t *) e->cl_vals[1].p, e->cl_dir.p,
+                launch_pile_sample(nd, cc, pp.uniform_len, (const uint32_t *) e->cl_keys[1].p, (const uint32_t *) e->cl_vals[1].p,
                                    (unsigned long long *) e->cl_pile_cnt.p, e->opt_pile >= 2 ? e->opt_pile - 1 : 0, s);
                 if ((rc = alga_check_launch(e, "k_pile_build<sample>"))) return rc;
+                if (!dir_first) {
+                    HIP_TRY(e, launch_cluster_dir(cc, (const uint32_t *) e->cl_keys[1].p, (uint64_t) nd.n, e->cl_dir.p, false, cnt + CNT_TOTAL + 1,
+                                                  (const unsigned long long *) e->cl_pile_cnt.p, s));
+                    if ((rc = alga_check_launch(e, "k_tgt_dir"))) return rc;
+                }
             }
             HIP_TRY(e, launch_cluster_gather(nd, cc, pp.cluster_eq, (const uint32_t *) e->cl_keys[1].p, (const uint32_t *) e->cl_vals[1].p, (const uint32_t *) e->cl_meta.p,
                                              pp.uniform_len, e->cl_store.p, (pile && e->opt_pile_skip_gather) ? (const unsigned long long *) e->cl_pile_cnt.p : nullptr, s));
@@ -225,10 +246,19 @@
                 }
                 e->pile_epoch++;
                 const bool from_consensus = e->opt_pile_runs != 0;
-                launch_pile_build(nd, cfg, cc, pp.uniform_len, (const uint32_t *) e->cl_keys[1].p, (const uint32_t *) e->cl_vals[1].p, e->cl_dir.p, e->cl_pile_rec.p, e->cl_pile_rec2.p, e->cl_pile_tab.p,
-                                  e->pile_epoch, e->cl_pile_succ.p, e->cl_runs.p, pp.uniform_len - cfg.Lmin + 1, (const unsigned long long *) e->cl_pile_cnt.p,
+                launch_pile_build(nd, cfg, cc, pp.uniform_len, (const uint32_t *) e->cl_keys[1].p, (const uint32_t *) e->cl_vals[1].p, dir_first ? nullptr : e->cl_dir.p,
+                                  cnt + CNT_TOTAL + 1, e->cl_pile_rec.p, e->cl_pile_rec2.p, e->cl_pile_tab.p, e->pile_epoch, e->cl_pile_succ.p, e->cl_runs.p, pp.uniform_len - cfg.Lmin + 1, (const unsigned long long *) e->cl_pile_cnt.p,
                                   from_consensus ? (uint32_t *) e->cl_pile_own.p : nullptr, (from_consensus && e->opt_pile_runs_list) ? e->cl_pile_list.p : nullptr, s);
                 if ((rc = alga_check_launch(e, "k_pile_build"))) return rc;
+                if (e->opt_pile_dir_check) {
+                    const size_t dbytes = ((size_t) cc.n_buckets + 2) * 16;
+                    if ((rc = alga_ensure(e, e->cl_dir_check, dbytes + 16))) return rc;
+                    unsigned long long *dchk = (unsigned long long *) ((char *) e->cl_dir_check.p + dbytes);
+                    HIP_TRY(e, hipMemsetAsync(e->cl_dir_check.p, 0, dbytes + 16, s));
+                    HIP_TRY(e, launch_cluster_dir(cc, (const uint32_t *) e->cl_keys[1].p, (uint64_t) nd.n, e->cl_dir_check.p, false, cnt + CNT_TOTAL + 1, nullptr, s));
+                    launch_pile_dir_check(e->cl_dir.p, e->cl_dir_check.p, cc.n_buckets, cc.dir_epoch, dchk, (const unsigned long long *) e->cl_pile_cnt.p, s);
+                    if ((rc = alga_check_launch(e, "k_pile_dir_check"))) return rc;
+                }
                 if (keys_only) {
                     launch_pile_own_ids((const uint32_t *) e->cl_pile_own.p, (const uint32_t *) e->cl_vals[1].p, (uint64_t) nd.n, (int32_t *) e->cl_defer.p, (uint32_t) nd.n,
                                         (unsigned long long *) e->cl_pile_cnt.p, s);
@@ -379,6 +409,13 @@
                 e->expect_pairwise = !kept;
                 e->pile_kept_pure = kept && !e->stats.pile_mixed && e->opt_pile_skip_gather != 0;
                 e->stats.pile_list_checked = 0; e->stats.pile_list_mismatch = 0;
+                e->stats.pile_dir_checked = 0; e->stats.pile_dir_mismatch = 0;
+                if (e->opt_pile_dir_check) {
+                    unsigned long long chk[2] = {0ull, 0ull};
+                    HIP_TRY(e, hipMemcpyAsync(chk, (const char *) e->cl_dir_check.p + ((size_t) cc.n_buckets + 2) * 16, sizeof(chk), hipMemcpyDeviceToHost, s));
+                    HIP_TRY(e, hipStreamSynchronize(s));
+                    e->stats.pile_dir_checked = chk[0]; e->stats.pile_dir_mismatch = chk[1];
+                }
                 if (e->opt_pile_check) {
                     unsigned long long chk[2] = {0ull, 0ull};
                     HIP_TRY(e, hipMemcpyAsync(chk, (const unsigned long long *) e->cl_pile_cnt.p + 4, sizeof(chk), hipMemcpyDeviceToHost, s));
@@ -636,6 +673,13 @@
         e->opt_pile_probe_lean = value != 0;
     } else if (!strcmp(name, "pile_check")) {
         e->opt_pile_check = value != 0;
+    } else if (!strcmp(name, "pile_dir")) {
+        e->opt_pile_dir = value != 0;
+    } else if (!strcmp(name, "pile_dir_check")) {
+        e->opt_pile_dir_check = value != 0;
+    } else if (!strcmp(name, "test_dir_epoch")) {
+        if (value < 0 || value > (int64_t) DIR_EPOCH_LAST) return alga_fail(e, ALGA_ERR_INVALID_ARGUMENT, "test_dir_epoch must be in [0, 255]");
+        e->dir_epoch = (uint32_t) value;
     } else if (!strcmp(name, "pile_skip_gather")) {
         e->opt_pile_skip_gather = value != 0;
     } else if (!strcmp(name, "cluster_order")) {
diff --git a/alga_amd/csrc/engine_internal.h b/alga_amd/csrc/engine_internal.h
--- a/alga_amd/csrc/engine_internal.h
+++ b/alga_amd/csrc/engine_internal.h
@@ -61,6 +61,9 @@
     int    opt_pile_probe_lean = 1;
     bool   pile_deg_pending = false;
     int    opt_pile_check = 0;
+    int    opt_pile_dir = 1;
+    int    opt_pile_dir_check = 0;
+    DevBuf cl_dir_check;
     bool   expect_pairwise = false;
     DevBuf cl_pile_side_r, cl_pile_cursor;
     DevBuf cl_pile_own;
@@ -77,6 +80,8 @@
     int    opt_cluster_order = 1;
     int    opt_cluster_pairs = 1;
     DevBuf cl_keys[2], cl_vals[2], cl_meta, cl_runs, cl_nruns, cl_store, cl_dir;
+    uint32_t dir_epoch = 0;
+    const void *dir_p = nullptr; size_t dir_cap = 0;
     DevBuf loc_second;
     bool   loc_second_used = false;
     uint32_t loc_slot_stride = 0;
diff --git a/alga_amd/csrc/prefsuf_cluster.hip b/alga_amd/csrc/prefsuf_cluster.hip
--- a/alga_amd/csrc/prefsuf_cluster.hip
+++ b/alga_amd/csrc/prefsuf_cluster.hip
@@ -140,7 +140,9 @@
 constexpr int TD_TILE = 256, TD_HALO = 96;
 __global__ void __launch_bounds__(TD_TILE) k_tgt_dir(const uint32_t *__restrict__ keys, uint64_t n, int shift, uint32_t n_buckets ,
                                                      uint32_t bucket_base , uint4 *__restrict__ dir,
-                                                     unsigned long long *__restrict__ bad ) {
+                                                     unsigned long long *__restrict__ bad ,
+                                                     uint32_t epoch, const unsigned long long *__restrict__ pile_cnt) {
+    if (pile_cnt && !pile_cnt_declines(pile_cnt)) return;
     __shared__ uint32_t sb[TD_TILE + TD_HALO + 1];
     const uint64_t base = (uint64_t) blockIdx.x * TD_TILE;
     const uint32_t nb3 = n_buckets << 3;
@@ -150,7 +152,7 @@
     __syncthreads();
     const int t = (int) threadIdx.x, lane = lane_id();
     const uint64_t j = base + (uint64_t) t;
-    auto put = [&](int64_t b, const uint4 &rec) { dir[b] = rec; };
+    auto put = [&](int64_t b, const uint4 &rec) { dir[b] = make_uint4(rec.x, rec.y, rec.z | epoch, rec.w); };
     auto tally = [](unsigned long long acc, uint32_t cls) { return acc + (0x0101010101010100ull << (8u * cls)); };
     if (j >= 1 && j < n && sb[t + 1] < sb[t]) atomicOr(bad, 1ull);
     const uint32_t b = sb[t + 1] >> 3;
@@ -305,7 +307,7 @@
         if (lane < STAGE_WORDS) sB[wave][buf][lane] = lane < nwB ? word0 : 0u;
         return lane < nr ? run.x >> cc.idx_shift : 0u;
     };
-    auto index_loads = [&](uint32_t bucket, uint4 &rec) { rec = dir[bucket]; };
+    auto index_loads = [&](uint32_t bucket, uint4 &rec) { rec = dir_load(dir, bucket, cc.dir_epoch); };
     auto finish_runs = [&](int buf, int nr, const uint2 &run, const uint4 &rec) -> uint32_t {
         uint32_t e0, cnt;
         run_slice(rec, run.y, e0, cnt);
@@ -513,7 +515,7 @@
                     wave_lds_fence();
                     uint32_t cnt = 0u;
                     if (start && rank >= rb && rank < rb + CL_RMAX) {
-                        const uint4 rec = dir[key >> cc.idx_shift];
+                        const uint4 rec = dir_load(dir, key >> cc.idx_shift, cc.dir_epoch);
                         const uint32_t ry = (wm & 255u) | ((uint32_t) wl << 8) | ((uint32_t) p1 << 16);
                         uint32_t e0;
                         run_slice(rec, ry, e0, cnt);
@@ -691,7 +693,7 @@
         if (gl == 0) sSrc[wave][4 * qb + g] = make_uint2((uint32_t) id, (uint32_t) lenB);
         return gl < nr_eff ? run.x >> cc.idx_shift : 0u;
     };
-    auto index_loads = [&](uint32_t bucket, uint4 &rec) { rec = dir[bucket]; };
+    auto index_loads = [&](uint32_t bucket, uint4 &rec) { rec = dir_load(dir, bucket, cc.dir_epoch); };
     auto finish_runs = [&](int qb, int nr_eff, const uint2 &run, const uint4 &rec) -> uint32_t {
         uint32_t e0, cnt;
         run_slice(rec, run.y, e0, cnt);
@@ -1058,8 +1060,8 @@
 }
 
 hipError_t launch_cluster_store(const NodesDev &nd, const ClusterCfg &cc, uint32_t *keys, uint32_t *vals, uint32_t *keys2, uint32_t *vals2,
-                                void *sort_temp, size_t sort_temp_bytes, void *dir, bool fill_vals,
-                                hipEvent_t ev_sorted, unsigned long long *bad_flag, bool test_skip_sort, hipStream_t s, bool own_sort) {
+                                void *sort_temp, size_t sort_temp_bytes, bool fill_vals,
+                                hipEvent_t ev_sorted, bool test_skip_sort, hipStream_t s, bool own_sort) {
     if (nd.n <= 0) return hipSuccess;
     const uint64_t n = (uint64_t) nd.n;
     if (fill_vals && (!own_sort || test_skip_sort)) hipLaunchKernelGGL(k_iota, dim3((unsigned) std::min<uint64_t>((n + 255) / 256, 8192)), dim3(256), 0, s, vals, (uint32_t) n);
@@ -1070,9 +1072,18 @@
     } else err = sort_u32_pairs(sort_temp, sort_temp_bytes, keys, keys2, own_sort ? (const uint32_t *) nullptr : vals, vals2, n, cc.idx_shift - 3, s, own_sort);
     if (err != hipSuccess) return err;
     if (ev_sorted) (void) hipEventRecord(ev_sorted, s);
-    err = hipMemsetAsync(dir, 0, ((size_t) cc.n_buckets + 2) * 16, s);
-    if (err != hipSuccess) return err;
-    hipLaunchKernelGGL(k_tgt_dir, dim3((unsigned) ((n + 1 + TD_TILE - 1) / TD_TILE)), dim3(TD_TILE), 0, s, (const uint32_t *) keys2, n, cc.idx_shift, cc.n_buckets, 0u, (uint4 *) dir, bad_flag);
+    return hipGetLastError();
+}
+
+hipError_t launch_cluster_dir(const ClusterCfg &cc, const uint32_t *keys2, uint64_t n, void *dir, bool fill, unsigned long long *bad_flag,
+                              const unsigned long long *pile_cnt, hipStream_t s) {
+    if (n == 0) return hipSuccess;
+    if (fill) {
+        const hipError_t err = hipMemsetAsync(dir, 0, ((size_t) cc.n_buckets + 2) * 16, s);
+        if (err != hipSuccess) return err;
+    }
+    hipLaunchKernelGGL(k_tgt_dir, dim3((unsigned) ((n + 1 + TD_TILE - 1) / TD_TILE)), dim3(TD_TILE), 0, s, keys2, n, cc.idx_shift, cc.n_buckets, 0u, (uint4 *) dir, bad_flag,
+                       cc.dir_epoch, pile_cnt);
     return hipGetLastError();
 }
 
@@ -1115,7 +1126,7 @@
 #undef TG_EQ
 #undef TG_LAUNCH
     hipLaunchKernelGGL(k_tgt_dir, dim3((unsigned) ((n + 1 + TD_TILE - 1) / TD_TILE)), dim3(TD_TILE), 0, s, (const uint32_t *) keys2, n, cc.idx_shift, n_buckets_local, bucket_base,
-                       (uint4 *) dir, bad_flag);
+                       (uint4 *) dir, bad_flag, 0u, (const unsigned long long *) nullptr);
     return hipGetLastError();
 }
 
diff --git a/alga_amd/csrc/prefsuf_cluster_device.h b/alga_amd/csrc/prefsuf_cluster_device.h
--- a/alga_amd/csrc/prefsuf_cluster_device.h
+++ b/alga_amd/csrc/prefsuf_cluster_device.h
@@ -45,6 +45,10 @@
 constexpr unsigned long long PILE_DECLINE_ONE_IN = ALGA_PILE_DECLINE_ONE_IN;
 __device__ __forceinline__ bool pile_cnt_declines(const unsigned long long *c) { return c[1] * PILE_DECLINE_ONE_IN > c[0]; }
 __device__ __forceinline__ bool pile_cnt_mixed(const unsigned long long *c) { return !pile_cnt_declines(c) && c[1] * PILE_IRREGULAR_ONE_IN > c[0]; }
+__device__ __forceinline__ uint4 dir_load(const uint4 *dir, uint32_t b, uint32_t epoch) {
+    const uint4 r = dir[b];
+    return (r.z & 255u) == epoch ? make_uint4(r.x, r.y, r.z & ~255u, r.w) : make_uint4(0u, 0u, 0u, 0u);
+}
 __device__ __forceinline__ void run_slice(const uint4 &rec, uint32_t run_y, uint32_t &e0, uint32_t &cnt) {
     const int q = (int) (run_y & 255u), p0 = (int) ((run_y >> 8) & 255u), p1 = (int) ((run_y >> 16) & 255u);
     int mlo = q - p1 + 1, mhi = q - p0;
diff --git a/alga_amd/csrc/prefsuf_common.h b/alga_amd/csrc/prefsuf_common.h
--- a/alga_amd/csrc/prefsuf_common.h
+++ b/alga_amd/csrc/prefsuf_common.h
@@ -95,7 +95,9 @@
     uint32_t hi_mask;
     int32_t  idx_shift;
     uint32_t n_buckets;
+    uint32_t dir_epoch = 0;
 };
+constexpr uint32_t DIR_EPOCH_LAST = 255;
 
 struct PrefSufCfg {
     int32_t Lmin;
diff --git a/alga_amd/csrc/prefsuf_kernels.h b/alga_amd/csrc/prefsuf_kernels.h
--- a/alga_amd/csrc/prefsuf_kernels.h
+++ b/alga_amd/csrc/prefsuf_kernels.h
@@ -41,9 +41,11 @@
 void       launch_cluster_runs_list(const NodesDev &nd, const PrefSufCfg &cfg, const ClusterCfg &cc, const int32_t *ids, const unsigned long long *count, uint32_t cap,
                                     uint32_t grid_blocks, void *runs, uint8_t *nruns, hipStream_t s);
 hipError_t launch_cluster_store(const NodesDev &nd, const ClusterCfg &cc, uint32_t *keys, uint32_t *vals, uint32_t *keys2 , uint32_t *vals2, void *sort_temp,
-                                size_t sort_temp_bytes, void *dir, bool fill_vals, hipEvent_t ev_sorted ,
-                                unsigned long long *bad_flag ,
+                                size_t sort_temp_bytes, bool fill_vals, hipEvent_t ev_sorted ,
                                 bool test_skip_sort , hipStream_t s, bool own_sort = true);
+hipError_t launch_cluster_dir(const ClusterCfg &cc, const uint32_t *keys2, uint64_t n, void *dir , bool fill ,
+                              unsigned long long *bad_flag ,
+                              const unsigned long long *pile_cnt , hipStream_t s);
 hipError_t launch_cluster_gather(const NodesDev &nd, const ClusterCfg &cc, int eq, const uint32_t *keys2, const uint32_t *vals2, const uint32_t *meta,
                                  int uniform_len , void *store,
                                  const unsigned long long *pile_cnt , hipStream_t s);
@@ -64,16 +66,20 @@
 bool       pile_plan(const PrefSufCfg &cfg, const ClusterCfg &cc, int eq, int uniform_len, bool masks);
 size_t     pile_record_bytes(uint64_t n);
 size_t     pile_table_bytes(uint32_t n_buckets);
-void       launch_pile_sample(const NodesDev &nd, const ClusterCfg &cc, int uniform_len, const uint32_t *skeys , const uint32_t *sids , const void *dir,
+void       launch_pile_sample(const NodesDev &nd, const ClusterCfg &cc, int uniform_len, const uint32_t *skeys , const uint32_t *sids ,
                               unsigned long long *pile_cnt , int no_sample, hipStream_t s);
 constexpr int PILE_CNT_WORDS = 6;
 size_t     pile_own_mask_bytes(uint64_t n);
 size_t     pile_list_bytes(uint64_t n);
-void       launch_pile_build(const NodesDev &nd, const PrefSufCfg &cfg, const ClusterCfg &cc, int uniform_len, const uint32_t *skeys, const uint32_t *sids, const void *dir, void *rec,
+void       launch_pile_build(const NodesDev &nd, const PrefSufCfg &cfg, const ClusterCfg &cc, int uniform_len, const uint32_t *skeys, const uint32_t *sids,
+                             void *dir ,
+                             unsigned long long *bad , void *rec,
                              void *rec2 , void *tab, uint32_t epoch, void *side, const void *runs, int nwin, const unsigned long long *pile_cnt,
                              uint32_t *own_mask ,
                              void *plist , hipStream_t s);
 void       launch_pile_own_ids(const uint32_t *own_mask, const uint32_t *sids, uint64_t n_entries, int32_t *list, uint32_t cap, unsigned long long *pile_cnt, hipStream_t s);
+void       launch_pile_dir_check(const void *dir, const void *ref , uint32_t n_buckets, uint32_t epoch,
+                                 unsigned long long *out , const unsigned long long *pile_cnt, hipStream_t s);
 void       launch_pile_check(const void *side, uint64_t n_entries, uint32_t n_buckets, const void *tab, const void *rec2, uint32_t epoch, const void *runs, int n_nodes, int nwin,
                              unsigned long long *pile_cnt, hipStream_t s);
 void       launch_probe_stream_list(const NodesDev &nd, const PrefSufCfg &cfg, const ClusterCfg &cc, int eq, const void *store, const void *dir, const void *runs, const uint8_t *nruns,
diff --git a/alga_amd/csrc/prefsuf_pile.hip b/alga_amd/csrc/prefsuf_pile.hip
--- a/alga_amd/csrc/prefsuf_pile.hip
+++ b/alga_amd/csrc/prefsuf_pile.hip
@@ -30,11 +30,13 @@
     }
 }
 
+constexpr int PB_BACK = PB_HALO + 1;
 template <bool SAMPLE>
-__global__ void __launch_bounds__(PB_THREADS, 6) k_pile_build(NodesDev nd, const uint32_t *__restrict__ skeys, const uint32_t *__restrict__ sids, uint64_t n_entries, const uint4 *__restrict__ dir, ClusterCfg cc, int U,
+__global__ void __launch_bounds__(PB_THREADS, 6) k_pile_build(NodesDev nd, const uint32_t *__restrict__ skeys, const uint32_t *__restrict__ sids, uint64_t n_entries, ClusterCfg cc, int U,
                                                            uint4 *__restrict__ rec, uint4 *__restrict__ tab, uint32_t epoch,
                                                            uint4 *__restrict__ side, unsigned long long *__restrict__ pile_cnt, uint32_t *__restrict__ own_mask,
-                                                           uint32_t *__restrict__ plist, uint32_t *__restrict__ pcount) {
+                                                           uint32_t *__restrict__ plist, uint32_t *__restrict__ pcount,
+                                                           uint4 *__restrict__ dir, unsigned long long *__restrict__ bad) {
     if (!SAMPLE && pile_declines(pile_cnt)) return;
     const int idx_shift = cc.idx_shift, kk = cc.kk;
     __shared__ uint32_t sRow[PB_THREADS][PILE_SW];
@@ -46,6 +48,7 @@
     __shared__ uint8_t sTag[PB_THREADS];
     __shared__ uint32_t sCount[3];
     __shared__ uint32_t sPiles;
+    __shared__ unsigned long long sStart[PB_THREADS / 64 + 2];
     const int t = (int) threadIdx.x;
     const uint64_t base = (uint64_t) blockIdx.x * PB_TILE;
     const uint64_t j = base + (uint64_t) t;
@@ -54,16 +57,51 @@
     const uint32_t key = skeys[jc], node_id = min(sids[jc], (uint32_t) nd.n - 1u);
     const uint32_t meta = key >> (cc.idx_shift - CL_MBITS);
     const bool tgt = have && key != 0xFFFFFFFFu;
-    uint4 drec = make_uint4(0u, 0u, 0u, 0u);
-    if (tgt) drec = dir[key >> idx_shift];
-    const uint64_t e0 = drec.x;
-    const uint32_t cnt = drec.y;
-    const bool owned = tgt && e0 >= base && e0 < base + PB_TILE && e0 <= j && j - e0 < (uint64_t) cnt;
-    const int s = owned ? (int) (e0 - base) : 0;
-    const int i = owned ? (int) (j - e0) : 0;
+    uint32_t *sKey = &sRow[0][0];
+    const uint32_t nb3 = cc.n_buckets << 3;
+    auto tagged = [&](uint64_t k) -> uint32_t { if (k >= n_entries) return nb3; const uint32_t x = skeys[k]; return x == 0xFFFFFFFFu ? nb3 : x >> (idx_shift - 3); };
+    sKey[t + PB_BACK] = !have || key == 0xFFFFFFFFu ? nb3 : key >> (idx_shift - 3);
+    if (t < PB_BACK) sKey[t] = base + (uint64_t) t >= (uint64_t) PB_BACK ? tagged(base + (uint64_t) t - PB_BACK) : 0xFFFFFFFFu;
+    if (t == PB_THREADS - 1) sKey[PB_THREADS + PB_BACK] = tagged(base + PB_THREADS);
+    __syncthreads();
+    {
+        const uint32_t x = sKey[t + PB_BACK], xp = sKey[t + PB_BACK - 1];
+        if (!SAMPLE && bad && t < PB_TILE && j >= 1 && j < n_entries && x < xp) atomicOr(bad, 1ull);
+        const unsigned long long st = __ballot((x >> 3) != (xp >> 3));
+        const unsigned long long sb = __ballot(t < 64 && (sKey[t + 1] >> 3) != (sKey[t] >> 3));
+        if ((t & 63) == 0) sStart[1 + (t >> 6)] = st;
+        if (t == 0) sStart[0] = sb;
+        if (t == PB_THREADS - 1) sStart[PB_THREADS / 64 + 1] = (sKey[PB_THREADS + PB_BACK] >> 3) != (x >> 3) ? 1ull : 0ull;
+    }
+    __syncthreads();
+    constexpr int SW = PB_THREADS / 64 + 2;
+    constexpr uint32_t BIG = 0xFFFFFFFFu;
+    int sp = -1000;
+    uint32_t cnt = BIG;
+    {
+        int w = 1 + (t >> 6);
+        unsigned long long m = sStart[w] & ((2ull << (t & 63)) - 1ull);
+        while (m == 0ull && w > 0) { w--; m = sStart[w]; }
+        if (m != 0ull) {
+            sp = (w - 1) * 64 + 63 - __builtin_clzll(m);
+            const int q = sp + 1 + 64;
+            int v = q >> 6;
+            unsigned long long r = sStart[v] & (~0ull << (q & 63));
+            while (r == 0ull && v < SW - 1) { v++; r = sStart[v]; }
+            if (r != 0ull) cnt = (uint32_t) ((v - 1) * 64 + __builtin_ctzll(r) - sp);
+        }
+    }
+    const bool owned = tgt && sp >= 0 && sp < PB_TILE;
+    const uint64_t e0 = base + (uint64_t) (sp >= 0 ? sp : 0);
+    const int s = owned ? sp : 0;
+    const int i = owned ? t - sp : 0;
     const bool part = owned && cnt <= 64u;
     uint32_t row[9] = {0u, 0u, 0u, 0u, 0u, 0u, 0u, 0u, 0u};
     if (part) load_row9(nd, node_id, row);
+    unsigned long long cls = 0ull;
+    if (!SAMPLE && part && i == 0)
+        for (uint32_t u = 0; u < cnt; u++) cls += 0x0101010101010100ull << (8u * (sKey[t + PB_BACK + (int) u] & 7u));
+    const bool bstart = (int) sp == t;
     sLead[t] = 0ull; sRm[t] = 0ull; sMin[t] = 0xFFFFFFFFu; sMax[t] = 0u; sBad[t] = 0u;
     if (t < 3) sCount[t] = 0u;
     if (t == 0) sPiles = 0u;
@@ -143,7 +181,24 @@
         uint4 *line = tab + (size_t) (key >> idx_shift) * 8;
         if (!part) {
             if (i == 0) {
-                if (!SAMPLE) { line[3] = make_uint4(0u, 0u, 0u, (1u << 22) | (epoch << 23)); line[4] = make_uint4(127u, drec.x, drec.z, drec.w); }
+                if (!SAMPLE) {
+                    const uint32_t bb = key >> idx_shift;
+                    unsigned long long acc = 0ull;
+                    uint64_t k = e0;
+                    for (; k < e0 + 256u; k++) {
+                        const uint32_t x = tagged(k);
+                        if ((x >> 3) != bb) break;
+                        acc += 0x0101010101010100ull << (8u * (x & 7u));
+                    }
+                    if (k >= e0 + 256u && (tagged(k) >> 3) == bb) {
+                        uint64_t a = k, z = n_entries;
+                        while (z - a > 1) { const uint64_t mid = a + (z - a) / 2; if ((tagged(mid) >> 3) == bb) a = mid; else z = mid; }
+                        k = z;
+                    }
+                    const uint32_t c = (uint32_t) (k - e0), cz = c <= 255u ? (uint32_t) acc : 0u, cw = c <= 255u ? (uint32_t) (acc >> 32) : 0u;
+                    line[3] = make_uint4(0u, 0u, 0u, (1u << 22) | (epoch << 23)); line[4] = make_uint4(127u, (uint32_t) e0, cz, cw);
+                    if (dir) dir[bb] = make_uint4((uint32_t) e0, c, cz | cc.dir_epoch, cw);
+                }
                 atomicAdd(&sCount[0], 1u); atomicAdd(&sCount[1], 1u);
             }
         } else {
@@ -185,16 +240,16 @@
                     line[1] = make_uint4(S[4], S[5], S[6], S[7]);
                     line[2] = make_uint4(S[8], S[9], S[10], S[11]);
                     line[3] = make_uint4(S[12], (uint32_t) rm, (uint32_t) (rm >> 32), tg[0] | (tg[1] << 5) | (tg[2] << 10) | (tg[3] << 15) | (ns1 << 20) | (irregular ? 1u << 22 : 0u) | (epoch << 23));
+                    line[4] = make_uint4(cnt, (uint32_t) e0, (uint32_t) cls, (uint32_t) (cls >> 32));
+                    line[5] = make_uint4(sSlot[s], sMin[s] >> 16, 0u, 0u);
+                    if (dir) dir[key >> idx_shift] = make_uint4((uint32_t) e0, cnt, (uint32_t) cls | cc.dir_epoch, (uint32_t) (cls >> 32));
                 }
                 atomicAdd(&sCount[0], 1u);
                 if (irregular) atomicAdd(&sCount[1], 1u);
             }
-            if (!SAMPLE && L == s && t == (int) (sMax[s] & 0xFFFFu)) {
-                line[4] = make_uint4(cnt, drec.x, drec.z, drec.w);
-                line[5] = make_uint4(sSlot[s], sMin[s] >> 16, 0u, 0u);
-            }
-        }
-    }
+        }
+    }
+    if (!SAMPLE && dir && bstart && !tgt && j <= n_entries && (t < PB_TILE || j == n_entries)) dir[cc.n_buckets] = make_uint4((uint32_t) j, 0u, cc.dir_epoch, 0u);
     if (!SAMPLE && have && t < PB_TILE && !(tgt && cnt <= 64u)) {
         side[j] = make_uint4(node_id, 0xFFFFFFFFu, 0u, 0u);
         if (own_mask) atomicOr(&own_mask[j >> 5], 1u << (j & 31u));
@@ -904,7 +959,7 @@
 
 __global__ void k_pile_sample_force(unsigned long long *__restrict__ pile_cnt, unsigned long long buckets, unsigned long long irregular) { pile_cnt[0] = buckets; pile_cnt[1] = irregular; }
 
-void launch_pile_sample(const NodesDev &nd, const ClusterCfg &cc, int uniform_len, const uint32_t *skeys, const uint32_t *sids, const void *dir, unsigned long long *pile_cnt,
+void launch_pile_sample(const NodesDev &nd, const ClusterCfg &cc, int uniform_len, const uint32_t *skeys, const uint32_t *sids, unsigned long long *pile_cnt,
                         int no_sample, hipStream_t s) {
     (void) hipMemsetAsync(pile_cnt, 0, PILE_CNT_WORDS * sizeof(unsigned long long), s);
     const uint64_t n_entries = nd.n > 0 ? (uint64_t) nd.n : 0;
@@ -912,21 +967,21 @@
     if (n_entries == 0 || no_sample) return;
     const uint64_t tiles = (n_entries + PB_TILE - 1) / PB_TILE;
     const dim3 sample((unsigned) std::max<uint64_t>(1, std::min<uint64_t>(tiles, std::max<uint64_t>(64, tiles / 32)))), block(PB_THREADS);
-    hipLaunchKernelGGL((k_pile_build<true>), sample, block, 0, s, nd, skeys, sids, n_entries, (const uint4 *) dir, cc, uniform_len, (uint4 *) nullptr, (uint4 *) nullptr, 0u, (uint4 *) nullptr, pile_cnt,
-                       (uint32_t *) nullptr, (uint32_t *) nullptr, (uint32_t *) nullptr);
+    hipLaunchKernelGGL((k_pile_build<true>), sample, block, 0, s, nd, skeys, sids, n_entries, cc, uniform_len, (uint4 *) nullptr, (uint4 *) nullptr, 0u, (uint4 *) nullptr, pile_cnt,
+                       (uint32_t *) nullptr, (uint32_t *) nullptr, (uint32_t *) nullptr, (uint4 *) nullptr, (unsigned long long *) nullptr);
     hipLaunchKernelGGL(k_pile_sample_close, dim3(1), dim3(1), 0, s, pile_cnt);
 }
 
-void launch_pile_build(const NodesDev &nd, const PrefSufCfg &cfg, const ClusterCfg &cc, int uniform_len, const uint32_t *skeys, const uint32_t *sids, const void *dir, void *rec, void *rec2,
-                       void *tab, uint32_t epoch, void *side, const void *runs, int nwin, const unsigned long long *pile_cnt, uint32_t *own_mask, void *plist, hipStream_t s) {
+void launch_pile_build(const NodesDev &nd, const PrefSufCfg &cfg, const ClusterCfg &cc, int uniform_len, const uint32_t *skeys, const uint32_t *sids, void *dir, unsigned long long *bad,
+                       void *rec, void *rec2, void *tab, uint32_t epoch, void *side, const void *runs, int nwin, const unsigned long long *pile_cnt, uint32_t *own_mask, void *plist, hipStream_t s) {
     const uint64_t n_entries = nd.n > 0 ? (uint64_t) nd.n : 0;
     if (n_entries == 0) return;
     const uint64_t tiles = (n_entries + PB_TILE - 1) / PB_TILE;
     if (!own_mask) plist = nullptr;
     uint32_t *pl = (uint32_t *) plist, *pc = pl ? pl + tiles * PB_THREADS : nullptr;
     if (own_mask) (void) hipMemsetAsync(own_mask, 0, pile_own_mask_bytes(n_entries), s);
-    hipLaunchKernelGGL((k_pile_build<false>), dim3((unsigned) tiles), dim3(PB_THREADS), 0, s, nd, skeys, sids, n_entries, (const uint4 *) dir, cc, uniform_len, (uint4 *) rec, (uint4 *) tab, epoch,
-                       (uint4 *) side, const_cast<unsigned long long *>(pile_cnt), own_mask, pl, pc);
+    hipLaunchKernelGGL((k_pile_build<false>), dim3((unsigned) tiles), dim3(PB_THREADS), 0, s, nd, skeys, sids, n_entries, cc, uniform_len, (uint4 *) rec, (uint4 *) tab, epoch,
+                       (uint4 *) side, const_cast<unsigned long long *>(pile_cnt), own_mask, pl, pc, (uint4 *) dir, dir ? bad : (unsigned long long *) nullptr);
     if (pl)
         hipLaunchKernelGGL(k_pile_runs_consensus_list, dim3((unsigned) ((tiles + PR_SEGS - 1) / PR_SEGS)), dim3(TK_ROWS), 0, s, (const uint32_t *) pl, (const uint32_t *) pc, (uint32_t) tiles,
                            (const uint4 *) side, n_entries, (uint4 *) tab, (const uint4 *) rec, (uint4 *) rec2, cc, uniform_len, cfg.Lmin, pile_cnt, own_mask);
@@ -945,6 +1000,27 @@
     if (n_entries == 0) return;
     const uint64_t words = (n_entries + 31) / 32;
     hipLaunchKernelGGL(k_pile_own_ids, dim3((unsigned) ((words + 1023) / 1024)), dim3(256), 0, s, own_mask, sids, n_entries, list, cap, pile_cnt + 3, (const unsigned long long *) pile_cnt);
+}
+
+__global__ void __launch_bounds__(256) k_pile_dir_check(const uint4 *__restrict__ dir, const uint4 *__restrict__ ref, uint32_t n_buckets, uint32_t epoch,
+                                                        unsigned long long *__restrict__ out , const unsigned long long *__restrict__ pile_cnt) {
+    if (pile_declines(pile_cnt)) return;
+    const uint64_t b = (uint64_t) blockIdx.x * 256 + threadIdx.x;
+    const bool in = b <= (uint64_t) n_buckets;
+    bool diff = false;
+    if (in) {
+        const uint4 x = dir_load(dir, (uint32_t) b, epoch), y = dir_load(ref, (uint32_t) b, epoch);
+        diff = x.x != y.x || x.y != y.y || x.z != y.z || x.w != y.w;
+    }
+    const unsigned long long nin = __ballot(in), nd = __ballot(diff);
+    if ((threadIdx.x & 63) == 0) {
+        if (nin) atomicAdd(&out[0], (unsigned long long) __popcll(nin));
+        if (nd) atomicAdd(&out[1], (unsigned long long) __popcll(nd));
+    }
+}
+
+void launch_pile_dir_check(const void *dir, const void *ref, uint32_t n_buckets, uint32_t epoch, unsigned long long *out, const unsigned long long *pile_cnt, hipStream_t s) {
+    hipLaunchKernelGGL(k_pile_dir_check, dim3((unsigned) (((uint64_t) n_buckets + 1 + 255) / 256)), dim3(256), 0, s, (const uint4 *) dir, (const uint4 *) ref, n_buckets, epoch, out, pile_cnt);
 }
 
 void launch_pile_check(const void *side, uint64_t n_entries, uint32_t n_buckets, const void *tab, const void *rec2, uint32_t epoch, const void *runs, int n_nodes, int nwin,
diff --git a/alga_amd/csrc/prefsuf_shard.hip b/alga_amd/csrc/prefsuf_shard.hip
--- a/alga_amd/csrc/prefsuf_shard.hip
+++ b/alga_amd/csrc/prefsuf_shard.hip
@@ -287,7 +287,7 @@
     auto big_group = [&](uint64_t gs, int D) {
         if (D > dmax) { if (lane == 0) atomicOr(declined, 1ull); return; }
         const uint32_t b = (uint32_t) __builtin_amdgcn_readfirstlane((int) (dkey[gs] >> shift));
-        const uint4 rec = dir[b];
+        const uint4 rec = dir_load(dir, b, cc.dir_epoch);
         const uint32_t e0 = rec.x, ecnt = rec.y;
         const int nch = (D + 63) >> 6;
         for (int cc2 = 0; cc2 < nch; cc2++) {
@@ -377,7 +377,7 @@
             const uint32_t bprev = bperm(b, (lane + 63) & 63);
             const uint64_t starts = __ballot(act && (lane == 0 || b != bprev));
             const int gfirst = 63 - __builtin_clzll((long long) ((starts & (lane >= 63 ? ~0ull : ((2ull << lane) - 1ull))) | 1ull));
-            const uint4 rec = dir[act ? b - bucket_base : 0u];
+            const uint4 rec = dir_load(dir, act ? b - bucket_base : 0u, cc.dir_epoch);
             uint32_t e0 = rec.x, ecnt = act ? rec.y : 0u;
             const uint64_t wide = __ballot(act && ecnt > 64u);
             if (wide != 0ull) ecnt = ecnt > 64u ? 0u : ecnt;
diff --git a/alga_amd/engine.py b/alga_amd/engine.py
--- a/alga_amd/engine.py
+++ b/alga_amd/engine.py
@@ -41,7 +41,8 @@
                 ("ms_keys", C.c_double), ("ms_sort", C.c_double), ("ms_gather", C.c_double), ("ms_dir", C.c_double), ("probe_rounds", C.c_uint64), ("ms_pile", C.c_double),
                 ("pile_buckets", C.c_uint64), ("pile_irregular", C.c_uint64), ("pile_list_checked", C.c_uint64), ("pile_list_mismatch", C.c_uint64),
                 ("pile_own_lists", C.c_uint64), ("host_ms_check", C.c_double), ("host_ms_upload", C.c_double), ("host_ms_build", C.c_double),
-                ("host_ms_download", C.c_double), ("pile_mixed", C.c_uint64), ("pile_deferred", C.c_uint64)]
+                ("host_ms_download", C.c_double), ("pile_mixed", C.c_uint64), ("pile_deferred", C.c_uint64),
+                ("pile_dir_checked", C.c_uint64), ("pile_dir_mismatch", C.c_uint64)]
 
     def as_dict(self):
         return {k: getattr(self, k) for k, _ in self._fields_ if k != "reserved"}
diff --git a/include/alga_amd.h b/include/alga_amd.h
--- a/include/alga_amd.h
+++ b/include/alga_amd.h
@@ -78,6 +78,7 @@
     double   host_ms_check, host_ms_upload, host_ms_build, host_ms_download;
     uint64_t pile_mixed;
     uint64_t pile_deferred;
+    uint64_t pile_dir_checked, pile_dir_mismatch;
 } alga_prefsuf_stats;
 #define ALGA_PILE_IRREGULAR_ONE_IN 250
 #define ALGA_PILE_DECLINE_ONE_IN 20
```

New measurement: 5.228 billion edges/s (median of 6 runs). 1.03x the previous value.
